# StephenTaf/Modern-Search-Engines-Project

Measured on AMD Instinct MI355X. Metric: queries/sec, two-stage retrieval top-100 (BM25 top-1000 + dense full scan + rerank/fuse), higher is better.
Workload: dtype f32 (exact f32 cosines of every returned document; candidates filtered by one pass of f16 products with a measured margin; batches <= 64 queries: f16x2-split products, |err| <= 8e-6) (dense cosine) / f64 (BM25, fuse)

## Files before the change

### modern-search-engines-project_amd/csrc/msr_common.h

```cpp
#pragma once
#include <hip/hip_runtime.h>
#include <stdint.h>

#define MSR_WAVE 64

__host__ __device__ __forceinline__ uint32_t msr_ord32(float f) {
    uint32_t u;
    __builtin_memcpy(&u, &f, 4);
    if (f == 0.0f) u = 0;
    return (u & 0x80000000u) ? ~u : (u | 0x80000000u);
}
__host__ __device__ __forceinline__ float msr_unord32(uint32_t u) {
    u = (u & 0x80000000u) ? (u & 0x7FFFFFFFu) : ~u;
    float f;
    __builtin_memcpy(&f, &u, 4);
    return f;
}
__host__ __device__ __forceinline__ uint64_t msr_ord64(double d) {
    uint64_t u;
    __builtin_memcpy(&u, &d, 8);
    if (d == 0.0) u = 0;
    return (u >> 63) ? ~u : (u | 0x8000000000000000ull);
}
__host__ __device__ __forceinline__ double msr_unord64(uint64_t u) {
    u = (u >> 63) ? (u & 0x7FFFFFFFFFFFFFFFull) : ~u;
    double d;
    __builtin_memcpy(&d, &u, 8);
    return d;
}

__device__ __forceinline__ bool msr_valid(float s) { return s > -__builtin_inff(); }
__device__ __forceinline__ bool msr_valid(double s) { return s > -__builtin_inf(); }
```

### modern-search-engines-project_amd/csrc/msr_dense.hip

```cpp
#include <stdlib.h>

#include <algorithm>
#include <type_traits>

#include "msr_common.h"
#include "msr_internal.h"
#include "msr_frag.h"

namespace {

constexpr int KSTEPS = MSR_DIM / 16;



template <int QB, int MODE, int WAVES, int OBD = 32> struct ScanCfgV2 {
    static constexpr int NL = MODE == MODE_BF16 ? MSR_DIM / 32 : MSR_DIM / 16;
    static constexpr int KS = MODE == MODE_F32 ? MSR_DIM / 16 : MSR_DIM / 32;
    static constexpr int QPIECES = MODE == MODE_F16X2 ? 2 : 1;
    static constexpr int ROW16 = MODE == MODE_BF16 ? MSR_DIM * 2 / 16 : MSR_DIM * 4 / 16;
    static constexpr int NQP = 16 * QB;
    static constexpr int SROW = NQP + 1;
    static constexpr int THREADS = WAVES * 64;
    static constexpr size_t q_bytes = (size_t)QB * KS * QPIECES * 64 * 16;
    static constexpr size_t t_bytes = (size_t)16 * SROW * 4;
    static constexpr size_t o_bytes = (size_t)OBD * SROW * 4;
    static constexpr size_t wave_bytes = (t_bytes + o_bytes + 15) & ~(size_t)15;
    static constexpr size_t total = q_bytes + WAVES * wave_bytes;
};

template <int QB, bool TILED, int LB, int MODE, int WAVES, int OBD = 32, int G = 1>
__global__ __launch_bounds__(WAVES * 64) void dense_scan_v2_kernel(DenseIndex ix, const void* __restrict__ emb,
                                                                    const int32_t* __restrict__ wspan,
                                                                    int n_wspans, const f32x4* __restrict__ qimg,
                                                                    int nq, int max_chunks,
                                                                    float* __restrict__ docscore, int dbg) {
    using L = ScanCfgV2<QB, MODE, WAVES, OBD>;
    constexpr int KS = L::KS, NL = L::NL;
    constexpr bool BF16 = MODE == MODE_BF16;
    constexpr bool DIRECT = OBD == 0;
    static_assert(OBD == 0 || OBD == 8 || OBD == 16 || OBD == 32, "staging depth");
    static_assert(NL % LB == 0 && (MODE != MODE_F16X2 || LB % 2 == 0), "whole load batches per group");
    static_assert(!(BF16 && TILED), "the interleaved image exists for f32 only");
    extern __shared__ __attribute__((aligned(16))) char smem[];
    f32x4* Qs = (f32x4*)smem;
    const int tid = threadIdx.x;
    const int lane = tid & 63;
    const int w = __builtin_amdgcn_readfirstlane(tid >> 6);
    float* T = (float*)(smem + L::q_bytes + (size_t)w * L::wave_bytes);
    float* OB = T + 16 * L::SROW;
    const int li = lane & 15, lg = lane >> 4;

    for (int idx = tid; idx < QB * KS * L::QPIECES * 64; idx += L::THREADS) Qs[idx] = qimg[idx];
    __syncthreads();

    const int s = blockIdx.x * WAVES + w;
    if (s >= n_wspans) return;
    if (ix.gate && *ix.gate == 0) return;
    const int64_t C = ix.n_chunks;
    const float NEG_INF = -__builtin_inff();
    const int d0 = wspan[s], d1 = wspan[s + 1];
    const int64_t c0 = ix.doc_off[d0], c1 = ix.doc_off[d1];

    int ob_base = d0, ob_n = 0;
    auto flush = [&]() {
        constexpr int OD = OBD > 0 ? OBD : 32;
        constexpr int QPI = 64 / OD;
        for (int qq0 = 0; qq0 < nq; qq0 += QPI) {
            const int qq = qq0 + lane / OD, dd = lane % OD;
            if (qq < nq && dd < ob_n && !(dbg & 1)) docscore[(int64_t)qq * ix.score_stride + ob_base + dd] = OB[dd * L::SROW + qq];
        }
        ob_base += ob_n;
        ob_n = 0;
    };
    auto emit = [&](float m) {
        if (DIRECT) {
            if (lane < nq) docscore[(int64_t)lane * ix.score_stride + ob_base] = m;
            ++ob_base;
            return;
        }
        if (lane < L::NQP) OB[ob_n * L::SROW + lane] = m;
        constexpr int OD = OBD > 0 ? OBD : 32;
        ++ob_n;
        if (((ob_base + ob_n) & (OD - 1)) == 0) flush();
    };

    int cur_doc = d0 - 1;
    bool open = false;
    int cnt = 0;
    float m = NEG_INF;

    if (c1 > c0) {
        constexpr int PSTRIDE = TILED ? 64 : 4;
        constexpr int NBATCH = NL / LB;
        const int64_t g0 = c0 >> 4, g1 = (c1 + 15) >> 4;
        auto row_ptr = [&](int64_t grp) -> const f32x4* {
            if (TILED) return (const f32x4*)emb + (size_t)grp * (16 * L::ROW16) + lane;
            int64_t r = grp * 16 + li;
            if (r > C - 1) r = C - 1;
            return (const f32x4*)emb + (size_t)r * L::ROW16 + lg;
        };
        auto meta_row = [&](int64_t grp) -> int64_t {
            int64_t r = grp * 16 + li;
            return r > C - 1 ? C - 1 : r;
        };
        auto clampg = [&](int64_t g) { return g < g1 ? g : g1 - 1; };
        f32x4 buf0[G][LB], buf1[G][LB];
        const f32x4* p[G];
        int dv[G];
        float iv[G];
#pragma unroll
        for (int g = 0; g < G; ++g) {
            p[g] = row_ptr(clampg(g0 + g));
#pragma unroll
            for (int u = 0; u < LB; ++u) buf0[g][u] = p[g][(size_t)u * PSTRIDE];
            dv[g] = ix.chunk_doc[meta_row(clampg(g0 + g))];
            iv[g] = ix.inv_norm[meta_row(clampg(g0 + g))];
        }
        __builtin_amdgcn_sched_barrier(0);
        auto body = [&](auto ph_c, int64_t grp) {
            constexpr int PH = decltype(ph_c)::value;
            const f32x4* pn[G];
#pragma unroll
            for (int g = 0; g < G; ++g) pn[g] = row_ptr(clampg(grp + G + g));
            const bool has_next = grp + G < g1;
            constexpr int NCH = (QB == 1 && G == 1) ? 2 : QB;
            f32x4 acc[G][NCH];
#pragma unroll
            for (int g = 0; g < G; ++g)
#pragma unroll
                for (int c = 0; c < NCH; ++c) acc[g][c] = (f32x4){0.f, 0.f, 0.f, 0.f};
            int dv_next[G];
            float iv_next[G];
#pragma unroll
            for (int g = 0; g < G; ++g) { dv_next[g] = dv[g]; iv_next[g] = iv[g]; }
#pragma unroll
            for (int nb = 0; nb < NBATCH; ++nb) {
                const bool into1 = ((nb + 1 + PH) & 1) != 0;
                if (nb + 1 < NBATCH) {
#pragma unroll
                    for (int g = 0; g < G; ++g)
#pragma unroll
                        for (int u = 0; u < LB; ++u) {
                            const f32x4 x = p[g][(size_t)((nb + 1) * LB + u) * PSTRIDE];
                            if (into1) buf1[g][u] = x; else buf0[g][u] = x;
                        }
                } else if (has_next) {
#pragma unroll
                    for (int g = 0; g < G; ++g) {
#pragma unroll
                        for (int u = 0; u < LB; ++u) {
                            const f32x4 x = pn[g][(size_t)u * PSTRIDE];
                            if (into1) buf1[g][u] = x; else buf0[g][u] = x;
                        }
                        dv_next[g] = ix.chunk_doc[meta_row(clampg(grp + G + g))];
                        iv_next[g] = ix.inv_norm[meta_row(clampg(grp + G + g))];
                    }
                }
                __builtin_amdgcn_sched_barrier(0);
                if constexpr (MODE == MODE_F16X2) {
#pragma unroll
                    for (int u = 0; u < LB; u += 2) {
                        const int t = (nb * LB + u) >> 1;
                        f16x8 ahi[G], alo[G];
#pragma unroll
                        for (int g = 0; g < G; ++g) {
                            const f32x4 a0 = ((nb + PH) & 1) ? buf1[g][u] : buf0[g][u];
                            const f32x4 a1 = ((nb + PH) & 1) ? buf1[g][u + 1] : buf0[g][u + 1];
                            split_f16(a0, a1, ahi[g], alo[g]);
                        }
                        f16x8 bhi[QB], blo[QB];
#pragma unroll
                        for (int qb = 0; qb < QB; ++qb) {
                            bhi[qb] = __builtin_bit_cast(f16x8, Qs[((qb * KS + t) * 2 + 0) * 64 + lane]);
                            blo[qb] = __builtin_bit_cast(f16x8, Qs[((qb * KS + t) * 2 + 1) * 64 + lane]);
                        }
                        if constexpr (NCH > QB) {
                            acc[0][0] = __builtin_amdgcn_mfma_f32_16x16x32_f16(alo[0], bhi[0], acc[0][0], 0, 0, 0);
                            acc[0][1] = __builtin_amdgcn_mfma_f32_16x16x32_f16(ahi[0], blo[0], acc[0][1], 0, 0, 0);
                            acc[0][t & 1] = __builtin_amdgcn_mfma_f32_16x16x32_f16(ahi[0], bhi[0], acc[0][t & 1], 0, 0, 0);
                        } else {
#pragma unroll
                            for (int piece = 0; piece < 3; ++piece)
#pragma unroll
                                for (int g = 0; g < G; ++g)
#pragma unroll
                                    for (int qb = 0; qb < QB; ++qb)
                                        acc[g][qb] = __builtin_amdgcn_mfma_f32_16x16x32_f16(
                                            piece == 0 ? alo[g] : ahi[g], piece == 1 ? blo[qb] : bhi[qb], acc[g][qb], 0, 0, 0);
                        }
                    }
                } else {
#pragma unroll
                    for (int u = 0; u < LB; ++u) {
                        const int t = nb * LB + u;
                        f32x4 a[G];
#pragma unroll
                        for (int g = 0; g < G; ++g) a[g] = ((nb + PH) & 1) ? buf1[g][u] : buf0[g][u];
                        f32x4 bq[QB];
#pragma unroll
                        for (int qb = 0; qb < QB; ++qb) bq[qb] = Qs[(qb * KS + t) * 64 + lane];
                        if constexpr (BF16) {
#pragma unroll
                            for (int g = 0; g < G; ++g)
#pragma unroll
                                for (int qb = 0; qb < QB; ++qb) {
                                    const int ch = NCH > QB ? (t & 1) : qb;
                                    acc[g][ch] = __builtin_amdgcn_mfma_f32_16x16x32_bf16(
                                        __builtin_bit_cast(bf16x8, a[g]), __builtin_bit_cast(bf16x8, bq[qb]), acc[g][ch], 0, 0, 0);
                                }
                        } else if constexpr (NCH > QB) {
                            acc[0][0] = __builtin_amdgcn_mfma_f32_16x16x4f32(a[0].x, bq[0].x, acc[0][0], 0, 0, 0);
                            acc[0][1] = __builtin_amdgcn_mfma_f32_16x16x4f32(a[0].y, bq[0].y, acc[0][1], 0, 0, 0);
                            acc[0][0] = __builtin_amdgcn_mfma_f32_16x16x4f32(a[0].z, bq[0].z, acc[0][0], 0, 0, 0);
                            acc[0][1] = __builtin_amdgcn_mfma_f32_16x16x4f32(a[0].w, bq[0].w, acc[0][1], 0, 0, 0);
                        } else {
#pragma unroll
                            for (int c = 0; c < 4; ++c)
#pragma unroll
                                for (int g = 0; g < G; ++g)
#pragma unroll
                                    for (int qb = 0; qb < QB; ++qb)
                                        acc[g][qb] = __builtin_amdgcn_mfma_f32_16x16x4f32(a[g][c], bq[qb][c], acc[g][qb], 0, 0, 0);
                        }
                    }
                }
            }
            if constexpr (NCH > QB) acc[0][0] = acc[0][0] + acc[0][1];
#pragma unroll
            for (int g = 0; g < G; ++g) {
#pragma unroll
                for (int reg = 0; reg < 4; ++reg) {
                    const float inv = __shfl(iv[g], 4 * lg + reg);
#pragma unroll
                    for (int qb = 0; qb < QB; ++qb) T[(4 * lg + reg) * L::SROW + 16 * qb + li] = acc[g][qb][reg] * inv;
                }
                const int64_t row0 = (grp + g) * 16;
#pragma unroll
                for (int r = 0; r < 16; ++r) {
                    const int64_t row = row0 + r;
                    const int d = __builtin_amdgcn_readlane(dv[g], r);
                    if (row < c0 || row >= c1) continue;
                    if (!open || d != cur_doc) {
                        if (open) emit(m);
                        for (int e = cur_doc + 1; e < d; ++e) emit(NEG_INF);
                        cur_doc = d; open = true; cnt = 0; m = NEG_INF;
                    }
                    if (max_chunks == 0 || cnt < max_chunks) {
                        const float v = lane < L::NQP ? T[r * L::SROW + lane] : NEG_INF;
                        m = fmaxf(m, v);
                    }
                    ++cnt;
                }
            }
#pragma unroll
            for (int g = 0; g < G; ++g) { p[g] = pn[g]; dv[g] = dv_next[g]; iv[g] = iv_next[g]; }
        };
        for (int64_t grp = g0; grp < g1;) {
            body(std::integral_constant<int, 0>{}, grp);
            grp += G;
            if constexpr ((NBATCH & 1) != 0) {
                if (grp >= g1) break;
                body(std::integral_constant<int, 1>{}, grp);
                grp += G;
            }
        }
    }
    if (open) emit(m);
    for (int e = cur_doc + 1; e < d1; ++e) emit(NEG_INF);
    if (ob_n) flush();
}

template <int MODE>
__global__ __launch_bounds__(256) void build_qimage_kernel(const float* __restrict__ qn, int n_blocks,
                                                            f32x4* __restrict__ qimg) {
    constexpr int KS = MODE == MODE_F32 ? MSR_DIM / 16 : MSR_DIM / 32;
    const int idx = blockIdx.x * 256 + threadIdx.x;
    if (idx >= n_blocks * KS * 64) return;
    const int l = idx & 63;
    const int t = (idx >> 6) % KS;
    const int qb = idx / (KS * 64);
    const float* src = qn + (size_t)(16 * qb + (l & 15)) * MSR_DIM;
    if (MODE == MODE_BF16) {
        const float* s8 = src + 32 * t + 8 * (l >> 4);
        bf16x8 v;
#pragma unroll
        for (int j = 0; j < 8; ++j) v[j] = (__bf16)s8[j];
        qimg[idx] = __builtin_bit_cast(f32x4, v);
    } else if (MODE == MODE_F16X2) {
        const f32x4 a = *(const f32x4*)(src + 16 * (2 * t) + 4 * (l >> 4));
        const f32x4 b = *(const f32x4*)(src + 16 * (2 * t + 1) + 4 * (l >> 4));
        f16x8 hi, lo;
        split_f16(a, b, hi, lo);
        qimg[(size_t)(idx >> 6) * 128 + l] = __builtin_bit_cast(f32x4, hi);
        qimg[(size_t)(idx >> 6) * 128 + 64 + l] = __builtin_bit_cast(f32x4, lo);
    } else {
        qimg[idx] = *(const f32x4*)(src + 16 * t + 4 * (l >> 4));
    }
}

__global__ __launch_bounds__(256) void fill_f32_kernel(float* __restrict__ dst, int64_t n, float value) {
    for (int64_t i = (int64_t)blockIdx.x * 256 + threadIdx.x; i < n; i += (int64_t)gridDim.x * 256) dst[i] = value;
}

__global__ __launch_bounds__(256) void prep_queries_kernel(const float* __restrict__ q, int nq,
                                                            float* __restrict__ qn, int nq_pad) {
    const int row = blockIdx.x * 4 + (threadIdx.x >> 6);
    const int lane = threadIdx.x & 63;
    if (row >= nq_pad) return;
    float v[12];
    float ss = 0.f;
    for (int j = 0; j < 12; ++j) {
        v[j] = row < nq ? q[(size_t)row * MSR_DIM + lane + 64 * j] : 0.f;
        ss += v[j] * v[j];
    }
    for (int off = 32; off > 0; off >>= 1) ss += __shfl_xor(ss, off);
    float nrm = sqrtf(ss);
    if (nrm == 0.f) nrm = 1.f;
    for (int j = 0; j < 12; ++j) qn[(size_t)row * MSR_DIM + lane + 64 * j] = v[j] / nrm;
}

__global__ void fill_chunk_doc_kernel(const int32_t* __restrict__ doc_off, int64_t n_docs,
                                      int32_t* __restrict__ chunk_doc) {
    const int64_t d = (int64_t)blockIdx.x * blockDim.x + threadIdx.x;
    if (d >= n_docs) return;
    for (int64_t c = doc_off[d]; c < doc_off[d + 1]; ++c) chunk_doc[c] = (int32_t)d;
}

__global__ __launch_bounds__(256) void row_inv_norm_kernel(const float* __restrict__ emb, int64_t n_rows,
                                                            float* __restrict__ inv_norm) {
    const int64_t row = (int64_t)blockIdx.x * 4 + (threadIdx.x >> 6);
    const int lane = threadIdx.x & 63;
    if (row >= n_rows) return;
    const f32x4* p = (const f32x4*)(emb + (size_t)row * MSR_DIM);
    float ss = 0.f;
    for (int j = 0; j < 3; ++j) {
        const f32x4 v = p[lane + 64 * j];
        ss += v.x * v.x + v.y * v.y + v.z * v.z + v.w * v.w;
    }
    for (int off = 32; off > 0; off >>= 1) ss += __shfl_xor(ss, off);
    float nrm = sqrtf(ss);
    if (nrm == 0.f) nrm = 1.f;
    if (lane == 0) inv_norm[row] = 1.0f / nrm;
}

__global__ __launch_bounds__(256) void interleave_kernel(const float* __restrict__ src, int64_t n_rows,
                                                          float* __restrict__ dst, int64_t n_vec) {
    for (int64_t v = (int64_t)blockIdx.x * blockDim.x + threadIdx.x; v < n_vec;
         v += (int64_t)gridDim.x * blockDim.x) {
        const int l = (int)(v & 63);
        const int64_t bt = v >> 6;
        const int t = (int)(bt % KSTEPS);
        const int64_t grp = bt / KSTEPS;
        const int64_t r = grp * 16 + (l & 15);
        f32x4 x = (f32x4){0.f, 0.f, 0.f, 0.f};
        if (r < n_rows) x = *(const f32x4*)(src + (size_t)r * MSR_DIM + 16 * t + 4 * (l >> 4));
        ((f32x4*)dst)[v] = x;
    }
}

template <bool TILED>
__global__ __launch_bounds__(64) void best_chunk_kernel(DenseIndex ix, const float* __restrict__ qn, int k,
                                                         int max_chunks, const int32_t* __restrict__ out_doc,
                                                         const int32_t* __restrict__ out_n,
                                                         int32_t* __restrict__ out_chunk, int per_wave) {
    const int q = blockIdx.y, lane = threadIdx.x;
    if (ix.gate && ix.gate[ix.gate_per64 ? q >> 6 : 0] == 0) return;
    float qv[12];
    for (int j = 0; j < 12; ++j) qv[j] = qn[(size_t)q * MSR_DIM + lane + 64 * j];
    const int r_end = (int)(blockIdx.x + 1) * per_wave < k ? (int)(blockIdx.x + 1) * per_wave : k;
    for (int r = blockIdx.x * per_wave; r < r_end; ++r) {
    if (r >= out_n[q]) {
        if (lane == 0) out_chunk[(int64_t)q * k + r] = -1;
        continue;
    }
    const int d = out_doc[(int64_t)q * k + r];
    const int64_t ds = ix.doc_off[d];
    int64_t de = ix.doc_off[d + 1];
    if (max_chunks > 0 && ds + max_chunks < de) de = ds + max_chunks;
    float best = -__builtin_inff();
    int64_t arg = -1;
    for (int64_t c = ds; c < de; ++c) {
        float s = 0.f;
        for (int j = 0; j < 12; ++j) {
            const int dim = lane + 64 * j;
            size_t off;
            if (TILED) {
                const int t = dim >> 4, g = (dim >> 2) & 3, e = dim & 3;
                off = (size_t)(c >> 4) * (16 * MSR_DIM) + ((size_t)t * 64 + g * 16 + (c & 15)) * 4 + e;
            } else {
                off = (size_t)c * MSR_DIM + dim;
            }
            s += ix.emb[off] * qv[j];
        }
        for (int o = 32; o > 0; o >>= 1) s += __shfl_xor(s, o);
        s *= ix.inv_norm[c];
        if (s > best) { best = s; arg = c; }
    }
    if (lane == 0) out_chunk[(int64_t)q * k + r] = (int32_t)arg;
    }
}

static int scan_debug_flags() {
#ifdef MSR_DIAG
    static const int v = [] { const char* e = getenv("MSR_SCAN_DEBUG"); return e ? atoi(e) : 0; }();
    return v;
#else
    return 0;
#endif
}

template <int QB, bool TILED, int LB, int WAVES = 8, int OBD = 32, int MODE = MODE_F32, int G = 1>
hipError_t launch_scan_v2(const DenseIndex& ix, const float* qn, int nq, int max_chunks, float* docscore,
                          hipStream_t stream) {
    using L = ScanCfgV2<QB, MODE, WAVES, OBD>;
    static_assert(L::total <= 160 * 1024, "LDS budget");
    const size_t lds = L::total;
    hipError_t err = hipFuncSetAttribute((const void*)dense_scan_v2_kernel<QB, TILED, LB, MODE, WAVES, OBD, G>,
                                         hipFuncAttributeMaxDynamicSharedMemorySize, (int)lds);
    if (err != hipSuccess) return err;
    const int n_img = QB * L::KS * 64;
    build_qimage_kernel<MODE><<<(n_img + 255) / 256, 256, 0, stream>>>(qn, QB, (f32x4*)ix.qimg);
    const int32_t* spans = WAVES == 12 ? ix.wspan12_doc : ix.wspan_doc;
    const int n_sp = WAVES == 12 ? ix.n_wspans12 : ix.n_wspans;
    const int grid = (n_sp + WAVES - 1) / WAVES;
    dense_scan_v2_kernel<QB, TILED, LB, MODE, WAVES, OBD, G><<<grid, L::THREADS, lds, stream>>>(
        ix, ix.emb, spans, n_sp, (const f32x4*)ix.qimg, nq, max_chunks, docscore, scan_debug_flags());
    return hipGetLastError();
}

template <int QB, int WAVES, int OBD, int LB = 12>
hipError_t launch_scan_bf16_cfg(const DenseIndex& ix, const float* qn, int nq, int max_chunks, float* docscore,
                                hipStream_t stream) {
    using L = ScanCfgV2<QB, MODE_BF16, WAVES, OBD>;
    const size_t lds = L::total;
    static_assert(L::total <= 160 * 1024, "LDS budget");
    hipError_t err = hipFuncSetAttribute((const void*)dense_scan_v2_kernel<QB, false, LB, MODE_BF16, WAVES, OBD>,
                                         hipFuncAttributeMaxDynamicSharedMemorySize, (int)lds);
    if (err != hipSuccess) return err;
    const int n_img = QB * L::KS * 64;
    build_qimage_kernel<MODE_BF16><<<(n_img + 255) / 256, 256, 0, stream>>>(qn, QB, (f32x4*)ix.qimg);
    const int grid = (ix.n_wspans + WAVES - 1) / WAVES;
    dense_scan_v2_kernel<QB, false, LB, MODE_BF16, WAVES, OBD><<<grid, L::THREADS, lds, stream>>>(
        ix, ix.emb_bf16, ix.wspan_doc, ix.n_wspans, (const f32x4*)ix.qimg, nq, max_chunks, docscore, scan_debug_flags());
    return hipGetLastError();
}

template <int QB>
hipError_t launch_scan_bf16(const DenseIndex& ix, const float* qn, int nq, int max_chunks, float* docscore,
                            hipStream_t stream) {
    if constexpr (QB <= 2) return launch_scan_bf16_cfg<QB, 8, 32>(ix, qn, nq, max_chunks, docscore, stream);
#ifdef MSR_DIAG
    static const int knob = [] { const char* v = getenv("MSR_BF16_CFG"); return v ? atoi(v) : 0; }();
    if (knob == 1) return launch_scan_bf16_cfg<QB, 8, 8>(ix, qn, nq, max_chunks, docscore, stream);
    if (knob == 2) return launch_scan_bf16_cfg<QB, 8, 0>(ix, qn, nq, max_chunks, docscore, stream);
    if (knob == 3) return launch_scan_bf16_cfg<QB, 4, 32, 24>(ix, qn, nq, max_chunks, docscore, stream);
#endif
    return launch_scan_bf16_cfg<QB, 4, 32>(ix, qn, nq, max_chunks, docscore, stream);
}

template <int QB, bool TILED>
hipError_t dispatch_variant(const DenseIndex& ix, const float* qn, int nq, int max_chunks, float* docscore,
                            hipStream_t stream) {
    if (ix.variant == 2) return launch_scan_v2<QB, TILED, 12>(ix, qn, nq, max_chunks, docscore, stream);
    return launch_scan_v2<QB, TILED, 12, 8, 32, MODE_F16X2>(ix, qn, nq, max_chunks, docscore, stream);
}

__global__ __launch_bounds__(256) void norm_range_kernel(const float* __restrict__ inv_norm, int64_t n,
                                                          uint32_t* __restrict__ out) {
    uint32_t lo = 0x7F800000u, hi = 0;
    for (int64_t i = (int64_t)blockIdx.x * 256 + threadIdx.x; i < n; i += (int64_t)gridDim.x * 256) {
        const uint32_t u = __float_as_uint(inv_norm[i]);
        lo = u < lo ? u : lo; hi = u > hi ? u : hi;
    }
    for (int o = 32; o > 0; o >>= 1) {
        const uint32_t a = __shfl_xor(lo, o), b = __shfl_xor(hi, o);
        lo = a < lo ? a : lo; hi = b > hi ? b : hi;
    }
    if ((threadIdx.x & 63) == 0) { atomicMin(&out[0], lo); atomicMax(&out[1], hi); }
}

}

hipError_t msr_dense_scan(const DenseIndex& ix, const float* qn, int nq, int max_chunks, float* docscore,
                          hipStream_t stream) {
    if (nq <= 0 || ix.n_docs <= 0) return hipSuccess;
    if ((ix.variant == 14 || ix.variant == 15) && ix.wide_ok && ix.layout == 0 && max_chunks == 0)
        return msr_dense_scan_wide(ix, qn, nq, docscore, stream);
    if (ix.variant == 2 && nq > 32 && ix.wide_ok && ix.layout == 0 && max_chunks == 0)
        return msr_dense_scan_wide_exact(ix, qn, nq, docscore, stream);
    if (nq > 32) return hipErrorInvalidValue;
    const bool tiled = ix.layout == 1;
    if (nq <= 16)
        return tiled ? dispatch_variant<1, true>(ix, qn, nq, max_chunks, docscore, stream)
                     : dispatch_variant<1, false>(ix, qn, nq, max_chunks, docscore, stream);
    return tiled ? dispatch_variant<2, true>(ix, qn, nq, max_chunks, docscore, stream)
                 : dispatch_variant<2, false>(ix, qn, nq, max_chunks, docscore, stream);
}

hipError_t msr_build_qimage(int mode, const float* qn, int n_blocks, void* qimg, hipStream_t stream) {
    const int ks = mode == MODE_F32 ? MSR_DIM / 16 : MSR_DIM / 32;
    const int n_img = n_blocks * ks * 64;
    const int grid = (n_img + 255) / 256;
    if (mode == MODE_F32) build_qimage_kernel<MODE_F32><<<grid, 256, 0, stream>>>(qn, n_blocks, (f32x4*)qimg);
    else if (mode == MODE_BF16) build_qimage_kernel<MODE_BF16><<<grid, 256, 0, stream>>>(qn, n_blocks, (f32x4*)qimg);
    else build_qimage_kernel<MODE_F16X2><<<grid, 256, 0, stream>>>(qn, n_blocks, (f32x4*)qimg);
    return hipGetLastError();
}

hipError_t msr_inv_norm_range(const float* inv_norm, int64_t n, uint32_t* out2, hipStream_t stream) {
    const uint32_t init[2] = {0x7F800000u, 0u};
    hipError_t err = hipMemcpyAsync(out2, init, sizeof(init), hipMemcpyHostToDevice, stream);
    if (err != hipSuccess) return err;
    if (n > 0) norm_range_kernel<<<1024, 256, 0, stream>>>(inv_norm, n, out2);
    return hipGetLastError();
}

hipError_t msr_dense_scan_bf16(const DenseIndex& ix, const float* qn, int nq, int max_chunks, float* docscore,
                               hipStream_t stream) {
    if (nq <= 0 || ix.n_docs <= 0) return hipSuccess;
    if (nq > 64 || !ix.emb_bf16) return hipErrorInvalidValue;
    if (nq <= 16) return launch_scan_bf16<1>(ix, qn, nq, max_chunks, docscore, stream);
    if (nq <= 32) return launch_scan_bf16<2>(ix, qn, nq, max_chunks, docscore, stream);
    if (nq <= 48) return launch_scan_bf16<3>(ix, qn, nq, max_chunks, docscore, stream);
    return launch_scan_bf16<4>(ix, qn, nq, max_chunks, docscore, stream);
}

hipError_t msr_fill_f32(float* dst, int64_t n, float value, hipStream_t stream) {
    if (n <= 0) return hipSuccess;
    fill_f32_kernel<<<(unsigned)std::min<int64_t>((n + 255) / 256, 65536), 256, 0, stream>>>(dst, n, value);
    return hipGetLastError();
}

hipError_t msr_prep_queries(const float* q, int nq, float* qn, int nq_pad, hipStream_t stream) {
    if (nq_pad <= 0) return hipSuccess;
    prep_queries_kernel<<<(nq_pad + 3) / 4, 256, 0, stream>>>(q, nq, qn, nq_pad);
    return hipGetLastError();
}

hipError_t msr_fill_chunk_doc(const int32_t* doc_off, int64_t n_docs, int32_t* chunk_doc, hipStream_t stream) {
    if (n_docs <= 0) return hipSuccess;
    fill_chunk_doc_kernel<<<(unsigned)((n_docs + 255) / 256), 256, 0, stream>>>(doc_off, n_docs, chunk_doc);
    return hipGetLastError();
}

hipError_t msr_row_inv_norm(const float* emb, int64_t n_rows, float* inv_norm, hipStream_t stream) {
    if (n_rows <= 0) return hipSuccess;
    row_inv_norm_kernel<<<(unsigned)((n_rows + 3) / 4), 256, 0, stream>>>(emb, n_rows, inv_norm);
    return hipGetLastError();
}

hipError_t msr_interleave(const float* src, int64_t n_rows, float* dst, hipStream_t stream) {
    if (n_rows <= 0) return hipSuccess;
    const int64_t n_vec = ((n_rows + 15) / 16) * KSTEPS * 64;
    int64_t blocks = (n_vec + 255) / 256;
    if (blocks > 65536) blocks = 65536;
    interleave_kernel<<<(unsigned)blocks, 256, 0, stream>>>(src, n_rows, dst, n_vec);
    return hipGetLastError();
}

hipError_t msr_best_chunk(const DenseIndex& ix, const float* qn, int nq, int k, int max_chunks,
                          const int32_t* out_doc, const int32_t* out_n, int32_t* out_chunk, hipStream_t stream) {
    if (nq <= 0 || k <= 0) return hipSuccess;
    const int per_wave = ix.gate ? 16 : 1;
    dim3 grid((unsigned)((k + per_wave - 1) / per_wave), (unsigned)nq);
    if (ix.layout == 1)
        best_chunk_kernel<true><<<grid, 64, 0, stream>>>(ix, qn, k, max_chunks, out_doc, out_n, out_chunk, per_wave);
    else
        best_chunk_kernel<false><<<grid, 64, 0, stream>>>(ix, qn, k, max_chunks, out_doc, out_n, out_chunk, per_wave);
    return hipGetLastError();
}
```

### modern-search-engines-project_amd/csrc/msr_engine.hip

```cpp
#include <hip/hip_runtime.h>
#include <stdarg.h>
#include <stdio.h>
#include <stdlib.h>
#include <string.h>

#include <algorithm>
#include <new>
#include <vector>

#include "../../include/msretr.h"
#include "msr_devmem.h"
#include "msr_internal.h"

struct HipMem {
    static hipError_t alloc(void** p, size_t bytes) { return hipMalloc(p, bytes); }
    static void free(void* p) { (void)hipFree(p); }
};
using Group = DevGroup<HipMem>;

struct msr_engine {
    msr_config cfg;
    char err[512];
    Group mem_engine;
    Group mem_corpus;
// ... 988 lines not shown
    if (n_rows == 0) return MSR_OK;
    HIP_TRY(e, hipSetDevice(e->cfg.device));
    HIP_TRY(e, msr_phrase_sets_run(e->tok_off, e->tok_ids, e->bm25.n_docs, e->bm25.n_terms, n_rows, phrase_off, phrase_terms,
                                   cand_bits, n_cand, cand_stride, row_cand, out_bits, out_stride, (hipStream_t)stream));
    return MSR_OK;
}

extern "C" int msr_proximity_sets(msr_engine* e, int32_t n_rows, const int32_t* phrase_off, const int32_t* phrase_terms,
                                  const int32_t* row_span, const int32_t* row_ordered, const uint32_t* cand_bits, int32_t n_cand,
                                  int64_t cand_stride, const int32_t* row_cand, uint32_t* out_bits, int64_t out_stride,
                                  void* stream) {
    if (!e) return MSR_ERR_INVALID;
    int rc = tokens_bound(e, "msr_proximity_sets");
    if (rc) return rc;
    rc = set_rows_args_ok(e, "msr_proximity_sets", n_rows, out_bits && phrase_off && row_span && row_ordered,
                          "out_bits, phrase_off, row_span or row_ordered", out_stride, "n_cand", n_cand, cand_bits && row_cand,
                          "cand_bits or row_cand", "cand_stride", cand_stride);
    if (rc) return rc;
    if (n_rows == 0) return MSR_OK;
    HIP_TRY(e, hipSetDevice(e->cfg.device));
    HIP_TRY(e, msr_proximity_sets_run(e->tok_off, e->tok_ids, e->bm25.n_docs, e->bm25.n_terms, n_rows, phrase_off, phrase_terms,
                                      row_span, row_ordered, cand_bits, n_cand, cand_stride, row_cand, out_bits, out_stride,
                                      (hipStream_t)stream));
    return MSR_OK;
}

extern "C" int msr_best_windows(msr_engine* e, int32_t n_pairs, const int32_t* pair_doc, const int32_t* pair_row, int32_t n_rows,
                                const int32_t* row_off, const int32_t* row_terms, const int32_t* row_weights,
                                const int32_t* row_span, int32_t* out_start, int32_t* out_cover, int32_t* out_hits,
                                uint64_t* out_mask, uint32_t* out_terms, void* stream) {
    if (!e) return MSR_ERR_INVALID;
    const int rc = tokens_bound(e, "msr_best_windows");
    if (rc) return rc;
    if (n_pairs < 0 || n_rows < 0)
        return fail(e, MSR_ERR_INVALID, "msr_best_windows: bad argument (n_pairs=%d, n_rows=%d)", n_pairs, n_rows);
    if (n_pairs == 0) return MSR_OK;
    if (n_rows == 0) return fail(e, MSR_ERR_INVALID, "msr_best_windows: bad argument (n_rows=0 with n_pairs=%d)", n_pairs);
    if (!pair_doc || !pair_row || !row_off || !row_terms || !row_weights || !row_span)
        return fail(e, MSR_ERR_INVALID, "msr_best_windows: bad argument (pair_doc, pair_row, row_off, row_terms, row_weights or "
                    "row_span is NULL with n_pairs=%d)", n_pairs);
    if (!out_start || !out_cover || !out_hits || !out_mask || !out_terms)
        return fail(e, MSR_ERR_INVALID, "msr_best_windows: bad argument (an output pointer is NULL with n_pairs=%d)", n_pairs);
    HIP_TRY(e, hipSetDevice(e->cfg.device));
    HIP_TRY(e, msr_best_windows_run(e->tok_off, e->tok_ids, e->bm25.n_docs, e->bm25.n_terms, n_pairs, pair_doc, pair_row, n_rows,
                                    row_off, row_terms, row_weights, row_span, out_start, out_cover, out_hits, out_mask, out_terms,
                                    (hipStream_t)stream));
    return MSR_OK;
}

extern "C" int msr_bind_vocab(msr_engine* e, const int64_t* char_off, const uint16_t* chars, const uint32_t* weight,
                              int64_t n_terms, int64_t n_chars, void* stream) {
    if (!e) return MSR_ERR_INVALID;
    if (!e->have_postings) return fail(e, MSR_ERR_NOT_BOUND, "msr_bind_vocab: postings not bound");
    HIP_TRY(e, hipSetDevice(e->cfg.device));
    drop_vocab(e);
    if (!char_off || !weight || n_chars < 0 || (n_chars > 0 && !chars)) return fail(e, MSR_ERR_INVALID, "msr_bind_vocab: bad argument");
    if (n_terms != e->bm25.n_terms)
        return fail(e, MSR_ERR_INVALID, "msr_bind_vocab: n_terms %lld differs from bound postings (%lld)", (long long)n_terms,
                    (long long)e->bm25.n_terms);
    hipStream_t st = (hipStream_t)stream;
    if (!e->sim_flag) ALLOC(e, e->mem_engine, e->sim_flag, 64);
    int32_t flag = 0;
    HIP_TRY(e, hipMemsetAsync(e->sim_flag, 0, sizeof(int32_t), st));
    HIP_TRY(e, msr_vocab_validate(char_off, weight, n_terms, n_chars, e->sim_flag, st));
    HIP_TRY(e, hipMemcpyAsync(&flag, e->sim_flag, sizeof(int32_t), hipMemcpyDeviceToHost, st));
    HIP_TRY(e, hipStreamSynchronize(st));
    if (flag) {
        static const char* why[] = {"", "char_off does not run from 0 to n_chars", "char_off descends",
                                    "a weight is 2^31 or more"};
        return fail(e, MSR_ERR_INVALID, "msr_bind_vocab: malformed vocabulary: %s", why[std::min(std::max(flag, 0), 3)]);
    }
    ALLOC(e, e->mem_postings, e->voc_sig, (size_t)std::max<int64_t>(n_terms, 1) * sizeof(uint64_t));
    hipError_t err = msr_vocab_signatures(char_off, chars, n_terms, e->voc_sig, st);
    if (err == hipSuccess) err = hipStreamSynchronize(st);
    if (err != hipSuccess) {
        e->mem_postings.free_one(&e->voc_sig);
        return fail(e, MSR_ERR_HIP, "msr_bind_vocab: %s", hipGetErrorString(err));
    }
    e->voc_char_off = char_off; e->voc_chars = chars; e->voc_weight = weight; e->voc_n_chars = n_chars;
    e->have_vocab = true;
    return MSR_OK;
}

extern "C" int64_t msr_fuzzy_scratch_bytes(int64_t n_terms, int32_t n_words, int32_t limit) {
    if (n_terms < 0 || n_terms >= (1ll << 31) || n_words < 0 || n_words > MSR_FUZZY_MAX_WORDS || limit < 1 ||
        limit > MSR_FUZZY_MAX_LIMIT)
        return -1;
    return (int64_t)n_words * msr_fuzzy_spans(n_terms) * ((int64_t)limit * 8 + 4);
}

extern "C" int msr_fuzzy_terms(msr_engine* e, int32_t n_words, const int32_t* word_off, const uint16_t* word_chars,
                               const int32_t* word_max, int32_t limit, int32_t* out_term, int32_t* out_dist, int32_t* out_n,
                               int32_t* out_total, void* scratch, int64_t scratch_bytes, void* stream) {
    if (!e) return MSR_ERR_INVALID;
    if (!e->have_postings || !e->have_vocab)
        return fail(e, MSR_ERR_NOT_BOUND, "msr_fuzzy_terms: vocabulary not bound (msr_bind_vocab: the index has no term strings)");
    if (n_words < 0 || n_words > MSR_FUZZY_MAX_WORDS || limit < 1 || limit > MSR_FUZZY_MAX_LIMIT)
        return fail(e, MSR_ERR_INVALID, "msr_fuzzy_terms: bad argument (n_words=%d, at most %d; limit=%d, 1 .. %d)", n_words,
                    MSR_FUZZY_MAX_WORDS, limit, MSR_FUZZY_MAX_LIMIT);
    if (n_words == 0) return MSR_OK;
    if (!word_off || !word_chars || !word_max || !out_term || !out_dist || !out_n || !out_total || !scratch)
        return fail(e, MSR_ERR_INVALID, "msr_fuzzy_terms: bad argument (a NULL pointer with n_words=%d)", n_words);
    const int64_t need = msr_fuzzy_scratch_bytes(e->bm25.n_terms, n_words, limit);
    if (need < 0 || scratch_bytes < need || ((uintptr_t)scratch & 7))
        return fail(e, MSR_ERR_INVALID, "msr_fuzzy_terms: bad argument (scratch_bytes=%lld, needed %lld, 8-byte aligned)",
                    (long long)scratch_bytes, (long long)need);
    HIP_TRY(e, hipSetDevice(e->cfg.device));
    HIP_TRY(e, msr_fuzzy_terms_run(e->voc_char_off, e->voc_chars, e->voc_weight, e->voc_sig, e->bm25.n_terms, n_words, word_off,
                                   word_chars, word_max, limit, out_term, out_dist, out_n, out_total, scratch,
                                   (hipStream_t)stream));
    return MSR_OK;
}

extern "C" int64_t msr_wildcard_scratch_bytes(int64_t n_terms, int32_t n_patterns, int32_t limit) {
    if (n_terms < 0 || n_terms >= (1ll << 31) || n_patterns < 0 || n_patterns > MSR_WILD_MAX_PATTERNS || limit < 1 ||
        limit > MSR_WILD_MAX_LIMIT)
        return -1;
    return (int64_t)n_patterns * msr_fuzzy_spans(n_terms) * ((int64_t)limit * 8 + 4);
}

extern "C" int msr_wildcard_terms(msr_engine* e, int32_t n_patterns, const int32_t* pat_off, const uint16_t* pat_chars,
                                  int32_t limit, int32_t* out_term, int32_t* out_n, int32_t* out_total, void* scratch,
                                  int64_t scratch_bytes, void* stream) {
    if (!e) return MSR_ERR_INVALID;
    if (!e->have_postings || !e->have_vocab)
        return fail(e, MSR_ERR_NOT_BOUND, "msr_wildcard_terms: vocabulary not bound (msr_bind_vocab: the index has no term strings)");
    if (n_patterns < 0 || n_patterns > MSR_WILD_MAX_PATTERNS || limit < 1 || limit > MSR_WILD_MAX_LIMIT)
        return fail(e, MSR_ERR_INVALID, "msr_wildcard_terms: bad argument (n_patterns=%d, at most %d; limit=%d, 1 .. %d)",
                    n_patterns, MSR_WILD_MAX_PATTERNS, limit, MSR_WILD_MAX_LIMIT);
    if (n_patterns == 0) return MSR_OK;
    if (!pat_off || !pat_chars || !out_term || !out_n || !out_total || !scratch)
        return fail(e, MSR_ERR_INVALID, "msr_wildcard_terms: bad argument (a NULL pointer with n_patterns=%d)", n_patterns);
    const int64_t need = msr_wildcard_scratch_bytes(e->bm25.n_terms, n_patterns, limit);
    if (need < 0 || scratch_bytes < need || ((uintptr_t)scratch & 7))
        return fail(e, MSR_ERR_INVALID, "msr_wildcard_terms: bad argument (scratch_bytes=%lld, needed %lld, 8-byte aligned)",
                    (long long)scratch_bytes, (long long)need);
    HIP_TRY(e, hipSetDevice(e->cfg.device));
    HIP_TRY(e, msr_wildcard_terms_run(e->voc_char_off, e->voc_chars, e->voc_weight, e->voc_sig, e->bm25.n_terms, n_patterns,
                                      pat_off, pat_chars, limit, out_term, out_n, out_total, scratch, (hipStream_t)stream));
    return MSR_OK;
}

extern "C" int msr_combine_sets(msr_engine* e, int32_t n_rows, const int32_t* and_off, const int32_t* and_rows,
                                const int32_t* not_off, const int32_t* not_rows, const uint32_t* in_bits, int32_t n_in,
                                int64_t in_stride, uint32_t* out_bits, int64_t out_stride, void* stream) {
    if (!e) return MSR_ERR_INVALID;
    if (!e->have_postings) return fail(e, MSR_ERR_NOT_BOUND, "msr_combine_sets: postings not bound");
    const int rc = set_rows_args_ok(e, "msr_combine_sets", n_rows, out_bits && and_off && not_off, "out_bits, and_off or not_off",
                                    out_stride, "n_in", n_in, in_bits != nullptr, "in_bits", "in_stride", in_stride);
    if (rc) return rc;
    if (n_rows == 0) return MSR_OK;
    HIP_TRY(e, hipSetDevice(e->cfg.device));
    HIP_TRY(e, msr_combine_sets_run(e->bm25.n_docs, n_rows, and_off, and_rows, not_off, not_rows, in_bits, n_in, in_stride,
                                    out_bits, out_stride, (hipStream_t)stream));
    return MSR_OK;
}

extern "C" int msr_debug_bm25_split(msr_engine* e, int32_t n_queries, int32_t* tiles_per_item, int32_t* n_segments) {
    if (!e) return MSR_ERR_INVALID;
    if (!e->have_postings) return fail(e, MSR_ERR_NOT_BOUND, "msr_debug_bm25_split: postings not bound");
    if (n_queries < 1 || n_queries > e->cfg.max_queries || !tiles_per_item || !n_segments)
        return fail(e, MSR_ERR_INVALID, "msr_debug_bm25_split: bad argument (n_queries=%d, max_queries=%d)", n_queries,
                    e->cfg.max_queries);
    int tpw = 1, n_spans = 0;
    msr_bm25_split(e->bm25.n_tiles, n_queries, &tpw, &n_spans);
    *tiles_per_item = tpw;
    *n_segments = n_spans;
    return MSR_OK;
}

extern "C" int msr_debug_select(msr_engine* e, int32_t mode, const void* scores, int64_t n, int64_t stride, int32_t n_queries,
                                int32_t k, const int32_t* idx, const int32_t* counts, int32_t n_seg, int64_t seg_stride,
                                const uint64_t* win_base, const uint32_t* set_bits, int32_t n_sets, int64_t set_stride,
                                const int32_t* q_set, const int32_t* gate, int32_t gate_per64, int32_t* out_doc, void* out_score,
                                int32_t* out_n, msr_select_state* out_state, void* stream) {
    static_assert(sizeof(msr_select_state) == sizeof(SelState), "msr_select_state mirrors SelState");
    if (!e) return MSR_ERR_INVALID;
    if (mode < MSR_SELECT_F32 || mode > MSR_SELECT_F64_LIST)
        return fail(e, MSR_ERR_INVALID, "msr_debug_select: bad argument (mode=%d)", mode);
    if (n_queries < 1 || n_queries > e->cfg.max_queries || k < 1 || k > e->cfg.max_k)
        return fail(e, MSR_ERR_INVALID, "msr_debug_select: bad argument (n_queries=%d, max_queries=%d, k=%d, max_k=%d)", n_queries,
                    e->cfg.max_queries, k, e->cfg.max_k);
    if (!scores || !out_doc || !out_score || !out_n || n < 0 || n >= (1ll << 31) || stride < n)
        return fail(e, MSR_ERR_INVALID, "msr_debug_select: bad argument (NULL scores or output, or n=%lld, stride=%lld)",
                    (long long)n, (long long)stride);
    if (mode == MSR_SELECT_F64_LIST && (!idx || !counts || n_seg < 1 || seg_stride < 0 || (int64_t)n_seg * seg_stride > stride))
        return fail(e, MSR_ERR_INVALID, "msr_debug_select: bad argument (list: idx or counts NULL, n_seg=%d < 1, or n_seg * "
                    "seg_stride=%lld > stride=%lld)", n_seg, (long long)seg_stride, (long long)stride);
    if (mode == MSR_SELECT_F32_WITHIN &&
        (n_sets < 1 || !set_bits || !q_set || set_stride < (n + 31) / 32))
        return fail(e, MSR_ERR_INVALID, "msr_debug_select: bad argument (within: n_sets=%d < 1, set_bits or q_set NULL, or "
                    "set_stride=%lld < ceil(n / 32))", n_sets, (long long)set_stride);
    hipStream_t st = (hipStream_t)stream;
    HIP_TRY(e, hipSetDevice(e->cfg.device));
    SelScratch sel = e->sel;
    sel.gate = gate;
    sel.gate_per64 = gate && gate_per64 ? 1 : 0;
    switch (mode) {
    case MSR_SELECT_F32:
        HIP_TRY(e, msr_select_topk(32, scores, n, stride, n_queries, k, sel, out_doc, out_score, out_n, st));
        break;
    case MSR_SELECT_F64:
        HIP_TRY(e, msr_select_topk(64, scores, n, stride, n_queries, k, sel, out_doc, out_score, out_n, st));
        break;
    case MSR_SELECT_F32_WITHIN: {
        const MsrSetView set{set_bits, set_stride, q_set, n_sets};
        HIP_TRY(e, msr_select_topk_within((const float*)scores, n, stride, n_queries, k, sel, set, out_doc, (float*)out_score,
                                          out_n, st));
        break;
    }
    default:
        HIP_TRY(e, msr_select_topk_list((const double*)scores, idx, counts, n_seg, seg_stride, stride, n_queries, k, sel, out_doc,
                                        (double*)out_score, out_n, st, win_base));
    }
    if (out_state)
        HIP_TRY(e, hipMemcpyAsync(out_state, e->sel.state, (size_t)n_queries * sizeof(SelState), hipMemcpyDeviceToDevice, st));
    return MSR_OK;
}

extern "C" int msr_bm25_score_docs(msr_engine* e, const int32_t* q_term_off, const int32_t* q_terms, const int32_t* q_qtf,
                                   int32_t n_queries, const int32_t* doc, const int32_t* doc_n, int32_t max_docs,
                                   double* out_score, int32_t* out_touched, void* stream) {
    if (!e) return MSR_ERR_INVALID;
    if (!e->have_postings) return fail(e, MSR_ERR_NOT_BOUND, "msr_bm25_score_docs: postings not bound");
    if (n_queries < 0 || max_docs < 0 || !q_term_off || (n_queries > 0 && max_docs > 0 && (!doc || !out_score || !out_touched)))
        return fail(e, MSR_ERR_INVALID, "msr_bm25_score_docs: bad argument (n_queries=%d, max_docs=%d)", n_queries, max_docs);
    if (n_queries == 0 || max_docs == 0) return MSR_OK;
    HIP_TRY(e, hipSetDevice(e->cfg.device));
    HIP_TRY(e, msr_bm25_point(e->bm25, q_term_off, q_terms, q_qtf, n_queries, doc, doc_n, max_docs, out_score, out_touched,
                              (hipStream_t)stream));
    return MSR_OK;
}

extern "C" int msr_union_candidates(msr_engine* e, int32_t n_queries, const int32_t* lex_doc, const double* lex_score,
                                    const int32_t* lex_n, int32_t k_lex, const int32_t* dense_doc, const double* dense_bm25,
                                    const int32_t* dense_n, int32_t k_dense, int32_t* out_doc, double* out_score, int32_t* out_src,
                                    int32_t* out_n, int32_t max_cand, void* stream) {
    if (!e) return MSR_ERR_INVALID;
    if (n_queries < 0 || k_lex < 0 || k_lex > MSR_MAX_K || k_dense < 0 || k_dense > MSR_MAX_K || max_cand < 1 ||
        (int64_t)k_lex + k_dense > max_cand)
        return fail(e, MSR_ERR_INVALID, "msr_union_candidates: bad argument (k_lex=%d, k_dense=%d: each in [0, %d], their sum <= "
                    "max_cand=%d)", k_lex, k_dense, MSR_MAX_K, max_cand);
    if (!out_doc || !out_score || !out_src || !out_n || (k_lex > 0 && (!lex_doc || !lex_score || !lex_n)) ||
        (k_dense > 0 && (!dense_doc || !dense_bm25 || !dense_n)))
        return fail(e, MSR_ERR_INVALID, "msr_union_candidates: bad argument (NULL list)");
    if (n_queries == 0) return MSR_OK;
    HIP_TRY(e, hipSetDevice(e->cfg.device));
    HIP_TRY(e, msr_union_lists(n_queries, lex_doc, lex_score, lex_n, k_lex, dense_doc, dense_bm25, dense_n, k_dense, out_doc,
                               out_score, out_src, out_n, max_cand, (hipStream_t)stream));
    return MSR_OK;
}

static int dense_gated_fallback(msr_engine* e, int nq, int k, int32_t* out_doc, float* out_score, int32_t* out_chunk,
                                int32_t* out_n, hipStream_t st) {
    const int64_t N = e->dense.n_docs;
    DenseIndex ix = e->dense;
    ix.gate = e->gf_gate;
    HIP_TRY(e, msr_dense_scan_slices(ix, e->gf_qn, nq, (float*)e->score_rows, e->gf_fb_qimg, st));
    SelScratch sel = e->sel;
    sel.gate = e->gf_gate; sel.gate_per64 = 1;
    HIP_TRY(e, msr_select_topk(32, e->score_rows, N, e->dense.score_stride, nq, k, sel, out_doc, out_score, out_n, st));
    ix.gate = e->gf_gate; ix.gate_per64 = 1;
    if (out_chunk) HIP_TRY(e, msr_best_chunk(ix, e->gf_qn, nq, k, 0, out_doc, out_n, out_chunk, st));
    return MSR_OK;
}

static bool dense_sweep_wide(const msr_engine* e, int max_chunks_per_doc) {
    return (e->dense.variant == 2 || e->dense.variant == 14 || e->dense.variant == 15) && e->dense.layout == 0 &&
           e->dense.wide_ok && max_chunks_per_doc == 0;
}

static bool dense_stream_ok(const msr_engine* e, int k) {
    return dense_sweep_wide(e, 0) && e->gf_ok && e->dense.variant == 14 && e->gf.n_tiles >= 2 * k;
}

static int dense_stream_cap(const msr_engine* e) { return e->gf.max_groups >= 2 ? (e->gf.max_groups & ~1) * 128 : 128; }

static hipEvent_t* pass_events(msr_engine* e, int kind, hipEvent_t ev[4]) {
    if (!e->timing || e->ev_count[kind] >= msr_engine::EV_RING || e->ev_count[3] >= msr_engine::EV_RING) return nullptr;
    ev[0] = e->ev_start[3][e->ev_count[3]]; ev[1] = e->ev_stop[3][e->ev_count[3]];
    ev[2] = e->ev_start[kind][e->ev_count[kind]]; ev[3] = e->ev_stop[kind][e->ev_count[kind]];
    return ev;
}
static void pass_events_used(msr_engine* e, int kind, const hipEvent_t* ev) {
    if (ev) { e->ev_count[kind]++; e->ev_count[3]++; }
}

extern "C" int msr_dense_split_max(const msr_engine* e, int32_t k) {
    if (!e || !e->have_chunks || k < 1 || k > e->cfg.max_k || !dense_stream_ok(e, k)) return 0;
    return dense_stream_cap(e);
}

extern "C" int msr_dense_topk_begin(msr_engine* e, const float* q, int32_t n_queries, int32_t k, int32_t k_part, float* out_part,
                                    void* stream) {
    if (!e) return MSR_ERR_INVALID;
    if (!e->have_chunks) return fail(e, MSR_ERR_NOT_BOUND, "msr_dense_topk_begin: chunks not bound");
    if (e->split_pending) return fail(e, MSR_ERR_INVALID, "msr_dense_topk_begin: the previous begin has not been ended");
    const int cap = msr_dense_split_max(e, k);
    if (!q || !out_part || k_part < 1 || k_part > k || n_queries <= 64 || n_queries > cap)
        return fail(e, MSR_ERR_INVALID, "msr_dense_topk_begin: needs 64 < n_queries <= msr_dense_split_max() = %d, 1 <= k_part <= k (got %d, %d, %d)",
                    cap, n_queries, k_part, k);
    hipStream_t st = (hipStream_t)stream;
    HIP_TRY(e, hipSetDevice(e->cfg.device));
    HIP_TRY(e, msr_prep_queries(q, n_queries, e->gf_qn, (n_queries + 63) / 64 * 64, st));
    HIP_TRY(e, hipMemsetAsync(e->gf_gate, 0, GF_GATE_BYTES, st));
    hipEvent_t ev_buf[4];
    hipEvent_t* ev = pass_events(e, 0, ev_buf);
    int width = 0;
    int segs = 0;
    HIP_TRY(e, msr_gemm_f32_pass(e->gf, e->dense, e->gf_qn, n_queries, k, k_part, out_part, ev, &width, &segs, st));
    e->last_dense_width = width;
    e->last_dense_segments = segs;
    pass_events_used(e, 0, ev);
    e->split_pending = n_queries;
    return MSR_OK;
}

extern "C" int msr_dense_topk_end(msr_engine* e, int32_t n_queries, int32_t k, const float* bound, int32_t* out_doc,
                                  float* out_score, int32_t* out_chunk, int32_t* out_n, void* stream) {
    if (!e) return MSR_ERR_INVALID;
    if (!e->have_chunks) return fail(e, MSR_ERR_NOT_BOUND, "msr_dense_topk_end: chunks not bound");
    if (!e->gf_ok || e->split_pending != n_queries || n_queries <= 0)
        return fail(e, MSR_ERR_INVALID, "msr_dense_topk_end: no matching msr_dense_topk_begin (pending %d, got %d)", e->split_pending, n_queries);
    if (!out_doc || !out_score || !out_n || k < 1 || k > e->cfg.max_k) return fail(e, MSR_ERR_INVALID, "msr_dense_topk_end: bad argument");
    e->split_pending = 0;
    hipStream_t st = (hipStream_t)stream;
    HIP_TRY(e, hipSetDevice(e->cfg.device));
    HIP_TRY(e, msr_gemm_f32_finish(e->gf, e->dense, e->gf_qn, n_queries, k, bound, out_doc, out_score, out_chunk, out_n, e->gf_gate, st));
    return dense_gated_fallback(e, n_queries, k, out_doc, out_score, out_chunk, out_n, st);
}

static int dense_sweeps(msr_engine* e, const float* q, int q0, int cnt, int k, int max_chunks_per_doc, bool wide, const int32_t* gate,
                        int32_t* out_doc, float* out_score, int32_t* out_chunk, int32_t* out_n, hipStream_t st,
                        const MsrSetView* set) {
    const int64_t N = e->dense.n_docs;
    const int slice = wide ? 64 : 32;
    DenseIndex ix = e->dense;
    SelScratch sel = e->sel;
    for (int s0 = q0; s0 < q0 + cnt; s0 += slice) {
        const int nq = std::min(slice, q0 + cnt - s0);
        ix.gate = sel.gate = gate ? gate + (s0 - q0) / 64 : nullptr;
        const int nq_pad = nq > 32 ? 64 : (nq > 16 || (wide && e->dense.variant >= 14)) ? 32 : 16;
        const bool timed = !gate && e->timing && e->ev_count[0] < msr_engine::EV_RING;
        HIP_TRY(e, msr_prep_queries(q + (int64_t)s0 * MSR_DIM, nq, e->qn, nq_pad, st));
        if (timed) HIP_TRY(e, hipEventRecord(e->ev_start[0][e->ev_count[0]], st));
        HIP_TRY(e, msr_dense_scan(ix, e->qn, nq, max_chunks_per_doc, (float*)e->score_rows, st));
        if (timed) {
            HIP_TRY(e, hipEventRecord(e->ev_stop[0][e->ev_count[0]], st));
            e->ev_count[0]++;
        }
        if (set) {
            MsrSetView sv = *set;
            sv.q_set += s0;
            HIP_TRY(e, msr_select_topk_within((const float*)e->score_rows, N, e->dense.score_stride, nq, k, sel, sv,
                                              out_doc + (int64_t)s0 * k, out_score + (int64_t)s0 * k, out_n + s0, st));
        } else {
            HIP_TRY(e, msr_select_topk(32, e->score_rows, N, e->dense.score_stride, nq, k, sel, out_doc + (int64_t)s0 * k,
                                       out_score + (int64_t)s0 * k, out_n + s0, st));
        }
        if (out_chunk)
            HIP_TRY(e, msr_best_chunk(ix, e->qn, nq, k, max_chunks_per_doc, out_doc + (int64_t)s0 * k,
                                      out_n + s0, out_chunk + (int64_t)s0 * k, st));
    }
    return MSR_OK;
}

extern "C" int msr_dense_topk(msr_engine* e, const float* q, int32_t n_queries, int32_t k, int32_t max_chunks_per_doc,
                              int32_t* out_doc, float* out_score, int32_t* out_chunk, int32_t* out_n, void* stream) {
    if (!e) return MSR_ERR_INVALID;
    if (!e->have_chunks) return fail(e, MSR_ERR_NOT_BOUND, "msr_dense_topk: chunks not bound");
    if (e->split_pending)
        return fail(e, MSR_ERR_INVALID, "msr_dense_topk: an msr_dense_topk_begin is pending (its scratch is in use): call msr_dense_topk_end first");
    if (n_queries < 0 || k < 1 || k > e->cfg.max_k || max_chunks_per_doc < 0 || !q || !out_doc || !out_score || !out_n)
        return fail(e, MSR_ERR_INVALID, "msr_dense_topk: bad argument (k=%d, max_k=%d)", k, e->cfg.max_k);
    if (n_queries == 0) return MSR_OK;
    hipStream_t st = (hipStream_t)stream;
    HIP_TRY(e, hipSetDevice(e->cfg.device));
    const bool wide = dense_sweep_wide(e, max_chunks_per_doc);
    const bool gemm = wide && dense_stream_ok(e, k);
    e->last_dense_width = gemm && n_queries > 64 ? 0 : (wide ? 64 : 32);
    e->last_dense_segments = 0;
    int q0 = 0;
    while (q0 < n_queries) {
        const int left = n_queries - q0;
        if (gemm && left > 64) {
            const int nq = std::min(dense_stream_cap(e), left);
            HIP_TRY(e, msr_prep_queries(q + (int64_t)q0 * MSR_DIM, nq, e->gf_qn, (nq + 63) / 64 * 64, st));
            HIP_TRY(e, hipMemsetAsync(e->gf_gate, 0, GF_GATE_BYTES, st));
            hipEvent_t ev_buf[4];
            hipEvent_t* ev = pass_events(e, 0, ev_buf);
            int width = 0, segs = 0;
            HIP_TRY(e, msr_gemm_f32_topk(e->gf, e->dense, e->gf_qn, nq, k, out_doc + (int64_t)q0 * k,
                                         out_score + (int64_t)q0 * k, out_chunk ? out_chunk + (int64_t)q0 * k : nullptr,
                                         out_n + q0, e->gf_gate, ev, &width, &segs, st));
            e->last_dense_width = std::max(e->last_dense_width, width);
            e->last_dense_segments = segs;
            pass_events_used(e, 0, ev);
            {
                int rcf = dense_gated_fallback(e, nq, k, out_doc + (int64_t)q0 * k, out_score + (int64_t)q0 * k,
                                               out_chunk ? out_chunk + (int64_t)q0 * k : nullptr, out_n + q0, st);
                if (rcf) return rcf;
            }
            q0 += nq;
        } else {
            const int nq = std::min(wide ? 64 : 32, left);
            int rc = dense_sweeps(e, q, q0, nq, k, max_chunks_per_doc, wide, nullptr, out_doc, out_score, out_chunk, out_n, st,
                                  nullptr);
            if (rc) return rc;
            q0 += nq;
        }
    }
    return MSR_OK;
}

extern "C" int msr_dense_topk_within(msr_engine* e, const float* q, int32_t n_queries, int32_t k, int32_t max_chunks_per_doc,
                                     const uint32_t* set_bits, int32_t n_sets, int64_t set_stride, const int32_t* q_set,
                                     int32_t* out_doc, float* out_score, int32_t* out_chunk, int32_t* out_n, void* stream) {
    if (!e) return MSR_ERR_INVALID;
    if (!e->have_chunks) return fail(e, MSR_ERR_NOT_BOUND, "msr_dense_topk_within: chunks not bound");
    if (e->split_pending)
        return fail(e, MSR_ERR_INVALID, "msr_dense_topk_within: an msr_dense_topk_begin is pending (its scratch is in use): call msr_dense_topk_end first");
    if (n_queries < 0 || k < 1 || k > e->cfg.max_k || max_chunks_per_doc < 0 || !q || !out_doc || !out_score || !out_n)
        return fail(e, MSR_ERR_INVALID, "msr_dense_topk_within: bad argument (k=%d, max_k=%d)", k, e->cfg.max_k);
    {
        const int rc = within_args_ok(e, "msr_dense_topk_within", e->dense.n_docs, set_bits, n_sets, set_stride, q_set);
        if (rc) return rc;
    }
    if (n_sets == 0)
        return msr_dense_topk(e, q, n_queries, k, max_chunks_per_doc, out_doc, out_score, out_chunk, out_n, stream);
    if (n_queries == 0) return MSR_OK;
    hipStream_t st = (hipStream_t)stream;
    HIP_TRY(e, hipSetDevice(e->cfg.device));
    const bool wide = dense_sweep_wide(e, max_chunks_per_doc);
    e->last_dense_width = wide ? 64 : 32;
    e->last_dense_segments = 0;
    const MsrSetView set{set_bits, set_stride, q_set, n_sets};
    return dense_sweeps(e, q, 0, n_queries, k, max_chunks_per_doc, wide, nullptr, out_doc, out_score, out_chunk, out_n, st, &set);
}

static int sim_out_of_range(msr_engine* e, const int32_t* v, int64_t n, int64_t hi, hipStream_t st) {
    if (!e->sim_flag) ALLOC(e, e->mem_engine, e->sim_flag, 64);
    int32_t flag = 0;
    HIP_TRY(e, hipMemsetAsync(e->sim_flag, 0, sizeof(int32_t), st));
    HIP_TRY(e, msr_check_range(v, n, hi, e->sim_flag, st));
    HIP_TRY(e, hipMemcpyAsync(&flag, e->sim_flag, sizeof(int32_t), hipMemcpyDeviceToHost, st));
    HIP_TRY(e, hipStreamSynchronize(st));
    return flag ? 1 : 0;
}

extern "C" int msr_gather_rows(msr_engine* e, const int32_t* rows, int32_t n, float* out, void* stream) {
    if (!e) return MSR_ERR_INVALID;
    if (!e->have_chunks) return fail(e, MSR_ERR_NOT_BOUND, "msr_gather_rows: chunks not bound");
    if (n < 0 || (n > 0 && (!rows || !out))) return fail(e, MSR_ERR_INVALID, "msr_gather_rows: bad argument (n=%d)", n);
    if (n == 0) return MSR_OK;
    hipStream_t st = (hipStream_t)stream;
    HIP_TRY(e, hipSetDevice(e->cfg.device));
    const int bad = sim_out_of_range(e, rows, n, e->dense.n_chunks, st);
    if (bad < 0) return bad;
    if (bad) return fail(e, MSR_ERR_INVALID, "msr_gather_rows: a row lies outside [0, n_chunks = %lld)", (long long)e->dense.n_chunks);
    HIP_TRY(e, msr_gather_rows_run(e->dense, rows, n, out, st));
    return MSR_OK;
}

extern "C" int msr_dense_topk_grouped(msr_engine* e, const float* q, int32_t n_rows, const int32_t* group_off, int32_t n_groups,
                                      const int32_t* excl_off, const int32_t* excl_doc, int32_t k, float min_score,
                                      const uint32_t* set_bits, int32_t n_sets, int64_t set_stride, const int32_t* g_set,
                                      int32_t* out_doc, float* out_score, int32_t* out_chunk, int32_t* out_src_row,
                                      int32_t* out_n, void* stream) {
    static const char* fn = "msr_dense_topk_grouped";
    if (!e) return MSR_ERR_INVALID;
    if (!e->have_chunks) return fail(e, MSR_ERR_NOT_BOUND, "%s: chunks not bound", fn);
    if (e->split_pending)
        return fail(e, MSR_ERR_INVALID, "%s: an msr_dense_topk_begin is pending (its scratch is in use): call msr_dense_topk_end first", fn);
    if (n_rows < 0 || n_groups < 0 || k < 1 || k > e->cfg.max_k || min_score != min_score || !group_off || !excl_off ||
        (n_rows > 0 && !q) || (n_groups > 0 && (!out_doc || !out_score || !out_chunk || !out_src_row || !out_n)))
        return fail(e, MSR_ERR_INVALID, "%s: bad argument (n_rows=%d, n_groups=%d, k=%d, max_k=%d)", fn, n_rows, n_groups, k,
                    e->cfg.max_k);
    {
        const int rc = within_args_ok(e, fn, e->dense.n_docs, set_bits, n_sets, set_stride, g_set);
        if (rc) return rc;
    }
    hipStream_t st = (hipStream_t)stream;
    HIP_TRY(e, hipSetDevice(e->cfg.device));
    std::vector<int32_t> h_goff((size_t)n_groups + 1), h_eoff((size_t)n_groups + 1);
    HIP_TRY(e, hipMemcpyAsync(h_goff.data(), group_off, h_goff.size() * sizeof(int32_t), hipMemcpyDeviceToHost, st));
    HIP_TRY(e, hipMemcpyAsync(h_eoff.data(), excl_off, h_eoff.size() * sizeof(int32_t), hipMemcpyDeviceToHost, st));
    HIP_TRY(e, hipStreamSynchronize(st));
    if (h_goff[0] != 0 || h_goff[n_groups] != n_rows)
        return fail(e, MSR_ERR_INVALID, "%s: group_off must run from 0 to n_rows = %d (got %d .. %d)", fn, n_rows, h_goff[0],
                    h_goff[n_groups]);
    if (h_eoff[0] != 0) return fail(e, MSR_ERR_INVALID, "%s: excl_off[0] = %d, must be 0", fn, h_eoff[0]);
    int max_excl = 0;
    for (int g = 0; g < n_groups; ++g) {
        if (h_goff[g + 1] < h_goff[g]) return fail(e, MSR_ERR_INVALID, "%s: group_off not monotone at group %d", fn, g);
        if (h_eoff[g + 1] < h_eoff[g]) return fail(e, MSR_ERR_INVALID, "%s: excl_off not monotone at group %d", fn, g);
        max_excl = std::max(max_excl, h_eoff[g + 1] - h_eoff[g]);
    }
    if ((int64_t)k + max_excl > e->cfg.max_k)
        return fail(e, MSR_ERR_INVALID, "%s: k + max |excl_g| = %lld exceeds max_k = %d", fn, (long long)k + max_excl, e->cfg.max_k);
    const int64_t n_excl = h_eoff[n_groups];
    if (n_excl > 0) {
        if (!excl_doc) return fail(e, MSR_ERR_INVALID, "%s: excl_doc is NULL with %lld exclusions", fn, (long long)n_excl);
        const int bad = sim_out_of_range(e, excl_doc, n_excl, e->dense.n_docs, st);
        if (bad < 0) return bad;
        if (bad) return fail(e, MSR_ERR_INVALID, "%s: an excluded document lies outside [0, n_docs = %lld)", fn, (long long)e->dense.n_docs);
    }
    if (n_groups == 0) return MSR_OK;
    const int kk = k + max_excl;
    const size_t L = (size_t)n_rows * kk;
    const size_t lists_bytes = (L * 3 + 2 * (size_t)n_rows + 64) * 4;
    int rc = grow(e, e->mem_engine, &e->sim_lists, &e->sim_lists_bytes, lists_bytes, "grouped lists");
    if (rc) return rc;
    rc = grow(e, e->mem_engine, &e->sim_over, &e->sim_over_bytes, 2 * L * 16 + 64, "grouped merge records");
    if (rc) return rc;
    int32_t* l_doc = (int32_t*)e->sim_lists;
    float* l_score = (float*)(l_doc + L);
    int32_t* l_chunk = (int32_t*)(l_score + L);
    int32_t* l_n = l_chunk + L;
    int32_t* row_set = l_n + n_rows;
    if (n_sets > 0) HIP_TRY(e, msr_group_row_sets(group_off, n_groups, g_set, row_set, st));
    for (int r0 = 0; r0 < n_rows; r0 += e->cfg.max_queries) {
        const int cnt = std::min(e->cfg.max_queries, n_rows - r0);
        const int64_t o = (int64_t)r0 * kk;
        rc = msr_dense_topk_within(e, q + (int64_t)r0 * MSR_DIM, cnt, kk, 0, set_bits, n_sets, set_stride,
                                   n_sets > 0 ? row_set + r0 : nullptr, l_doc + o, l_score + o, l_chunk + o, l_n + r0, stream);
        if (rc) return rc;
    }
    GroupedMergeArgs a{};
    a.l_doc = l_doc; a.l_score = l_score; a.l_chunk = l_chunk; a.l_n = l_n; a.kk = kk;
    a.group_off = group_off; a.excl_off = excl_off; a.excl_doc = excl_doc; a.k = k; a.min_score = min_score;
    a.out_doc = out_doc; a.out_score = out_score; a.out_chunk = out_chunk; a.out_src = out_src_row; a.out_n = out_n;
    a.g_hi = (uint64_t*)e->sim_over;
    a.g_lo = (uint32_t*)(a.g_hi + 2 * L);
    a.g_val = a.g_lo + 2 * L;
    HIP_TRY(e, msr_grouped_merge(a, n_groups, st));
    return MSR_OK;
}

static int rerank_args_ok(msr_engine* e, const char* fn, int32_t n_queries, int32_t max_cand, int32_t max_chunks) {
    if (n_queries < 0 || max_cand < 1 || max_cand > e->cfg.rerank_max_docs)
        return fail(e, MSR_ERR_INVALID, "%s: bad argument (max_cand=%d, rerank_max_docs=%d)", fn, max_cand,
                    e->cfg.rerank_max_docs);
    if (max_chunks < 1 || max_chunks > MSR_RERANK_MAX_CHUNKS)
        return fail(e, MSR_ERR_INVALID, "%s: max_chunks out of range [1, %d]", fn, MSR_RERANK_MAX_CHUNKS);
    return MSR_OK;
}

static constexpr int BT_SLICE = 128;
static constexpr int GM_SLICE = 1024;
static constexpr int GM_WV_CAP = 16384;

static int build_bf16(msr_engine* e, hipStream_t st) {
    const int64_t C = e->dense.n_chunks;
    const int64_t n_pad = C + 512;
    ALLOC(e, e->mem_bf16, e->emb_bf16, (size_t)n_pad * MSR_DIM * 2);
    const size_t QS = GM_SLICE;
    if (!e->bt_top_doc) ALLOC(e, e->mem_engine, e->bt_top_doc, (size_t)BT_SLICE * MSR_MAX_K * 4);
    if (!e->bt_top_score) ALLOC(e, e->mem_engine, e->bt_top_score, (size_t)BT_SLICE * MSR_MAX_K * 4);
    if (!e->bt_top_n) ALLOC(e, e->mem_engine, e->bt_top_n, (size_t)BT_SLICE * 4);
    if (!e->bt_cand_doc) ALLOC(e, e->mem_engine, e->bt_cand_doc, QS * MSR_SEL_CAP * 4);
    if (!e->bt_cand_score) ALLOC(e, e->mem_engine, e->bt_cand_score, QS * MSR_SEL_CAP * 4);
    if (!e->bt_cand_chunk) ALLOC(e, e->mem_engine, e->bt_cand_chunk, QS * MSR_SEL_CAP * 4);
    if (!e->bt_cand_n) ALLOC(e, e->mem_engine, e->bt_cand_n, QS * 4);
    ALLOC(e, e->mem_bf16, e->bf_ones, (size_t)C * 4);
    ALLOC(e, e->mem_bf16, e->bf_err, 4);
    ALLOC(e, e->mem_bf16, e->bf_margin, QS * 4);
    HIP_TRY(e, hipMemsetAsync(e->bt_cand_n, 0, QS * 4, st));
    HIP_TRY(e, msr_unit_bf16_rows(e->dense.emb, e->dense.inv_norm, C, n_pad, e->emb_bf16, e->bf_err, st));
    HIP_TRY(e, msr_fill_f32(e->bf_ones, C, 1.0f, st));
    e->dense.emb_bf16 = e->emb_bf16;
    e->dense_bf16 = e->dense;
    e->dense_bf16.inv_norm = e->bf_ones;
    if (e->dense.wide_ok) {
        ALLOC(e, e->mem_bf16, e->bf_row_meta, (size_t)(C + 16) * 8);
        HIP_TRY(e, msr_pack_row_meta(e->chunk_doc, e->bf_ones, C, e->bf_row_meta, st));
        e->dense_bf16.row_meta = e->bf_row_meta;
    }
    const int n_tiles = e->n_tiles;
    const int grid = e->n_cus / 8 * 8;
    if (e->tiles_ok && n_tiles >= 64 && grid >= 32) {
        const int stride = (n_tiles + 31) / 32 * 32;
        GemmIndex& g = e->gemm;
        g.emb_n = e->emb_bf16; g.tile_row = e->tile_row; g.n_tiles = n_tiles; g.n_cus = e->n_cus; g.max_queries = GM_SLICE;
        g.tmax_stride = stride; g.wv_cap = GM_WV_CAP;
        ALLOC(e, e->mem_bf16, g.qmat, (size_t)GM_SLICE * MSR_DIM * 2);
        ALLOC(e, e->mem_bf16, e->gm_qn, (size_t)GM_SLICE * MSR_DIM * 4);
        ALLOC(e, e->mem_bf16, g.tmax, (size_t)GM_SLICE * stride * 4);
        ALLOC(e, e->mem_bf16, g.tmax_t, (size_t)n_tiles * 2 * GM_SLICE * 4);
        ALLOC(e, e->mem_bf16, g.thr, (size_t)GM_SLICE * 4);
        ALLOC(e, e->mem_bf16, g.thr2, (size_t)GM_SLICE * 4);
        ALLOC(e, e->mem_bf16, g.flag, (size_t)GM_SLICE * 4);
        ALLOC(e, e->mem_bf16, g.wgbuf, (size_t)grid * 8 * GM_WV_CAP * 16);
        ALLOC(e, e->mem_bf16, g.wv_count, (size_t)grid * 8 * 4);
        ALLOC(e, e->mem_bf16, g.pairs, (size_t)GM_SLICE * msr_gemm_pair_cap() * 8);
        ALLOC(e, e->mem_bf16, g.pair_n, (size_t)GM_SLICE * 4);
        HIP_TRY(e, hipMemsetAsync(g.pair_n, 0, (size_t)GM_SLICE * 4, st));
        e->gemm_ok = true;
    }
    return MSR_OK;
}

extern "C" int msr_enable_bf16(msr_engine* e, void* stream) {
    if (!e) return MSR_ERR_INVALID;
    if (!e->have_chunks) return fail(e, MSR_ERR_NOT_BOUND, "msr_enable_bf16: chunks not bound");
    if (e->cfg.scan_layout != 0) return fail(e, MSR_ERR_INVALID, "msr_enable_bf16: needs the row-major layout");
    if (e->emb_bf16) return MSR_OK;
    HIP_TRY(e, hipSetDevice(e->cfg.device));
    const int rc = build_bf16(e, (hipStream_t)stream);
    if (rc) drop_bf16(e);
    return rc;
}

extern "C" int msr_tune(msr_engine* e, int32_t key, int32_t value) {
    if (!e) return MSR_ERR_INVALID;
#ifdef MSR_DIAG
    if (key == 100) { msr_gemm_set_dbg(value); return MSR_OK; }
    if (key == 101) { msr_gemm_f32_set_dbg(value); return MSR_OK; }
    if (key == 102) { msr_bm25_set_dbg(value); return MSR_OK; }
#endif
    return fail(e, MSR_ERR_INVALID, "msr_tune: unknown key %d / value %d", key, value);
}

extern "C" int msr_batch_gemm_ok(const msr_engine* e) { return e && e->have_chunks && e->emb_bf16 && e->gemm_ok ? 1 : 0; }

extern "C" int msr_dense_topk_bf16(msr_engine* e, const float* q, int32_t n_queries, int32_t k,
                                   int32_t max_chunks_per_doc, int32_t* out_doc, float* out_score, int32_t* out_chunk,
                                   int32_t* out_n, void* stream) {
    if (!e) return MSR_ERR_INVALID;
    if (!e->have_chunks || !e->emb_bf16) return fail(e, MSR_ERR_NOT_BOUND, "msr_dense_topk_bf16: call msr_enable_bf16 first");
    if (e->split_pending)
        return fail(e, MSR_ERR_INVALID, "msr_dense_topk_bf16: an msr_dense_topk_begin is pending (its scratch is in use): call msr_dense_topk_end first");
    if (n_queries < 0 || k < 1 || k > e->cfg.max_k || max_chunks_per_doc < 0 || !q || !out_doc || !out_score || !out_n)
        return fail(e, MSR_ERR_INVALID, "msr_dense_topk_bf16: bad argument (k=%d, max_k=%d)", k, e->cfg.max_k);
    if (n_queries == 0) return MSR_OK;
    hipStream_t st = (hipStream_t)stream;
    HIP_TRY(e, hipSetDevice(e->cfg.device));
    const int64_t N = e->dense.n_docs;
    if (e->gemm_ok && max_chunks_per_doc == 0 && n_queries > BT_SLICE && e->gemm.n_tiles >= 2 * k) {
        for (int q0 = 0; q0 < n_queries; q0 += GM_SLICE) {
            const int nq = std::min(GM_SLICE, n_queries - q0);
            HIP_TRY(e, msr_prep_queries(q + (int64_t)q0 * MSR_DIM, nq, e->gm_qn, nq, st));
            HIP_TRY(e, msr_batch_margin(e->gm_qn, nq, e->bf_err, e->bf_margin, st));
            hipEvent_t ev_buf[4];
            hipEvent_t* ev = pass_events(e, 2, ev_buf);
            HIP_TRY(e, msr_gemm_candidates(e->gemm, e->dense, e->gm_qn, nq, k, e->bf_margin, e->bt_cand_doc, e->bt_cand_chunk,
                                           e->bt_cand_n, ev, st));
            pass_events_used(e, 2, ev);
            HIP_TRY(e, msr_batch_rescore_rows(e->dense, e->gm_qn, nq, k, (const int32_t*)e->gemm.pairs, 2, msr_gemm_pair_cap(),
                                              e->bt_cand_doc, e->bt_cand_score, e->bt_cand_chunk, e->bt_cand_n,
                                              out_doc + (int64_t)q0 * k, out_score + (int64_t)q0 * k,
                                              out_chunk ? out_chunk + (int64_t)q0 * k : nullptr, out_n + q0, st));
        }
        return MSR_OK;
    }
#ifdef MSR_DIAG
    static const bool wide_knob = [] { const char* v = getenv("MSR_BF16_WIDE"); return !v || atoi(v) != 0; }();
#else
    const bool wide_knob = true;
#endif
    const bool wide_able = wide_knob && e->dense.wide_ok && max_chunks_per_doc == 0;
    const int slice = wide_able && e->dense.wide_ok64 ? 128 : 64;
    for (int q0 = 0; q0 < n_queries; q0 += slice) {
        const int nq = std::min(slice, n_queries - q0);
        const bool wide = wide_able && nq > 32;
        const int nq_pad = wide ? (nq > 64 ? 128 : 64) : (nq + 15) / 16 * 16;
        HIP_TRY(e, msr_prep_queries(q + (int64_t)q0 * MSR_DIM, nq, e->qn, nq_pad, st));
        HIP_TRY(e, msr_batch_margin(e->qn, nq, e->bf_err, e->bf_margin, st));
        const bool timed = e->timing && e->ev_count[0] < msr_engine::EV_RING;
        if (timed) HIP_TRY(e, hipEventRecord(e->ev_start[0][e->ev_count[0]], st));
        if (wide) HIP_TRY(e, msr_dense_scan_bf16_wide(e->dense_bf16, e->qn, nq, (float*)e->score_rows, st));
        else HIP_TRY(e, msr_dense_scan_bf16(e->dense_bf16, e->qn, nq, max_chunks_per_doc, (float*)e->score_rows, st));
        if (timed) {
            HIP_TRY(e, hipEventRecord(e->ev_stop[0][e->ev_count[0]], st));
            e->ev_count[0]++;
        }
        HIP_TRY(e, msr_select_topk(32, (const float*)e->score_rows, N, e->dense.score_stride, nq, k, e->sel, e->bt_top_doc,
                                   e->bt_top_score, e->bt_top_n, st));
        HIP_TRY(e, msr_batch_finish(e->dense, e->qn, nq, k, max_chunks_per_doc, e->bf_margin, (const float*)e->score_rows,
                                    e->bt_top_score, e->bt_top_n, e->bt_cand_doc, e->bt_cand_score, e->bt_cand_chunk,
                                    e->bt_cand_n, out_doc + (int64_t)q0 * k, out_score + (int64_t)q0 * k,
                                    out_chunk ? out_chunk + (int64_t)q0 * k : nullptr, out_n + q0, st));
    }
    return MSR_OK;
}

static int rerank_gather_impl(msr_engine* e, const char* fn, const float* q, int32_t n_queries, const int32_t* cand_doc,
                              const int32_t* cand_n, int32_t max_cand, int32_t doc_base, int32_t row_base, int32_t max_chunks,
                              float* out_cos, int32_t* out_meta, int32_t q_per_block, int64_t block_stride, void* stream,
                              const RerankRecords* rec = nullptr) {
    if (!e) return MSR_ERR_INVALID;
    if (!e->have_chunks) return fail(e, MSR_ERR_NOT_BOUND, "%s: chunks not bound", fn);
    if (!q || !cand_doc || !cand_n || (!rec && (!out_cos || !out_meta))) return fail(e, MSR_ERR_INVALID, "%s: null argument", fn);
    int rc = rerank_args_ok(e, fn, n_queries, max_cand, max_chunks);
    if (rc) return rc;
    if (e->url_group && e->url_group_n != e->dense.n_docs)
        return fail(e, MSR_ERR_INVALID, "%s: doc meta bound for %lld docs, chunks for %lld", fn,
                    (long long)e->url_group_n, (long long)e->dense.n_docs);
// ... 176 lines not shown
```

### modern-search-engines-project_amd/csrc/msr_frag.h

```cpp
#pragma once
#include <hip/hip_runtime.h>

typedef float f32x4 __attribute__((ext_vector_type(4)));
typedef __bf16 bf16x8 __attribute__((ext_vector_type(8)));
typedef _Float16 f16x8 __attribute__((ext_vector_type(8)));
typedef _Float16 f16x2 __attribute__((ext_vector_type(2)));

constexpr int MODE_F32 = 0, MODE_BF16 = 1, MODE_F16X2 = 2, MODE_PRE = 3;

__device__ __forceinline__ void split_f16(const f32x4& a, const f32x4& b, f16x8& hi, f16x8& lo) {
    const float x[8] = {a.x, a.y, a.z, a.w, b.x, b.y, b.z, b.w};
#pragma unroll
    for (int j = 0; j < 8; j += 2) {
        const f16x2 h = __builtin_bit_cast(f16x2, __builtin_amdgcn_cvt_pkrtz(x[j], x[j + 1]));
        const f16x2 l = __builtin_bit_cast(f16x2, __builtin_amdgcn_cvt_pkrtz(x[j] - (float)h[0], x[j + 1] - (float)h[1]));
        hi[j] = h[0]; hi[j + 1] = h[1];
        lo[j] = l[0]; lo[j + 1] = l[1];
    }
}

__device__ __forceinline__ f16x8 cvt_f16_rtn(const f32x4& a, const f32x4& b) {
    f16x8 h;
    h[0] = (_Float16)a.x; h[1] = (_Float16)a.y; h[2] = (_Float16)a.z; h[3] = (_Float16)a.w;
    h[4] = (_Float16)b.x; h[5] = (_Float16)b.y; h[6] = (_Float16)b.z; h[7] = (_Float16)b.w;
    return h;
}
__device__ __forceinline__ float f16_err2(float x) {
    const float h = (float)(_Float16)x;
    const float d = __builtin_fabsf(h) < 6.103515625e-05f ? x : h - x;
    return d * d;
}
```

### modern-search-engines-project_amd/csrc/msr_gemm.hip

```cpp
#include <type_traits>

#include "msr_common.h"
#include "msr_internal.h"
#include "msr_frag.h"
#include "msr_gemm_dev.h"

namespace {


__global__ __launch_bounds__(256) void unit_bf16_rows_kernel(const float* __restrict__ src, const float* __restrict__ inv_norm,
                                                              int64_t n_rows, int64_t n_pad, bf16x8* __restrict__ dst,
                                                              uint32_t* __restrict__ err_max) {
    const int lane = threadIdx.x & 63;
    const int64_t wave = (int64_t)blockIdx.x * 4 + (threadIdx.x >> 6), n_waves = (int64_t)gridDim.x * 4;
    float worst = 0.f;
    for (int64_t r = wave; r < n_pad; r += n_waves) {
        float ss = 0.f;
#pragma unroll
        for (int h = 0; h < 2; ++h) {
            const int c = lane + 64 * h;
            if (c >= MSR_DIM / 8) continue;
            bf16x8 v;
            if (r < n_rows) {
                const float sc = inv_norm ? inv_norm[r] : 1.0f;
                const f32x4 x = ((const f32x4*)(src + (size_t)r * MSR_DIM))[2 * c], y = ((const f32x4*)(src + (size_t)r * MSR_DIM))[2 * c + 1];
                const float u[8] = {x.x * sc, x.y * sc, x.z * sc, x.w * sc, y.x * sc, y.y * sc, y.z * sc, y.w * sc};
#pragma unroll
                for (int j = 0; j < 8; ++j) {
                    v[j] = (__bf16)u[j];
                    const float d = (float)v[j] - u[j];
                    ss += d * d;
                }
            } else {
#pragma unroll
                for (int j = 0; j < 8; ++j) v[j] = (__bf16)0.f;
            }
            dst[(size_t)r * (MSR_DIM / 8) + c] = v;
        }
        for (int o = 32; o > 0; o >>= 1) ss += __shfl_xor(ss, o);
        worst = fmaxf(worst, ss);
    }
    if (lane == 0 && err_max) atomicMax(err_max, __float_as_uint(sqrtf(worst)));
}

__global__ __launch_bounds__(256) void batch_margin_kernel(const float* __restrict__ qn, int nq, const uint32_t* __restrict__ err_max,
                                                            float* __restrict__ margin) {
    const int q = blockIdx.x * 4 + (threadIdx.x >> 6), lane = threadIdx.x & 63;
    if (q >= nq) return;
    float ss = 0.f;
    for (int j = lane; j < MSR_DIM; j += 64) {
        const float x = qn[(size_t)q * MSR_DIM + j];
        const float d = (float)(__bf16)x - x;
        ss += d * d;
    }
    for (int o = 32; o > 0; o >>= 1) ss += __shfl_xor(ss, o);
    if (lane == 0) {
        const float dq = sqrtf(ss) * 1.0001f, dE = __uint_as_float(*err_max) * 1.0001f;
        margin[q] = 2.0f * (dE * (1.0f + dq) + dq * 1.000001f) + 1.0e-4f;
    }
}

template <int PARTS>
__global__ __launch_bounds__(256) void gemm_tmax_kernel(const float* __restrict__ in, int n_j, int parts, int nq_pad,
                                                         float* __restrict__ out, int out_stride) {
    __shared__ __attribute__((aligned(16))) float t[32][132];
    const int j0 = blockIdx.x * 32, q0 = blockIdx.y * 128;
    const int tx = threadIdx.x & 31, ty = threadIdx.x >> 5;
    const float ninf = -__builtin_inff();
    const size_t step = (size_t)nq_pad / 4;
#pragma unroll
    for (int h = 0; h < 2; ++h) {
        const f32x4* src[2];
#pragma unroll
        for (int r = 0; r < 2; ++r) {
            const int j = j0 + ty + 8 * (2 * h + r);
            const int jc = j < n_j ? j : n_j - 1;
            src[r] = (const f32x4*)(in + (size_t)jc * parts * nq_pad + q0) + tx;
        }
        f32x4 v[2] = {{ninf, ninf, ninf, ninf}, {ninf, ninf, ninf, ninf}};
        if constexpr (PARTS > 0) {
            f32x4 x[2][PARTS];
#pragma unroll
            for (int r = 0; r < 2; ++r)
#pragma unroll
                for (int p = 0; p < PARTS; ++p) x[r][p] = src[r][p * step];
#pragma unroll
            for (int r = 0; r < 2; ++r)
#pragma unroll
                for (int p = 0; p < PARTS; ++p) {
                    v[r].x = fmaxf(v[r].x, x[r][p].x); v[r].y = fmaxf(v[r].y, x[r][p].y);
                    v[r].z = fmaxf(v[r].z, x[r][p].z); v[r].w = fmaxf(v[r].w, x[r][p].w);
                }
        } else {
            for (int p = 0; p < parts; ++p) {
#pragma unroll
                for (int r = 0; r < 2; ++r) {
                    const f32x4 x = src[r][p * step];
                    v[r].x = fmaxf(v[r].x, x.x); v[r].y = fmaxf(v[r].y, x.y); v[r].z = fmaxf(v[r].z, x.z); v[r].w = fmaxf(v[r].w, x.w);
                }
            }
        }
#pragma unroll
        for (int r = 0; r < 2; ++r) *(f32x4*)&t[ty + 8 * (2 * h + r)][4 * tx] = v[r];
    }
    __syncthreads();
    const int j = j0 + tx;
    if (j < n_j) {
#pragma unroll
        for (int r = 0; r < 4; ++r) {
            const int ql = 4 * (ty + 8 * r);
            const f32x4 v = *(const f32x4*)&t[tx][ql];
            float* o = out + (size_t)(q0 + ql) * out_stride + j;
            o[0] = v.x; o[(size_t)out_stride] = v.y; o[2 * (size_t)out_stride] = v.z; o[3 * (size_t)out_stride] = v.w;
        }
    }
}

__global__ __launch_bounds__(1024) void gemm_kth_kernel(const float* __restrict__ tmax, int n, int stride, int nq, int k,
                                                         const float* __restrict__ margin, float* __restrict__ thr,
                                                         int32_t* __restrict__ flag, float short_val, float margin_scale,
                                                         int raise) {
    __shared__ uint32_t hist[2048];
    __shared__ uint32_t wsum[16];
    __shared__ uint32_t s_bin, s_kk, s_hit;
    const int q = blockIdx.x, t = threadIdx.x, lane = t & 63, wave = t >> 6;
    if (q >= nq) {
        if (t == 0 && !raise) { thr[q] = short_val; if (flag) flag[q] = 0; }
        return;
    }
    const float* row = tmax + (size_t)q * stride;
    uint32_t prefix = 0, mask = 0, kk = (uint32_t)k;
    bool short_row = false;
#pragma unroll 1
    for (int pass = 0; pass < 3; ++pass) {
        const int shift = pass == 0 ? 21 : pass == 1 ? 10 : 0;
        const uint32_t nb = pass == 2 ? 1024u : 2048u;
        hist[t] = 0; hist[t + 1024] = 0;
        if (t == 0) s_hit = 0;
        __syncthreads();
        for (int i = t; i < n; i += 1024) {
            const float x = row[i];
            if (!msr_valid(x)) continue;
            const uint32_t key = msr_ord32(x);
            if ((key & mask) == prefix) atomicAdd(&hist[(key >> shift) & (nb - 1)], 1u);
        }
        __syncthreads();
        const uint32_t h0 = 2 * t < (int)nb ? hist[2 * t] : 0u, h1 = 2 * t + 1 < (int)nb ? hist[2 * t + 1] : 0u;
        const uint32_t c2 = h0 + h1;
        uint32_t inc = c2;
#pragma unroll
        for (int o = 1; o < 64; o <<= 1) {
            const uint32_t v = __shfl_down(inc, o);
            if (lane + o < 64) inc += v;
        }
        if (lane == 0) wsum[wave] = inc;
        __syncthreads();
        uint32_t above = inc - c2;
        for (int w2 = wave + 1; w2 < 16; ++w2) above += wsum[w2];
        if (above < kk && kk <= above + c2) {
            if (above + h1 >= kk) { s_bin = 2 * t + 1; s_kk = kk - above; }
            else { s_bin = 2 * t; s_kk = kk - above - h1; }
            s_hit = 1;
        }
        __syncthreads();
        if (!s_hit) { short_row = true; break; }
        prefix |= s_bin << shift;
        mask |= (nb - 1) << shift;
        kk = s_kk;
        __syncthreads();
    }
    if (t == 0) {
        const float v = short_row ? short_val : msr_unord32(prefix) - (margin ? margin_scale * margin[q] : 0.0f);
        if (raise) {
            if (!short_row && v > thr[q]) thr[q] = v;
        } else {
            thr[q] = v;
            if (flag) flag[q] = short_row ? 1 : 0;
        }
    }
}


__global__ __launch_bounds__(256) void gemm_bucket_kernel(const int4* __restrict__ wgbuf, int wg_cap,
                                                           const int32_t* __restrict__ wg_count,
                                                           const float* __restrict__ thr2, int2* __restrict__ pairs,
                                                           int pair_cap, int32_t* __restrict__ pair_n) {
    const int wg = blockIdx.y;
    int n = wg_count[wg];
    if (n > wg_cap) n = wg_cap;
    for (int i = blockIdx.x * 256 + threadIdx.x; i < n; i += gridDim.x * 256) {
        const int4 e = wgbuf[(size_t)wg * wg_cap + i];
        if (__int_as_float(e.z) >= thr2[e.y]) {
            const int pos = atomicAdd(&pair_n[e.y], 1);
            if (pos < pair_cap) pairs[(size_t)e.y * pair_cap + pos] = make_int2(e.x, e.z);
        }
    }
}

__global__ __launch_bounds__(256) void gemm_entry_tmax_kernel(const int4* __restrict__ wgbuf, int wg_cap,
                                                               const int32_t* __restrict__ wg_count,
                                                               float* __restrict__ tmax, int stride, int tile_lo, int n_tiles,
                                                               int nq_pad) {
    const int wg = blockIdx.x;
    int n = wg_count[wg];
    if (n > wg_cap) n = wg_cap;
    for (int i = threadIdx.x; i < n; i += 256) {
        const int4 e = wgbuf[(size_t)wg * wg_cap + i];
        if ((unsigned)e.y >= (unsigned)nq_pad || e.w < tile_lo || e.w >= n_tiles) continue;
        float* p = tmax + (size_t)e.y * stride + e.w;
        if (e.z >= 0) atomicMax((int*)p, e.z);
        else atomicMin((unsigned int*)p, (unsigned int)e.z);
    }
}
__global__ __launch_bounds__(256) void gemm_fill_kernel(f32x4* __restrict__ dst, size_t n4, float v) {
    const size_t i = (size_t)blockIdx.x * 256 + threadIdx.x;
    if (i < n4) dst[i] = (f32x4){v, v, v, v};
}

constexpr int GM_PAIR_CAP = 4096;
static_assert(GM_PAIR_CAP <= (1 << 13), "cand_first_len packs first and len into 13 bits each");
__global__ __launch_bounds__(1024) void gemm_cand_kernel(int2* __restrict__ pairs, int32_t* __restrict__ pair_n,
                                                          const int32_t* __restrict__ chunk_doc, int64_t n_rows,
                                                          const int32_t* __restrict__ wg_count, int n_wg, int wg_cap,
                                                          const int32_t* __restrict__ flag, int k,
                                                          const float* __restrict__ margin,
                                                          int32_t* __restrict__ cand_doc, int32_t* __restrict__ cand_first_len,
                                                          int32_t* __restrict__ cand_n) {
    __shared__ uint64_t key[GM_PAIR_CAP];
    __shared__ uint32_t pay[GM_PAIR_CAP];
    __shared__ int s_heads, s_over;
    const int q = blockIdx.x, t = threadIdx.x;
    const int raw = pair_n[q];
    int over = raw > GM_PAIR_CAP || (flag && flag[q]);
    for (int i = t; i < n_wg; i += 1024) over |= wg_count[i] > wg_cap;
    if (t == 0) s_heads = 0;
    s_over = 0;
    __syncthreads();
    if (over) s_over = 1;
    __syncthreads();
    if (s_over) {
        if (t == 0) { cand_n[q] = MSR_SEL_CAP + 1; pair_n[q] = 0; }
        return;
    }
    int P = 64;
    while (P < raw) P <<= 1;
    auto sort_desc = [&]() {
        for (int kk = 2; kk <= P; kk <<= 1)
            for (int j = kk >> 1; j > 0; j >>= 1) {
                for (int idx = t; idx < (P >> 1); idx += 1024) {
                    const int i = ((idx & ~(j - 1)) << 1) | (idx & (j - 1));
                    const int p = i | j;
                    const bool desc = (i & kk) == 0;
                    const uint64_t x = key[i], y = key[p];
                    if (desc ? x < y : x > y) {
                        key[i] = y; key[p] = x;
                        const uint32_t v = pay[i]; pay[i] = pay[p]; pay[p] = v;
                    }
                }
                __syncthreads();
            }
    };
    for (int i = t; i < P; i += 1024) {
        uint64_t kk = 0;
        uint32_t row = 0;
        if (i < raw) {
            const int2 e = pairs[(size_t)q * GM_PAIR_CAP + i];
            if (e.x >= 0 && e.x < n_rows) {
                kk = ((uint64_t)(uint32_t)(chunk_doc[e.x] + 1) << 32) | msr_ord32(__int_as_float(e.y));
                row = (uint32_t)e.x;
            }
        }
        key[i] = kk; pay[i] = row;
    }
    __syncthreads();
    sort_desc();
    uint64_t mine[GM_PAIR_CAP / 1024];
    uint32_t mine_run[GM_PAIR_CAP / 1024];
#pragma unroll
    for (int u = 0; u < GM_PAIR_CAP / 1024; ++u) {
        const int i = t + u * 1024;
        uint64_t kk = 0;
        uint32_t run = 0;
        if (i < P && key[i] != 0) {
            pairs[(size_t)q * GM_PAIR_CAP + i].x = (int32_t)pay[i];
            const uint32_t d = (uint32_t)(key[i] >> 32);
            if (i == 0 || (uint32_t)(key[i - 1] >> 32) != d) {
                kk = ((uint64_t)(uint32_t)key[i] << 32) | (uint32_t)~(uint32_t)(d - 1);
                int len = 1;
                while (i + len < P && (uint32_t)(key[i + len] >> 32) == d) ++len;
                run = (uint32_t)i | ((uint32_t)len << 13);
            }
        }
        mine[u] = kk; mine_run[u] = run;
    }
    __syncthreads();
#pragma unroll
    for (int u = 0; u < GM_PAIR_CAP / 1024; ++u) {
        const int i = t + u * 1024;
        if (i < P) {
            key[i] = mine[u]; pay[i] = mine_run[u];
            if (mine[u]) atomicAdd(&s_heads, 1);
        }
    }
    __syncthreads();
    sort_desc();
    const int heads = s_heads;
    const float tk = heads >= k ? msr_unord32((uint32_t)(key[k - 1] >> 32)) : -__builtin_inff();
    const float cut = tk - margin[q];
    __shared__ int s_keep;
    if (t == 0) s_keep = 0;
    __syncthreads();
    for (int i = t; i < heads; i += 1024)
        if (msr_unord32((uint32_t)(key[i] >> 32)) >= cut) {
            atomicAdd(&s_keep, 1);
            if (i < MSR_SEL_CAP) {
                cand_doc[(size_t)q * MSR_SEL_CAP + i] = (int32_t)~(uint32_t)key[i];
                cand_first_len[(size_t)q * MSR_SEL_CAP + i] = (int32_t)pay[i];
            }
        }
    __syncthreads();
    if (t == 0) { cand_n[q] = s_keep; pair_n[q] = 0; }
}

int g_gemm_dbg = 0;

}

hipError_t msr_unit_bf16_rows(const float* src, const float* inv_norm, int64_t n_rows, int64_t n_pad, void* dst,
                              uint32_t* err_max, hipStream_t stream) {
    if (n_pad <= 0) return hipSuccess;
    hipError_t err = err_max ? hipMemsetAsync(err_max, 0, 4, stream) : hipSuccess;
    if (err != hipSuccess) return err;
    unit_bf16_rows_kernel<<<8192, 256, 0, stream>>>(src, inv_norm, n_rows, n_pad, (bf16x8*)dst, err_max);
    return hipGetLastError();
}

hipError_t msr_batch_margin(const float* qn, int nq, const uint32_t* err_max, float* margin, hipStream_t stream) {
    if (nq <= 0) return hipSuccess;
    batch_margin_kernel<<<(nq + 3) / 4, 256, 0, stream>>>(qn, nq, err_max, margin);
    return hipGetLastError();
}

int msr_gemm_pair_cap() { return GM_PAIR_CAP; }

hipError_t msr_gemm_tmax(const float* tmax_t, int n_j, int parts, int nq_pad, float* out, int out_stride, hipStream_t stream) {
    if (n_j <= 0 || nq_pad <= 0) return hipSuccess;
    if (parts <= 0 || nq_pad % 128 != 0) return hipErrorInvalidValue;
    const dim3 grid((n_j + 31) / 32, nq_pad / 128);
    if (parts == 8) gemm_tmax_kernel<8><<<grid, 256, 0, stream>>>(tmax_t, n_j, parts, nq_pad, out, out_stride);
    else if (parts == 1) gemm_tmax_kernel<1><<<grid, 256, 0, stream>>>(tmax_t, n_j, parts, nq_pad, out, out_stride);
    else gemm_tmax_kernel<0><<<grid, 256, 0, stream>>>(tmax_t, n_j, parts, nq_pad, out, out_stride);
    return hipGetLastError();
}
hipError_t msr_gemm_kth(const float* tmax, int n, int stride, int nq, int nq_pad, int k, const float* margin, float* thr,
                        int32_t* flag, hipStream_t stream, float short_val, float margin_scale, bool raise) {
    if (nq_pad <= 0) return hipSuccess;
    gemm_kth_kernel<<<nq_pad, 1024, 0, stream>>>(tmax, n, stride, nq, k, margin, thr, raise ? nullptr : flag, short_val, margin_scale,
                                                 raise ? 1 : 0);
    return hipGetLastError();
}
hipError_t msr_gemm_bucket(const void* wvbuf, int wv_cap, const int32_t* wv_count, int n_waves, const float* thr2,
                           void* pairs, int32_t* pair_n, hipStream_t stream) {
    gemm_bucket_kernel<<<dim3(2, (unsigned)n_waves), 256, 0, stream>>>((const int4*)wvbuf, wv_cap, wv_count, thr2, (int2*)pairs,
                                                                      GM_PAIR_CAP, pair_n);
    return hipGetLastError();
}
hipError_t msr_gemm_tmax_clear(float* tmax, int stride, int nq_pad, hipStream_t stream) {
    const size_t n4 = (size_t)nq_pad * stride / 4;
    if (n4 == 0) return hipSuccess;
    if (stride % 4 != 0) return hipErrorInvalidValue;
    gemm_fill_kernel<<<(unsigned)((n4 + 255) / 256), 256, 0, stream>>>((f32x4*)tmax, n4, -__builtin_inff());
    return hipGetLastError();
}
hipError_t msr_gemm_entry_tmax(const void* wvbuf, int wv_cap, const int32_t* wv_count, int n_waves, float* tmax, int stride,
                               int tile_lo, int n_tiles, int nq_pad, hipStream_t stream) {
    if (tile_lo < 0 || n_tiles > stride) return hipErrorInvalidValue;
    gemm_entry_tmax_kernel<<<(unsigned)n_waves, 256, 0, stream>>>((const int4*)wvbuf, wv_cap, wv_count, tmax, stride, tile_lo,
                                                                 n_tiles, nq_pad);
    return hipGetLastError();
}
void msr_gemm_set_dbg(int v) { g_gemm_dbg = v; }

hipError_t msr_gemm_candidates(const GemmIndex& g, const DenseIndex& ix, const float* qn, int nq, int k, const float* margin,
                               int32_t* cand_doc, int32_t* cand_first_len, int32_t* cand_n, hipEvent_t* ev, hipStream_t stream) {
    const int nq_pad = (nq + 255) / 256 * 256;
    const int nt = nq_pad / 256;
    if (nq <= 0 || nq_pad > g.max_queries || k < 1 || g.n_tiles < 2 * k) return hipErrorInvalidValue;
    const int grid = g.n_cus / 8 * 8;
    if (grid < 8 || grid / 8 < nt) return hipErrorInvalidValue;
    hipError_t err;
    int ss = g.n_tiles / (8 * k);
    ss = ss < 1 ? 1 : (ss > 16 ? 16 : ss);
#ifdef MSR_DIAG
    if (g_gemm_dbg & 256) ss = 1;
#endif
    const int n_s = (g.n_tiles - ss / 2 + ss - 1) / ss;
    {
        if ((err = msr_stream256_bf16_qimage(qn, nq, nt, g.qmat, stream)) != hipSuccess) return err;
        StreamArgs a{};
        a.E = (const char*)g.emb_n; a.inv_pad = nullptr; a.qimg = (const char*)g.qmat; a.tile_row = g.tile_row;
        a.n_rows = ix.n_chunks; a.tmax_t = g.tmax_t; a.nt = nt; a.q_base = 0; a.append = 0;
        a.t_first = ss / 2; a.t_stride = ss; a.t_count = n_s;
        if (ev && (err = hipEventRecord(ev[0], stream)) != hipSuccess) return err;
        if ((err = msr_stream256_bf16_launch(false, a, grid, stream)) != hipSuccess) return err;
        if (ev && (err = hipEventRecord(ev[1], stream)) != hipSuccess) return err;
        if ((err = msr_gemm_tmax(g.tmax_t, n_s, 1, nq_pad, (float*)g.tmax, g.tmax_stride, stream)) != hipSuccess) return err;
        gemm_kth_kernel<<<nq_pad, 1024, 0, stream>>>((const float*)g.tmax, n_s, g.tmax_stride, nq, k, margin, g.thr, g.flag, __builtin_inff(), 1.0f, 0);
        a.t_first = 0; a.t_stride = 1; a.t_count = g.n_tiles;
        a.thr = g.thr; a.wvbuf = g.wgbuf; a.wv_cap = g.wv_cap; a.wv_count = g.wv_count;
        if (ev && (err = hipEventRecord(ev[2], stream)) != hipSuccess) return err;
        if ((err = msr_stream256_bf16_launch(true, a, grid, stream)) != hipSuccess) return err;
        if (ev && (err = hipEventRecord(ev[3], stream)) != hipSuccess) return err;
        if ((err = msr_gemm_tmax(g.tmax_t, g.n_tiles, 1, nq_pad, (float*)g.tmax, g.tmax_stride, stream)) != hipSuccess) return err;
        gemm_kth_kernel<<<nq_pad, 1024, 0, stream>>>((const float*)g.tmax, g.n_tiles, g.tmax_stride, nq, k, margin, g.thr2, nullptr, __builtin_inff(), 1.0f, 0);
    }
    gemm_bucket_kernel<<<dim3(2, (unsigned)grid * 8), 256, 0, stream>>>((const int4*)g.wgbuf, g.wv_cap, g.wv_count, g.thr2,
                                                                       (int2*)g.pairs, GM_PAIR_CAP, g.pair_n);
    gemm_cand_kernel<<<nq, 1024, 0, stream>>>((int2*)g.pairs, g.pair_n, ix.chunk_doc, ix.n_chunks, g.wv_count, grid * 8, g.wv_cap,
                                              g.flag, k, margin, cand_doc, cand_first_len, cand_n);
    return hipGetLastError();
}
```

### modern-search-engines-project_amd/csrc/msr_gemm_f32.hip

```cpp
#include <cmath>
#include <type_traits>

#include "msr_common.h"
#include "msr_internal.h"
#include "msr_frag.h"
#include "msr_gemm_dev.h"

namespace {

constexpr int GF_THREADS = 512;
constexpr int GF_KT = MSR_DIM / 32;
constexpr int GF_ROWB = MSR_DIM * 4;
constexpr int GF_PAIR_CAP = 4096;

typedef StreamArgs GemmF32Args;

__device__ __forceinline__ const char* uniform_ptr(const char* p) {
    const uint64_t u = (uint64_t)p;
    const uint32_t lo = __builtin_amdgcn_readfirstlane((uint32_t)u), hi = __builtin_amdgcn_readfirstlane((uint32_t)(u >> 32));
    return (const char*)(((uint64_t)hi << 32) | lo);
}

constexpr int GS_NB = 8;
constexpr int GS_STEP = 8192;
// ... 399 lines not shown
    };
    constexpr int NKB = GF_KT / G2_NB;
    constexpr int BLKB = TILED ? RSLOTS * 2048 : RSLOTS * 128;
    stage_b(0, 0);
#pragma unroll
    for (int s = 0; s < RSLOTS; ++s)
#pragma unroll
        for (int mi = 0; mi < NMI; ++mi) ring[s][mi][0] = ring[s][mi][1] = (f32x4){0.f, 0.f, 0.f, 0.f};
    load_rows(std::integral_constant<int, 0>{}, bp, vp, std::integral_constant<int, 0>{});
    load_rows(std::integral_constant<int, 1>{}, bp, vp, std::integral_constant<int, 128>{});
    if (!BF16) {
        load_rows(std::integral_constant<int, RSLOTS - 2>{}, bp, vp, std::integral_constant<int, 256>{});
        load_rows(std::integral_constant<int, RSLOTS - 1>{}, bp, vp, std::integral_constant<int, 384>{});
    }
    wait_vm0();
    pin_rows(std::integral_constant<int, 0>{}); pin_rows(std::integral_constant<int, 1>{});
    pin_rows(std::integral_constant<int, RSLOTS - 2>{}); pin_rows(std::integral_constant<int, RSLOTS - 1>{});
    wg_barrier();
    int pb = 0;

    const float NEG_INF = -__builtin_inff();
    f16x8 bh[4];
#pragma unroll
    for (int i = 0; i < 4; ++i)
#pragma unroll
        for (int j = 0; j < 8; ++j) bh[i][j] = (_Float16)0.f;
    auto step = [&](auto s4_c, int kn, bool last) {
        constexpr int s4 = decltype(s4_c)::value;
        constexpr int slot = s4 / KPS, half = s4 % KPS;
        using SL = std::integral_constant<int, slot>;
        __builtin_amdgcn_sched_barrier(0);
#ifdef MSR_DIAG
        if (a.dbg & 32768) __builtin_amdgcn_s_setprio(3);
#endif
        if (half == 0) {
            if (BF16) asm volatile("s_waitcnt vmcnt(12)" ::: "memory");
            else asm volatile("s_waitcnt vmcnt(20)" ::: "memory");
            pin_rows(SL{});
        }
        f16x8 af[NMI];
#pragma unroll
        for (int mi = 0; mi < NMI; ++mi)
            af[mi] = BF16 ? take16(ring[slot][mi][half]) : cvt_f16_rtn(ring[slot][mi][0], ring[slot][mi][1]);
#pragma unroll
        for (int mi = 0; mi < NMI; ++mi) asm volatile("" :: "v"(af[mi]));
        if ((!BF16 || F16I) && s4 == 1 && last) {
            const char* src = uniform_ptr((const char*)(a.inv_pad + (size_t)row0 + w * 32));
            __builtin_amdgcn_global_load_lds((glb_void*)(src + (uint32_t)(fresh_lane() * 4)), (lds_void*)inv_lds, 4, 0, 0);
        }
        if (half == KPS - 1) {
#ifdef MSR_DIAG
            if (!(a.dbg & 262144))
#endif
            {
            if (last) load_rows(SL{}, bn, vn, std::integral_constant<int, slot * 128>{});
            else load_rows(SL{}, bp + (uint64_t)(kn * BLKB), vp, std::integral_constant<int, slot * 128>{});
            }
        }
#ifdef MSR_DIAG
        if (a.dbg & 32768) __builtin_amdgcn_s_setprio(0);
#endif
        __builtin_amdgcn_sched_barrier(0);
        const uint32_t ln = fresh_lane();
        const uint32_t fo = (ln & 15) * 64 + (((ln >> 4) ^ (((ln >> 3) & 1) << 1)) << 4);
        const char* bq = smem + pb * G2_BLK + s4 * G2_STEP + wc * (128 * 64) + fo;
        if (!BF16) {
#ifdef MSR_DIAG
            if (a.dbg & 8) return;
#endif
#pragma unroll
            for (int n4 = 0; n4 < NNI / 4; ++n4) {
                f16x8 b4[4];
#pragma unroll
                for (int i = 0; i < 4; ++i) b4[i] = *(const f16x8*)(bq + (4 * n4 + i) * 1024);
#ifdef MSR_DIAG
                if (a.dbg & 16) {
#pragma unroll
                    for (int i = 0; i < 4; ++i) asm volatile("" :: "v"(b4[i]));
                    continue;
                }
#endif
#pragma unroll
                for (int mi = 0; mi < NMI; ++mi)
#pragma unroll
                    for (int i = 0; i < 4; ++i)
                        acc[mi][4 * n4 + i] = __builtin_amdgcn_mfma_f32_16x16x32_f16(af[mi], b4[i], acc[mi][4 * n4 + i], 0, 0, 0);
            }
            return;
        }
        const uint32_t la = (uint32_t)(uintptr_t)(lds_char*)bq;
        if (s4 == 0) {
            lds_read16<0>(bh[0], la); lds_read16<1024>(bh[1], la); lds_read16<2048>(bh[2], la); lds_read16<3072>(bh[3], la);
        }
        auto frag = [&](auto f_c) {
            constexpr int f = decltype(f_c)::value;
            constexpr int ahead = (s4 + 1 < G2_NB) ? 3 : (NNI - 1 - f < 3 ? NNI - 1 - f : 3);
            if (ahead == 3) asm volatile("s_waitcnt lgkmcnt(3)" ::: "memory");
            else if (ahead == 2) asm volatile("s_waitcnt lgkmcnt(2)" ::: "memory");
            else if (ahead == 1) asm volatile("s_waitcnt lgkmcnt(1)" ::: "memory");
            else asm volatile("s_waitcnt lgkmcnt(0)" ::: "memory");
            asm volatile("" : "+v"(bh[f & 3]));
#pragma unroll
            for (int mi = 0; mi < NMI; ++mi)
                acc[mi][f] = F16I ? __builtin_amdgcn_mfma_f32_16x16x32_f16(af[mi], bh[f & 3], acc[mi][f], 0, 0, 0)
                                  : __builtin_amdgcn_mfma_f32_16x16x32_bf16(
                    __builtin_bit_cast(bf16x8, af[mi]), __builtin_bit_cast(bf16x8, bh[f & 3]), acc[mi][f], 0, 0, 0);
            if (f + 4 < NNI) lds_read16<(f + 4) * 1024>(bh[f & 3], la);
            else if (s4 + 1 < G2_NB) lds_read16<G2_STEP + (f + 4 - NNI) * 1024>(bh[f & 3], la);
        };
        frag(std::integral_constant<int, 0>{}); frag(std::integral_constant<int, 1>{});
        frag(std::integral_constant<int, 2>{}); frag(std::integral_constant<int, 3>{});
        frag(std::integral_constant<int, 4>{}); frag(std::integral_constant<int, 5>{});
        frag(std::integral_constant<int, 6>{}); frag(std::integral_constant<int, 7>{});
        frag(std::integral_constant<int, 8>{}); frag(std::integral_constant<int, 9>{});
        frag(std::integral_constant<int, 10>{}); frag(std::integral_constant<int, 11>{});
        frag(std::integral_constant<int, 12>{}); frag(std::integral_constant<int, 13>{});
        frag(std::integral_constant<int, 14>{}); frag(std::integral_constant<int, 15>{});
    };
    int jt_prev = jt;
    for (int it = 0; it < n_mine; ++it) {
#pragma unroll 1
        for (int kb = 0; kb < NKB; ++kb) {
            const bool last = kb == NKB - 1;
            const int kn = last ? 0 : kb + 1;
#ifdef MSR_DIAG
            if (!(a.dbg & 524288))
#endif
            stage_b(kn, pb ^ 1);
            step(std::integral_constant<int, 0>{}, kn, last);
            step(std::integral_constant<int, 1>{}, kn, last);
            step(std::integral_constant<int, 2>{}, kn, last);
            step(std::integral_constant<int, 3>{}, kn, last);
            if (BF16) asm volatile("s_waitcnt vmcnt(8)" ::: "memory");
            else asm volatile("s_waitcnt vmcnt(16)" ::: "memory");
#ifdef MSR_DIAG
            if (!(a.dbg & 131072))
#endif
            wg_barrier();
            pb ^= 1;
            if (JOIN && kb == 0 && it > 0) flush_tmax(jt_prev, (it - 1) & 1);
        }
        const int ln_e = (int)fresh_lane();
        const int lg_e = ln_e >> 4;
        f32x4 inv4[NMI];
        if (!BF16 || F16I) {
            if (F16I) asm volatile("s_waitcnt vmcnt(8)" ::: "memory");
            else asm volatile("s_waitcnt vmcnt(12)" ::: "memory");
#pragma unroll
            for (int mi = 0; mi < NMI; ++mi) inv4[mi] = *(const f32x4*)(inv_lds + mi * 16 + 4 * lg_e);
        }
        const int n_valid = row_end - row0;
        const int col_e = wc * 128 + (ln_e & 15);
        float thr_nx = (EMIT && !THR_REGS) ? thr_lds[col_e] : 0.f;
#ifdef MSR_DIAG
        if (a.dbg & 65536) {
#pragma unroll
            for (int ni = 0; ni < NNI; ++ni)
#pragma unroll
                for (int mi = 0; mi < NMI; ++mi) acc[mi][ni] = (f32x4){0.f, 0.f, 0.f, 0.f};
        } else
#endif
#pragma unroll
        for (int ni = 0; ni < NNI; ++ni) {
            f32x4 v[NMI];
            float cmax = NEG_INF;
            const float thr_cur = thr_nx;
            if (EMIT && !THR_REGS && ni + 1 < NNI) thr_nx = thr_lds[(ni + 1) * 16 + col_e];
#pragma unroll
            for (int mi = 0; mi < NMI; ++mi) {
                const int blk = wr * WROWS + mi * 16;
                if (BF16 && !F16I) v[mi] = acc[mi][ni];
                else v[mi] = acc[mi][ni] * inv4[mi];
                if (blk + 16 > n_valid) {
#pragma unroll
                    for (int rr = 0; rr < 4; ++rr)
                        if (blk + 4 * lg_e + rr >= n_valid) v[mi][rr] = NEG_INF;
                }
                cmax = max2_raw(cmax, max3_raw(max2_raw(v[mi][0], v[mi][1]), v[mi][2], v[mi][3]));
                acc[mi][ni] = (f32x4){0.f, 0.f, 0.f, 0.f};
            }
            if (EMIT) {
                float thr;
                if (THR_REGS) thr = (float)__builtin_bit_cast(_Float16, (uint16_t)(ni & 1 ? thr_h[ni >> 1] >> 16 : thr_h[ni >> 1] & 0xffffu));
                else thr = thr_cur;
                if (__ballot(cmax >= thr) != 0) {
                    const int q = q_base + ni * 16 + col_e;
#pragma unroll
                    for (int mi = 0; mi < NMI; ++mi) {
                        const int rb = wr * WROWS + mi * 16 + 4 * lg_e;
#pragma unroll
                        for (int rr = 0; rr < 4; ++rr) {
                            const float x = v[mi][rr];
                            const bool hit = x >= thr;
                            const unsigned long long hm = __ballot(hit);
                            if (hm != 0) {
                                const int pos = wave_cnt + (int)__builtin_amdgcn_mbcnt_hi((uint32_t)(hm >> 32), __builtin_amdgcn_mbcnt_lo((uint32_t)hm, 0u));
                                if (hit && pos < a.wv_cap)
                                    wvbuf[pos] = make_int4(row0 + rb + rr, q, __float_as_int(x), tile_of(jt));
                                wave_cnt += __popcll(hm);
                            }
                        }
                    }
                }
            }
            if (TMAX) {
                float m = cmax;
                auto s32 = __builtin_amdgcn_permlane32_swap(__float_as_uint(m), __float_as_uint(m), false, false);
                m = max2_raw(__uint_as_float(s32[0]), __uint_as_float(s32[1]));
                auto s16 = __builtin_amdgcn_permlane16_swap(__float_as_uint(m), __float_as_uint(m), false, false);
                m = max2_raw(__uint_as_float(s16[0]), __uint_as_float(s16[1]));
                if (JOIN) {
                    if (lg_e == 0) atomicMax(tmx + (it & 1) * 256 + ni * 16 + col_e, ord_key(m));
                } else {
                    if (lg_e == 0) a.tmax_t[((size_t)jt * 8 + w) * nq_pad + grp * 256 + ni * 16 + col_e] = m;
                }
            }
        }
        jt_prev = jt;
        jt = jn;
        row0 = row0n;
        row_end = a.tile_row[tile_of(jt) + 1];
        jn = jt + G < a.t_count ? jt + G : jt;
        row0n = a.tile_row[tile_of(jn)];
        bp = bn; bn = tile_base(TILED ? a.tile_trow[tile_of(jn)] : row0n);
#pragma unroll
        for (int mi = 0; mi < NV; ++mi) { vp[mi] = vn[mi]; vn[mi] = row_off(row0n, mi); }
    }
    wait_vm0();
    if (JOIN) {
        wg_barrier();
        flush_tmax(jt_prev, (n_mine - 1) & 1);
    }
    if (EMIT && lane == 0) a.wv_count[blockIdx.x * 8 + w] = wave_cnt;
}

template <bool BF16, bool TOBF16 = BF16>
__global__ __launch_bounds__(256) void build_qimg2_kernel(const float* __restrict__ qn, int nq, f16x8* __restrict__ qimg) {
    const int i = blockIdx.x * 256 + threadIdx.x;
    if (i >= GF_KT * 256 * 4) return;
    const int g = blockIdx.y;
    const int cp = i & 3, ql = (i >> 2) & 255, kt = i >> 10;
    const int q = 256 * g + ql;
    const int c = cp ^ (((ql >> 3) & 1) << 1);
    f16x8 h;
    if (q < nq) {
        const float* src = qn + (size_t)q * MSR_DIM + (BF16 ? 64 * (kt >> 1) + 16 * c + 8 * (kt & 1) : 32 * kt + 8 * c);
        if (TOBF16) {
            bf16x8 b;
#pragma unroll
            for (int j = 0; j < 8; ++j) b[j] = (__bf16)src[j];
            h = __builtin_bit_cast(f16x8, b);
        } else {
            h = cvt_f16_rtn(*(const f32x4*)src, *(const f32x4*)(src + 4));
        }
    } else {
#pragma unroll
        for (int j = 0; j < 8; ++j) h[j] = (_Float16)0.f;
    }
    qimg[(size_t)g * (GF_KT * 256 * 4) + i] = h;
}

__global__ __launch_bounds__(256) void build_qimg1_kernel(const float* __restrict__ qn, int nq, f16x8* __restrict__ qimg) {
    const int i = blockIdx.x * 256 + threadIdx.x;
    if (i >= GF_KT * 128 * 4) return;
    const int g = blockIdx.y;
    const int cp = i & 3, ql = (i >> 2) & 127, kt = i >> 9;
    const int q = 128 * g + ql;
    const int c = cp ^ (((ql >> 3) & 1) << 1);
    f16x8 h;
    if (q < nq) {
        const float* src = qn + (size_t)q * MSR_DIM + 32 * kt + 8 * c;
        h = cvt_f16_rtn(*(const f32x4*)src, *(const f32x4*)(src + 4));
    } else {
#pragma unroll
        for (int j = 0; j < 8; ++j) h[j] = (_Float16)0.f;
    }
    qimg[(size_t)g * (GF_KT * 128 * 4) + i] = h;
}

__global__ __launch_bounds__(256) void pad_inv_kernel(const float* __restrict__ inv, int64_t n, int64_t n_pad, float* __restrict__ out) {
    const int64_t i = (int64_t)blockIdx.x * 256 + threadIdx.x;
    if (i < n_pad) out[i] = i < n ? inv[i] : 1.0f;
}

__global__ __launch_bounds__(256) void f16_row_error_kernel(const float* __restrict__ src, const float* __restrict__ inv_norm,
                                                             int64_t n_rows, uint32_t* __restrict__ err_max) {
    const int lane = threadIdx.x & 63;
    const int64_t wave = (int64_t)blockIdx.x * 4 + (threadIdx.x >> 6), n_waves = (int64_t)gridDim.x * 4;
    float worst = 0.f;
    for (int64_t r = wave; r < n_rows; r += n_waves) {
        const f32x4* p = (const f32x4*)(src + (size_t)r * MSR_DIM);
        float ss = 0.f;
#pragma unroll
        for (int h = 0; h < 3; ++h) {
            const f32x4 x = p[lane + 64 * h];
            ss += f16_err2(x.x) + f16_err2(x.y) + f16_err2(x.z) + f16_err2(x.w);
        }
        for (int o = 32; o > 0; o >>= 1) ss += __shfl_xor(ss, o);
        worst = fmaxf(worst, sqrtf(ss) * inv_norm[r]);
    }
    if (lane == 0) atomicMax(err_max, __float_as_uint(worst));
}

__global__ __launch_bounds__(256) void f16_margin_kernel(const float* __restrict__ qn, int nq, const uint32_t* __restrict__ err_max,
                                                          float* __restrict__ margin) {
    const int q = blockIdx.x * 4 + (threadIdx.x >> 6), lane = threadIdx.x & 63;
    if (q >= nq) return;
    float ss = 0.f;
    for (int j = lane; j < MSR_DIM; j += 64) ss += f16_err2(qn[(size_t)q * MSR_DIM + j]);
    for (int o = 32; o > 0; o >>= 1) ss += __shfl_xor(ss, o);
    if (lane == 0) {
        const float dq = sqrtf(ss) * 1.0001f, dE = __uint_as_float(*err_max) * 1.0001f;
        margin[q] = 2.0f * (dE * (1.0f + dq) + dq * 1.000001f) + 1.0e-4f;
    }
}

static_assert(GF_PAIR_CAP <= (1 << 13), "cand_first_len packs first and len into 13 bits each");
__global__ __launch_bounds__(1024) void gemm_f32_cand_kernel(int2* __restrict__ pairs, int32_t* __restrict__ pair_n,
                                                              const int32_t* __restrict__ chunk_doc, int64_t n_rows,
                                                              const int32_t* __restrict__ wv_count, int n_waves, int wv_cap,
                                                              const int32_t* __restrict__ flag, int32_t* __restrict__ cand_doc,
                                                              int32_t* __restrict__ cand_first_len,
                                                              int32_t* __restrict__ cand_n, int32_t* __restrict__ gate) {
    __shared__ uint64_t key[GF_PAIR_CAP];
    __shared__ int s_over, s_n;
    const int q = blockIdx.x, t = threadIdx.x;
    const int raw = pair_n[q];
    int over = raw > GF_PAIR_CAP || flag[q];
    for (int i = t; i < n_waves; i += 1024) over |= wv_count[i] > wv_cap;
    if (t == 0) { s_n = 0; s_over = 0; }
    __syncthreads();
    if (over) s_over = 1;
    __syncthreads();
    if (s_over) {
        if (t == 0) { cand_n[q] = 0; pair_n[q] = 0; atomicOr(gate + (q >> 6), 1); }
        return;
    }
    int P = 64;
    while (P < raw) P <<= 1;
    for (int i = t; i < P; i += 1024) {
        uint64_t kk = 0u;
        if (i < raw) {
            const int64_t row = pairs[(size_t)q * GF_PAIR_CAP + i].x;
            if (row >= 0 && row < n_rows)
                kk = ((uint64_t)((uint32_t)chunk_doc[row] + 1u) << 32) | (uint32_t)row;
        }
        key[i] = kk;
    }
    __syncthreads();
    for (int kk = 2; kk <= P; kk <<= 1)
        for (int j = kk >> 1; j > 0; j >>= 1) {
            for (int idx = t; idx < (P >> 1); idx += 1024) {
                const int i = ((idx & ~(j - 1)) << 1) | (idx & (j - 1));
                const int p = i | j;
                const bool desc = (i & kk) == 0;
                const uint64_t a = key[i], b = key[p];
                if (desc ? a < b : a > b) { key[i] = b; key[p] = a; }
            }
            __syncthreads();
        }
    for (int i = t; i < P; i += 1024) {
        const uint64_t kk = key[i];
        if (kk == 0) continue;
        pairs[(size_t)q * GF_PAIR_CAP + i].x = (int32_t)(uint32_t)kk;
        const uint32_t d = (uint32_t)(kk >> 32);
        if (i == 0 || (uint32_t)(key[i - 1] >> 32) != d) {
            int len = 1;
            while (i + len < P && (uint32_t)(key[i + len] >> 32) == d) ++len;
            const int slot = atomicAdd(&s_n, 1);
            cand_doc[(size_t)q * MSR_SEL_CAP + slot] = (int32_t)(d - 1u);
            cand_first_len[(size_t)q * MSR_SEL_CAP + slot] = i | (len << 13);
        }
    }
    __syncthreads();
    if (t == 0) { cand_n[q] = s_n; pair_n[q] = 0; }
}

int g_f32_dbg = 0;

template <bool EMIT>
hipError_t launch_stream_t(const GemmF32Args& a, int grid, hipStream_t stream) {
    static bool attr_done = false;
    if (!attr_done) {
        hipError_t err = hipFuncSetAttribute((const void*)gemm_stream_kernel<EMIT>, hipFuncAttributeMaxDynamicSharedMemorySize, GS_LDS);
        if (err != hipSuccess) return err;
        attr_done = true;
    }
    gemm_stream_kernel<EMIT><<<grid, GF_THREADS, GS_LDS, stream>>>(a);
    return hipGetLastError();
}
template <bool EMIT, bool BF16, bool TILED = false, bool NTL = false, bool F16I = false>
hipError_t launch_stream256_t(const GemmF32Args& a, int grid, hipStream_t stream) {
    static bool attr_done = false;
    if (!attr_done) {
        hipError_t err = hipFuncSetAttribute((const void*)gemm_stream256_kernel<EMIT, BF16, TILED, NTL, F16I>, hipFuncAttributeMaxDynamicSharedMemorySize, G2_LDS);
        if (err != hipSuccess) return err;
        attr_done = true;
    }
    gemm_stream256_kernel<EMIT, BF16, TILED, NTL, F16I><<<grid, G2_THREADS, G2_LDS, stream>>>(a);
    return hipGetLastError();
}

__global__ __launch_bounds__(256) void f16_rows_kernel(const float* __restrict__ src, int64_t n_rows, int64_t n_pad,
                                                        f16x8* __restrict__ dst) {
    const int64_t n8 = n_pad * (MSR_DIM / 8), stride = (int64_t)gridDim.x * 256;
    for (int64_t i = (int64_t)blockIdx.x * 256 + threadIdx.x; i < n8; i += stride) {
        const int64_t r = i / (MSR_DIM / 8);
        f16x8 h;
        if (r < n_rows) {
            const float* p = src + i * 8;
            h = cvt_f16_rtn(*(const f32x4*)p, *(const f32x4*)(p + 4));
        } else {
#pragma unroll
            for (int j = 0; j < 8; ++j) h[j] = (_Float16)0.f;
        }
        dst[i] = h;
    }
}

template <int ROWB>
__global__ __launch_bounds__(256) void tile_rows_kernel(const char* __restrict__ E, const int32_t* __restrict__ tile_row,
                                                         const int32_t* __restrict__ tile_trow, f32x4* __restrict__ Et) {
    constexpr int SLOTS = ROWB / 128;
    const int t_ = blockIdx.x;
    const int row0 = tile_row[t_], n = tile_row[t_ + 1] - row0;
    const int groups = (n + 15) >> 4;
    f32x4* dst = Et + (size_t)tile_trow[t_] * (ROWB / 16);
    const int pieces = groups * SLOTS * 128;
    for (int i = threadIdx.x; i < pieces; i += 256) {
        const int lane = i & 63, half = (i >> 6) & 1, sl = (i >> 7) % SLOTS, g = i / (128 * SLOTS);
        const int lr = 16 * g + (lane & 15);
        f32x4 v = {0.f, 0.f, 0.f, 0.f};
        if (lr < n) v = *(const f32x4*)(E + (size_t)(row0 + lr) * ROWB + 128 * sl + 32 * (lane >> 4) + 16 * half);
        dst[i] = v;
    }
}
hipError_t launch_f32(int width, bool emit, const GemmF32Args& a, int grid, hipStream_t stream, bool tiled = false,
                      bool image16 = false) {
    if (image16)
        return emit ? launch_stream256_t<true, true, false, false, true>(a, grid, stream)
                    : launch_stream256_t<false, true, false, false, true>(a, grid, stream);
    bool ntl = width == 256 && tiled && a.nt == 1;
#ifdef MSR_DIAG
    if (g_f32_dbg & 16384) ntl = false;
#endif
    if (ntl)
        return emit ? launch_stream256_t<true, false, true, true>(a, grid, stream) : launch_stream256_t<false, false, true, true>(a, grid, stream);
    if (width == 256 && tiled)
        return emit ? launch_stream256_t<true, false, true>(a, grid, stream) : launch_stream256_t<false, false, true>(a, grid, stream);
    if (width == 256) return emit ? launch_stream256_t<true, false>(a, grid, stream) : launch_stream256_t<false, false>(a, grid, stream);
    return emit ? launch_stream_t<true>(a, grid, stream) : launch_stream_t<false>(a, grid, stream);
}

}

void msr_gemm_f32_set_dbg(int v) { g_f32_dbg = v; }

hipError_t msr_stream256_bf16_launch(bool emit, const StreamArgs& a, int grid, hipStream_t stream) {
    if (a.nt < 1 || (grid & 7) || (grid >> 3) < a.nt) return hipErrorInvalidValue;
#ifdef MSR_DIAG
    if (g_f32_dbg & (32768 | 65536 | 131072 | 262144 | 524288)) { StreamArgs b = a; b.dbg |= g_f32_dbg & (32768 | 65536 | 131072 | 262144 | 524288); return emit ? launch_stream256_t<true, true>(b, grid, stream) : launch_stream256_t<false, true>(b, grid, stream); }
#endif
    return emit ? launch_stream256_t<true, true>(a, grid, stream) : launch_stream256_t<false, true>(a, grid, stream);
}
hipError_t msr_stream256_bf16_qimage(const float* qn, int nq, int n_groups, void* qimg, hipStream_t stream) {
    build_qimg2_kernel<true><<<dim3((GF_KT * 256 * 4 + 255) / 256, n_groups), 256, 0, stream>>>(qn, nq, (f16x8*)qimg);
    return hipGetLastError();
}

hipError_t msr_tile_rows(const float* emb, const int32_t* tile_row, const int32_t* tile_trow, int n_tiles, void* emb_tiled,
                         hipStream_t stream) {
    if (n_tiles <= 0) return hipSuccess;
    tile_rows_kernel<MSR_DIM * 4><<<n_tiles, 256, 0, stream>>>((const char*)emb, tile_row, tile_trow, (f32x4*)emb_tiled);
    return hipGetLastError();
}


hipError_t msr_f16_rows(const float* emb, int64_t n_rows, int64_t n_pad, void* out, hipStream_t stream) {
    if (n_pad <= 0) return hipSuccess;
    f16_rows_kernel<<<8192, 256, 0, stream>>>(emb, n_rows, n_pad, (f16x8*)out);
    return hipGetLastError();
}

hipError_t msr_pad_inv_norm(const float* inv, int64_t n, int64_t n_pad, float* out, hipStream_t stream) {
    if (n_pad <= 0) return hipSuccess;
    pad_inv_kernel<<<(unsigned)((n_pad + 255) / 256), 256, 0, stream>>>(inv, n, n_pad, out);
    return hipGetLastError();
}

hipError_t msr_f16_row_error(const float* emb, const float* inv_norm, int64_t n_rows, uint32_t* err_max, hipStream_t stream) {
    hipError_t err = hipMemsetAsync(err_max, 0, 4, stream);
    if (err != hipSuccess) return err;
    f16_row_error_kernel<<<8192, 256, 0, stream>>>(emb, inv_norm, n_rows, err_max);
    return hipGetLastError();
}

namespace {
struct PassShape {
    int ss, n_s;
    int n_seg;
    int bound[4];
};
PassShape pass_shape(int T, int k, int grid, bool single, int dbg) {
    PassShape p{};
    int ss = T / (3 * k);
    ss = ss < 1 ? 1 : (ss > 64 ? 64 : ss);
    p.ss = ss;
    p.n_s = (T - ss / 2 + ss - 1) / ss;
    p.n_seg = 1; p.bound[0] = 0; p.bound[1] = T;
    if (single) return p;
    (void)dbg;
#ifdef MSR_DIAG
    if ((dbg & 16777216) && grid >= 2 * k && p.n_s > grid) {
        p.n_s = p.n_s / grid * grid;
        p.ss = T / p.n_s;
    }
#endif
    const double root = std::sqrt((double)T * (double)p.n_s);
    int want3 = 0;
#ifdef MSR_DIAG
    want3 = dbg & 2097152;
#endif
    if (want3) {
        const double r = std::cbrt((double)T / (double)p.n_s);
        const int m1 = (int)std::floor(p.n_s * r / grid + 0.5), m2 = (int)std::floor(p.n_s * r * r / grid + 0.5);
        const int64_t t1 = (int64_t)m1 * grid, t2 = (int64_t)m2 * grid;
        if (m1 >= 1 && m2 > m1 && t1 >= 2 * k && T - t2 >= grid) {
            p.n_seg = 3; p.bound[1] = (int)t1; p.bound[2] = (int)t2; p.bound[3] = T;
            return p;
        }
    }
    int64_t t1 = (int64_t)std::floor(root / grid + 0.5) * grid;
#ifdef MSR_DIAG
    if (dbg & 4194304) t1 = std::max<int64_t>(grid, t1 / 2 / grid * grid);
    if (dbg & 8388608) t1 = 2 * t1;
#endif
    if (t1 >= std::max(grid, 2 * k) && T - t1 >= grid) {
        p.n_seg = 2; p.bound[1] = (int)t1; p.bound[2] = T;
    }
    return p;
}

}

hipError_t msr_gemm_f32_pass(const GemmF32Index& g, const DenseIndex& ix, const float* qn, int nq, int k, int k_part,
                             float* out_part, hipEvent_t* ev, int* width_out, int* seg_out, hipStream_t stream) {
    const int W = nq > 128 ? 256 : 128;
    const int waves = 8;
    const int G = (nq + W - 1) / W;
    if (nq <= 0 || G * W > 128 * g.max_groups || k < 1 || g.n_tiles < 2 * k) return hipErrorInvalidValue;
    if (width_out) *width_out = W;
    hipError_t err;
    int NT0 = 1;
    if (W == 256 && (g.n_cus & 7) == 0) NT0 = std::min(std::min(G, g.max_nt), g.n_cus >> 3);
    bool image16 = W == 256 && NT0 > 1 && g.emb_f16 != nullptr;
#ifdef MSR_DIAG
    if (g_f32_dbg & (2048 | 1048576)) image16 = false;
#endif
    if (image16) build_qimg2_kernel<true, false><<<dim3((GF_KT * 256 * 4 + 255) / 256, G), 256, 0, stream>>>(qn, nq, (f16x8*)g.qimg);
    else if (W == 256) build_qimg2_kernel<false><<<dim3((GF_KT * 256 * 4 + 255) / 256, G), 256, 0, stream>>>(qn, nq, (f16x8*)g.qimg);
    else build_qimg1_kernel<<<dim3((GF_KT * 128 * 4 + 255) / 256, G), 256, 0, stream>>>(qn, nq, (f16x8*)g.qimg);
    f16_margin_kernel<<<(nq + 3) / 4, 256, 0, stream>>>(qn, nq, g.err_max, g.margin);
    const float* margin = g.margin;
    const int grid = g.n_cus;
    const PassShape shape = pass_shape(g.n_tiles, k, grid, g.single_emit != 0, g_f32_dbg);
    const int ss = shape.ss, n_s = shape.n_s;
    if (seg_out) *seg_out = shape.n_seg;
    const size_t qimg_bytes = (size_t)GF_KT * W * 64;
    int NT = 1;
    if (W == 256 && (grid & 7) == 0) NT = std::min(std::min(G, g.max_nt), grid >> 3);
#ifdef MSR_DIAG
    if (g_f32_dbg & 2048) NT = 1;
    if (g_f32_dbg & 4096) NT = std::min(NT, 2);
#endif
    GemmF32Args a{};
    a.dbg = g_f32_dbg; a.nt = 1;
    a.E = (const char*)ix.emb; a.inv_pad = g.inv_pad; a.tile_row = g.tile_row;
    bool tiled = W == 256 && g.emb_tiled != nullptr && !image16;
#ifdef MSR_DIAG
    if (g_f32_dbg & 8192) tiled = false;
#endif
    if (tiled) { a.E = (const char*)g.emb_tiled; a.tile_trow = g.tile_trow; }
    if (image16) a.E = (const char*)g.emb_f16;
    const int tmax_parts = image16 ? 1 : waves;
    a.n_rows = ix.n_chunks; a.tmax_t = g.tmax_t;
    a.t_first = ss / 2; a.t_stride = ss; a.t_count = n_s;
    for (int gi = 0; gi < G; gi += NT) {
        a.nt = std::min(NT, G - gi);
        a.qimg = (const char*)g.qimg + gi * qimg_bytes;
        if (ev && gi == 0 && (err = hipEventRecord(ev[0], stream)) != hipSuccess) return err;
        if ((err = launch_f32(W, false, a, grid, stream, tiled, image16)) != hipSuccess) return err;
        if (ev && gi == 0 && (err = hipEventRecord(ev[1], stream)) != hipSuccess) return err;
        if ((err = msr_gemm_tmax(g.tmax_t, n_s, tmax_parts, W * a.nt, g.tmax + (size_t)gi * W * g.tmax_stride, g.tmax_stride, stream)) != hipSuccess) return err;
    }
    if ((err = msr_gemm_kth(g.tmax, n_s, g.tmax_stride, nq, W * G, k, margin, g.thr, g.flag, stream)) != hipSuccess) return err;
    bool entry_tmax = W == 256 && !image16;
#ifdef MSR_DIAG
    if (g_f32_dbg & 33554432) entry_tmax = false;
#endif
    if (entry_tmax && (err = msr_gemm_tmax_clear(g.tmax, g.tmax_stride, W * G, stream)) != hipSuccess) return err;
    a.t_stride = 1;
    a.wvbuf = g.wvbuf; a.wv_cap = g.wv_cap * (8 / waves); a.wv_count = g.wv_count;
    for (int s = 0; s < shape.n_seg; ++s) {
        const int t0 = shape.bound[s], t1 = shape.bound[s + 1];
        a.t_first = t0; a.t_count = t1 - t0;
        for (int gi = 0; gi < G; gi += NT) {
            a.nt = std::min(NT, G - gi);
            a.qimg = (const char*)g.qimg + gi * qimg_bytes;
            a.thr = g.thr + gi * W; a.q_base = gi * W; a.append = (s > 0 || gi > 0);
            if (ev && gi == 0 && s == 0 && (err = hipEventRecord(ev[2], stream)) != hipSuccess) return err;
            if ((err = launch_f32(W, true, a, grid, stream, tiled, image16)) != hipSuccess) return err;
            if (ev && gi == 0 && s == shape.n_seg - 1 && (err = hipEventRecord(ev[3], stream)) != hipSuccess) return err;
            if (!entry_tmax &&
                (err = msr_gemm_tmax(g.tmax_t, t1 - t0, tmax_parts, W * a.nt, g.tmax + (size_t)gi * W * g.tmax_stride + t0, g.tmax_stride, stream)) != hipSuccess) return err;
        }
        if (entry_tmax && (err = msr_gemm_entry_tmax(g.wvbuf, a.wv_cap, g.wv_count, grid * waves, g.tmax, g.tmax_stride, t0,
                                                     g.n_tiles, W * G, stream)) != hipSuccess) return err;
        if (s + 1 < shape.n_seg &&
            (err = msr_gemm_kth(g.tmax, t1, g.tmax_stride, nq, W * G, k, margin, g.thr, nullptr, stream, __builtin_inff(), 1.0f, true)) != hipSuccess)
            return err;
    }
    if ((err = msr_gemm_kth(g.tmax, g.n_tiles, g.tmax_stride, nq, W * G, k, margin, g.thr2, nullptr, stream)) != hipSuccess) return err;
    if (out_part && (err = msr_gemm_kth(g.tmax, g.n_tiles, g.tmax_stride, nq, nq, k_part, margin, out_part, nullptr, stream,
                                        -__builtin_inff(), 0.5f)) != hipSuccess) return err;
    return hipSuccess;
}

namespace {
__global__ __launch_bounds__(256) void raise_thr_kernel(float* __restrict__ thr2, const float* __restrict__ bound,
                                                         const float* __restrict__ margin, int nq) {
    const int q = blockIdx.x * 256 + threadIdx.x;
    if (q >= nq) return;
    const float b = bound[q] - 0.5f * margin[q];
    if (b > thr2[q]) thr2[q] = b;
}
}

hipError_t msr_gemm_f32_finish(const GemmF32Index& g, const DenseIndex& ix, const float* qn, int nq, int k, const float* bound,
                               int32_t* out_doc, float* out_score, int32_t* out_chunk, int32_t* out_n, int32_t* gate,
                               hipStream_t stream) {
    const int waves = 8, grid = g.n_cus;
    const int wv_cap = g.wv_cap * (8 / waves);
    if (nq <= 0 || k < 1) return hipErrorInvalidValue;
    hipError_t err;
    if (bound) {
        raise_thr_kernel<<<(nq + 255) / 256, 256, 0, stream>>>(g.thr2, bound, g.margin, nq);
        if ((err = hipGetLastError()) != hipSuccess) return err;
    }
    if ((err = msr_gemm_bucket(g.wvbuf, wv_cap, g.wv_count, grid * waves, g.thr2, g.pairs, g.pair_n, stream)) != hipSuccess) return err;
    gemm_f32_cand_kernel<<<nq, 1024, 0, stream>>>((int2*)g.pairs, g.pair_n, ix.chunk_doc, ix.n_chunks, g.wv_count, grid * waves,
                                                  wv_cap, g.flag, g.cand_doc, g.cand_chunk, g.cand_n, gate);
    if ((err = hipGetLastError()) != hipSuccess) return err;
    return msr_batch_rescore_rows(ix, qn, nq, k, (const int32_t*)g.pairs, 2, GF_PAIR_CAP, g.cand_doc, g.cand_score, g.cand_chunk,
                                  g.cand_n, out_doc, out_score, out_chunk, out_n, stream);
}

hipError_t msr_gemm_f32_topk(const GemmF32Index& g, const DenseIndex& ix, const float* qn, int nq, int k,
                             int32_t* out_doc, float* out_score, int32_t* out_chunk,
                             int32_t* out_n, int32_t* gate, hipEvent_t* ev, int* width_out, int* seg_out, hipStream_t stream) {
    hipError_t err = msr_gemm_f32_pass(g, ix, qn, nq, k, k, nullptr, ev, width_out, seg_out, stream);
    if (err != hipSuccess) return err;
    return msr_gemm_f32_finish(g, ix, qn, nq, k, nullptr, out_doc, out_score, out_chunk, out_n, gate, stream);
}
```

### modern-search-engines-project_amd/csrc/msr_internal.h

```cpp
#pragma once
#include <hip/hip_runtime.h>
#include <stdint.h>

#define MSR_DIM 768
#define MSR_SEL_BINS 4096
#define MSR_SEL_CAP 4096

struct SelState {
    uint64_t pref_hi, mask_hi;
    uint32_t pref_lo, mask_lo;
    int32_t k_rem;
    int32_t n_above;
    int32_t done;
    int32_t n_sel;
};

struct SelScratch {
    uint32_t* hist;
    SelState* state;
    uint64_t* cand_hi;
    uint32_t* cand_lo;
    int32_t* cand_n;
    const int32_t* gate;
    int gate_per64;
};

struct MsrSetView {
    const uint32_t* bits;
    int64_t stride;
    const int32_t* q_set;
    int32_t n_sets;
};
struct MsrSetRow {
    const uint32_t* bits;
    int32_t mode;
};
__device__ __forceinline__ MsrSetRow msr_set_row(int q, const MsrSetView& s) {
    const int32_t v = s.q_set[q];
    if (v == -1) return MsrSetRow{nullptr, 0};
    if (v < -1 || v >= s.n_sets) return MsrSetRow{nullptr, 2};
    return MsrSetRow{s.bits + (int64_t)v * s.stride, 1};
}
__device__ __forceinline__ bool msr_in_set(const MsrSetRow& r, int64_t d) {
    return r.mode == 0 || (r.mode == 1 && ((r.bits[d >> 5] >> (d & 31)) & 1u));
}

hipError_t msr_select_topk(int score_bits, const void* scores, int64_t n, int64_t stride, int nq, int k,
                           const SelScratch& sc, int32_t* out_doc, void* out_score, int32_t* out_n,
                           hipStream_t stream);
hipError_t msr_select_topk_within(const float* scores, int64_t n, int64_t stride, int nq, int k, const SelScratch& sc,
                                  const MsrSetView& set, int32_t* out_doc, float* out_score, int32_t* out_n, hipStream_t stream);

hipError_t msr_select_topk_list(const double* scores, const int32_t* idx, const int32_t* counts, int n_seg, int64_t seg_stride,
                                int64_t stride, int nq, int k, const SelScratch& sc, int32_t* out_doc,
                                double* out_score, int32_t* out_n, hipStream_t stream, const uint64_t* win_base = nullptr);

hipError_t msr_merge_lists(int score_bits, const int32_t* in_doc, const void* in_score, const int32_t* in_n,
                           const int32_t* in_pay, int n_parts, int64_t part_stride_bytes, int nq, int k, int32_t* out_doc,
                           void* out_score, int32_t* out_n, int32_t* out_pay, hipStream_t stream);

int msr_fail_global(int code, const char* fmt, ...);

constexpr int MSR_SCAN_BLOCK = 4096;
hipError_t exclusive_scan(const int64_t* in, int64_t n, int64_t* out, int64_t* tmp, int64_t* total, hipStream_t st);
inline int64_t exclusive_scan_tmp_words(int64_t n) {
    if (n <= 0) return 0;
    const int64_t nb = (n + MSR_SCAN_BLOCK - 1) / MSR_SCAN_BLOCK, nb2 = (nb + MSR_SCAN_BLOCK - 1) / MSR_SCAN_BLOCK;
    return 2 * nb + 2 * nb2;
}

struct Bm25Post {
    int32_t doc;
    uint32_t comp_lo, comp_hi;
};
struct Bm25Index {
    const int64_t* term_off;
    const int32_t* post_doc;
    const int32_t* post_tf;
    const int32_t* doc_len;
    const float* idf;
    int64_t n_terms, n_postings, n_docs;
    double avgdl, k1, b;
    const int32_t* heavy_id;
    const uint32_t* tile_off;
    int32_t n_tiles;
    const Bm25Post* post;
    const int32_t* dense_id;
    const double* dense_comp;
    int64_t dense_stride;
};
hipError_t msr_bm25_dnorm(const int32_t* doc_len, int64_t n_docs, int64_t n_pad, double k1, double b, double avgdl, double* out,
                          hipStream_t stream);
hipError_t msr_bm25_post_comp(const int32_t* post_doc, const int32_t* post_tf, const double* dnorm, double k1, int64_t n,
                              Bm25Post* out, hipStream_t stream);
hipError_t msr_bm25_build_dense(const Bm25Index& ix, const int32_t* dense_terms, int n_dense, double* dense_comp,
                                int64_t dense_stride, hipStream_t stream);
constexpr int MSR_BM25_TILE = 1024;
constexpr int MSR_BM25_HEAVY_DF = 2048;
constexpr int MSR_BM25_MAX_DENSE = 64;
hipError_t msr_bm25_build_skip(const Bm25Index& ix, const int32_t* heavy_terms, int n_heavy, uint32_t* tile_off,
                               hipStream_t stream);
int msr_bm25_max_segments(int64_t n_docs);
hipError_t msr_bm25_window(const Bm25Index& ix, const int32_t* q_term_off, const int32_t* q_terms, const int32_t* q_qtf,
                           int q_first, int nq, uint64_t* out , hipStream_t stream);
void msr_bm25_split(int n_tiles, int nq, int* tpw, int* n_spans);
hipError_t msr_bm25_scores(const Bm25Index& ix, const int32_t* q_term_off, const int32_t* q_terms,
                           const int32_t* q_qtf, int q_first, int nq, double min_score, double* cand_score,
                           int32_t* cand_doc, int32_t* seg_n, int* n_seg, int64_t* seg_stride, hipStream_t stream,
                           const MsrSetView* set = nullptr);

hipError_t msr_bm25_point(const Bm25Index& ix, const int32_t* q_term_off, const int32_t* q_terms, const int32_t* q_qtf, int nq,
                          const int32_t* doc, const int32_t* doc_n, int max_docs, double* out_score, int32_t* out_touched,
                          hipStream_t stream);
hipError_t msr_union_lists(int nq, const int32_t* lex_doc, const double* lex_score, const int32_t* lex_n, int k_lex,
                           const int32_t* dense_doc, const double* dense_bm25, const int32_t* dense_n, int k_dense,
                           int32_t* out_doc, double* out_score, int32_t* out_src, int32_t* out_n, int max_cand,
                           hipStream_t stream);

hipError_t msr_term_sets_run(const Bm25Index& ix, int n_rows, const int32_t* must_off, const int32_t* must_terms,
                             const int32_t* not_off, const int32_t* not_terms, const uint32_t* base_bits, int n_base,
                             int64_t base_stride, const int32_t* row_base, uint32_t* out_bits, int64_t out_stride,
                             hipStream_t stream);

hipError_t msr_tokens_validate(const int64_t* tok_off, const int32_t* tok_ids, int64_t n_docs, int64_t n_tokens, int64_t n_terms,
                               int32_t* flag, hipStream_t stream);
hipError_t msr_phrase_sets_run(const int64_t* tok_off, const int32_t* tok_ids, int64_t n_docs, int64_t n_terms, int n_rows,
                               const int32_t* phrase_off, const int32_t* phrase_terms, const uint32_t* cand_bits, int n_cand,
                               int64_t cand_stride, const int32_t* row_cand, uint32_t* out_bits, int64_t out_stride,
                               hipStream_t stream);
hipError_t msr_proximity_sets_run(const int64_t* tok_off, const int32_t* tok_ids, int64_t n_docs, int64_t n_terms, int n_rows,
                                  const int32_t* phrase_off, const int32_t* phrase_terms, const int32_t* row_span,
                                  const int32_t* row_ordered, const uint32_t* cand_bits, int n_cand, int64_t cand_stride,
                                  const int32_t* row_cand, uint32_t* out_bits, int64_t out_stride, hipStream_t stream);
hipError_t msr_best_windows_run(const int64_t* tok_off, const int32_t* tok_ids, int64_t n_docs, int64_t n_terms, int n_pairs,
                                const int32_t* pair_doc, const int32_t* pair_row, int n_rows, const int32_t* row_off,
                                const int32_t* row_terms, const int32_t* row_weights, const int32_t* row_span, int32_t* out_start,
                                int32_t* out_cover, int32_t* out_hits, uint64_t* out_mask, uint32_t* out_terms,
                                hipStream_t stream);
hipError_t msr_vocab_validate(const int64_t* char_off, const uint32_t* weight, int64_t n_terms, int64_t n_chars, int32_t* flag,
                              hipStream_t stream);
hipError_t msr_vocab_signatures(const int64_t* char_off, const uint16_t* chars, int64_t n_terms, uint64_t* sig,
                                hipStream_t stream);
int64_t msr_fuzzy_spans(int64_t n_terms);
hipError_t msr_fuzzy_terms_run(const int64_t* char_off, const uint16_t* chars, const uint32_t* weight, const uint64_t* sig,
                               int64_t n_terms, int n_words, const int32_t* word_off, const uint16_t* word_chars,
                               const int32_t* word_max, int limit, int32_t* out_term, int32_t* out_dist, int32_t* out_n,
                               int32_t* out_total, void* scratch, hipStream_t stream);
hipError_t msr_wildcard_terms_run(const int64_t* char_off, const uint16_t* chars, const uint32_t* weight, const uint64_t* sig,
                                  int64_t n_terms, int n_patterns, const int32_t* pat_off, const uint16_t* pat_chars, int limit,
                                  int32_t* out_term, int32_t* out_n, int32_t* out_total, void* scratch, hipStream_t stream);
struct FacetTable {
    const uint16_t* local;
    const int32_t* span_off;
    const int32_t* span_values;
    const int32_t* value_off;
    const int32_t* value_pos;
    int32_t n_values;
    int64_t n_entries;
};
hipError_t msr_facet_validate(const FacetTable& f, int64_t n_docs, int32_t* flag, hipStream_t stream);
int64_t msr_facet_row_bytes(const FacetTable& f, int64_t n_docs);
hipError_t msr_facet_counts_run(const Bm25Index& ix, const FacetTable& f, int n_rows, const int32_t* any_off,
                                const int32_t* any_terms, const uint32_t* base_bits, int n_base, int64_t base_stride,
                                const int32_t* row_base, int limit, int32_t* out_hits, int32_t* out_n_values_hit,
                                int32_t* out_top_value, int32_t* out_top_count, int32_t* out_counts, int64_t count_stride,
                                void* scratch, hipStream_t stream);
hipError_t msr_combine_sets_run(int64_t n_docs, int n_rows, const int32_t* and_off, const int32_t* and_rows,
                                const int32_t* not_off, const int32_t* not_rows, const uint32_t* in_bits, int n_in,
                                int64_t in_stride, uint32_t* out_bits, int64_t out_stride, hipStream_t stream);

hipError_t msr_bm25_validate(const Bm25Index& ix, int32_t* flag, hipStream_t stream);

constexpr int MSR_WIDE_RING = 128;
struct DenseIndex {
    const float* emb;
    const int32_t* doc_off;
    const int32_t* chunk_doc;
    const float* inv_norm;
    const int32_t* span_doc;
    int64_t n_chunks, n_docs;
    int64_t score_stride;
    int32_t n_spans;
    int32_t layout;
    const int32_t* wspan_doc;
    int32_t n_wspans;
    const int32_t* wspan12_doc;
    int32_t n_wspans12;
    void* qimg;
    const void* emb_bf16;
    const void* emb_presplit;
    const void* row_meta;
    int32_t wide_ok;
    int32_t wide_ok64;
    const int32_t* gate;
    int32_t variant;
    int32_t gate_per64;
};
hipError_t msr_dense_scan(const DenseIndex& ix, const float* qn, int nq, int max_chunks, float* docscore,
                          hipStream_t stream);
hipError_t msr_dense_scan_bf16(const DenseIndex& ix, const float* qn, int nq, int max_chunks, float* docscore,
                               hipStream_t stream);
hipError_t msr_dense_scan_wide(const DenseIndex& ix, const float* qn, int nq, float* docscore, hipStream_t stream);
size_t msr_ksplit_slice_image_bytes();
hipError_t msr_dense_scan_slices(const DenseIndex& ix, const float* qn, int nq, float* docscore, void* qimg_slices,
                                 hipStream_t stream);
hipError_t msr_dense_scan_wide_exact(const DenseIndex& ix, const float* qn, int nq, float* docscore, hipStream_t stream);
hipError_t msr_dense_scan_bf16_wide(const DenseIndex& ix, const float* qn, int nq, float* docscore,
                                    hipStream_t stream);
hipError_t msr_build_qimage(int mode, const float* qn, int n_blocks, void* qimg, hipStream_t stream);
hipError_t msr_presplit_rows(const float* src, int64_t n_rows, void* dst, hipStream_t stream);
hipError_t msr_pack_row_meta(const int32_t* chunk_doc, const float* inv_norm, int64_t n, void* row_meta, hipStream_t stream);
hipError_t msr_fill_f32(float* dst, int64_t n, float value, hipStream_t stream);
hipError_t msr_inv_norm_range(const float* inv_norm, int64_t n, uint32_t* out2, hipStream_t stream);
hipError_t msr_prep_queries(const float* q, int nq, float* qn, int nq_pad, hipStream_t stream);
hipError_t msr_fill_chunk_doc(const int32_t* doc_off, int64_t n_docs, int32_t* chunk_doc, hipStream_t stream);
hipError_t msr_row_inv_norm(const float* emb, int64_t n_rows, float* inv_norm, hipStream_t stream);
hipError_t msr_interleave(const float* src, int64_t n_rows, float* dst, hipStream_t stream);
hipError_t msr_best_chunk(const DenseIndex& ix, const float* qn, int nq, int k, int max_chunks,
                          const int32_t* out_doc, const int32_t* out_n, int32_t* out_chunk, hipStream_t stream);

hipError_t msr_check_range(const int32_t* v, int64_t n, int64_t hi, int32_t* flag, hipStream_t stream);
hipError_t msr_gather_rows_run(const DenseIndex& ix, const int32_t* rows, int n, float* out, hipStream_t stream);
hipError_t msr_group_row_sets(const int32_t* group_off, int n_groups, const int32_t* g_set, int32_t* row_set, hipStream_t stream);
struct GroupedMergeArgs {
    const int32_t* l_doc; const float* l_score; const int32_t* l_chunk; const int32_t* l_n;
    int32_t kk;
    const int32_t* group_off;
    const int32_t* excl_off;
    const int32_t* excl_doc;
    int32_t k;
    float min_score;
    int32_t* out_doc; float* out_score; int32_t* out_chunk; int32_t* out_src; int32_t* out_n;
    uint64_t* g_hi; uint32_t* g_lo; uint32_t* g_val;
};
hipError_t msr_grouped_merge(const GroupedMergeArgs& a, int n_groups, hipStream_t stream);

struct RerankParams {
    double smoothing, max_boost, max_decay;
    int32_t max_chunks;
};
#define MSR_RERANK_RECORD_WORDS 16
struct RerankRecords {
    int32_t* out;
    const int32_t* q_base;
    const int32_t* blk_off;
    int64_t capacity;
    int q_first;
};
hipError_t msr_rerank_gather(const DenseIndex& ix, const int32_t* url_group, const float* qn, int nq,
                             const int32_t* cand_doc, const int32_t* cand_n, int max_cand, int doc_base,
                             int row_base, int max_chunks, float* cos_out ,
                             int32_t* meta , int q_per_block, int64_t block_stride,
                             const RerankRecords& rec, hipStream_t stream);
hipError_t msr_rerank_plan_run(int nq, const int32_t* cand_doc, const int32_t* cand_n, int max_cand, const int32_t* bounds,
                               int n_shards, int my, int qps, int32_t* counts, int32_t* send_base, int32_t* blk_off,
                               int32_t* recv_off, int32_t* pair, hipStream_t stream);
hipError_t msr_rerank_scatter_run(const int32_t* records, int64_t capacity, const int32_t* counts, const int32_t* recv_off, int n_shards, int nq,
                                  int qps, int q_first, int n_mine, int max_cand, float* cos_out, int32_t* meta_out,
                                  hipStream_t stream);
hipError_t msr_rerank_fuse_run(int nq, const int32_t* cand_doc, const double* cand_bm25, const int32_t* cand_n,
                               int max_cand, const RerankParams& p, const float* cos_in, const int32_t* meta,
                               int32_t* out_doc, double* out_score, double* out_orig, int32_t* out_chunk,
                               int32_t* out_n, int32_t* out_rows, hipStream_t stream);

hipError_t msr_diversify_run(int nq, const int32_t* f_doc, const double* f_score, const double* f_orig, const int32_t* f_chunk,
                             const int32_t* f_n, int max_cand, const int32_t* doc_domain, int64_t n_domain_docs, int top_k,
                             double threshold, int diversify, int32_t* out_doc, double* out_score, double* out_orig,
                             int32_t* out_chunk, int32_t* out_n, hipStream_t stream);

hipError_t msr_or_parts(const void* in, int n_parts, int64_t part_stride_bytes, int64_t n_words, void* out, hipStream_t stream);

struct GemmIndex {
    const void* emb_n;
    const int32_t* tile_row;
    int32_t n_tiles;
    int32_t n_cus;
    int32_t max_queries;
    void* qmat;
    float* tmax;
    int32_t tmax_stride;
    float* tmax_t;
    float* thr; float* thr2;
    int32_t* flag;
    void* wgbuf;
    int32_t wv_cap;
    int32_t* wv_count;
    void* pairs;
    int32_t* pair_n;
};
int msr_gemm_pair_cap();
hipError_t msr_gemm_tmax(const float* tmax_t, int n_j, int parts, int nq_pad, float* out, int out_stride, hipStream_t stream);
hipError_t msr_gemm_kth(const float* tmax, int n, int stride, int nq, int nq_pad, int k, const float* margin, float* thr,
                        int32_t* flag, hipStream_t stream, float short_val = __builtin_inff(), float margin_scale = 1.0f,
                        bool raise = false);
hipError_t msr_gemm_bucket(const void* wvbuf, int wv_cap, const int32_t* wv_count, int n_waves, const float* thr2,
                           void* pairs, int32_t* pair_n, hipStream_t stream);
hipError_t msr_gemm_tmax_clear(float* tmax, int stride, int nq_pad, hipStream_t stream);
hipError_t msr_gemm_entry_tmax(const void* wvbuf, int wv_cap, const int32_t* wv_count, int n_waves, float* tmax, int stride,
                               int tile_lo, int n_tiles, int nq_pad, hipStream_t stream);
void msr_bm25_set_dbg(int v);
void msr_gemm_set_dbg(int v);
hipError_t msr_unit_bf16_rows(const float* src, const float* inv_norm, int64_t n_rows, int64_t n_pad, void* dst,
                              uint32_t* err_max, hipStream_t stream);
hipError_t msr_batch_margin(const float* qn, int nq, const uint32_t* err_max, float* margin, hipStream_t stream);
hipError_t msr_gemm_candidates(const GemmIndex& g, const DenseIndex& ix, const float* qn, int nq, int k, const float* margin,
                               int32_t* cand_doc, int32_t* cand_first_len, int32_t* cand_n, hipEvent_t* ev,
                               hipStream_t stream);

constexpr int MSR_STREAM256_TILE_ROWS = 256;

struct StreamArgs {
    const char* E;
    const float* inv_pad;
    const char* qimg;
    const int32_t* tile_row;
    const int32_t* tile_trow;
    int64_t n_rows;
    int t_first, t_stride, t_count;
    float* tmax_t;
    const float* thr;
    void* wvbuf; int wv_cap; int32_t* wv_count;
    int q_base;
    int append;
    int nt;
    int dbg;
};
hipError_t msr_stream256_bf16_launch(bool emit, const StreamArgs& a, int grid, hipStream_t stream);
hipError_t msr_stream256_bf16_qimage(const float* qn, int nq, int n_groups, void* qimg, hipStream_t stream);

struct GemmF32Index {
    const int32_t* tile_row;
    int32_t n_tiles;
    int32_t n_cus;
    int32_t max_groups;
    const float* inv_pad;
    void* qimg;
    float* tmax_t;
    float* tmax;
    int32_t tmax_stride;
    float* thr; float* thr2; int32_t* flag;
    void* wvbuf; int32_t wv_cap; int32_t* wv_count;
    void* pairs; int32_t* pair_n;
    uint32_t* err_max; float* margin;
    int32_t* cand_doc; float* cand_score; int32_t* cand_chunk; int32_t* cand_n;
    int32_t max_nt;
    const void* emb_tiled;
    const int32_t* tile_trow;
    const void* emb_f16;
    int32_t single_emit;
};
hipError_t msr_f16_rows(const float* emb, int64_t n_rows, int64_t n_pad, void* out, hipStream_t stream);
hipError_t msr_tile_rows(const float* emb, const int32_t* tile_row, const int32_t* tile_trow, int n_tiles, void* emb_tiled,
                         hipStream_t stream);
hipError_t msr_f16_row_error(const float* emb, const float* inv_norm, int64_t n_rows, uint32_t* err_max, hipStream_t stream);
void msr_gemm_f32_set_dbg(int v);
hipError_t msr_pad_inv_norm(const float* inv, int64_t n, int64_t n_pad, float* out, hipStream_t stream);
hipError_t msr_gemm_f32_topk(const GemmF32Index& g, const DenseIndex& ix, const float* qn, int nq, int k,
                             int32_t* out_doc, float* out_score, int32_t* out_chunk,
                             int32_t* out_n, int32_t* gate, hipEvent_t* ev, int* width_out, int* seg_out, hipStream_t stream);
hipError_t msr_gemm_f32_pass(const GemmF32Index& g, const DenseIndex& ix, const float* qn, int nq, int k, int k_part,
                             float* out_part, hipEvent_t* ev, int* width_out, int* seg_out, hipStream_t stream);
hipError_t msr_gemm_f32_finish(const GemmF32Index& g, const DenseIndex& ix, const float* qn, int nq, int k, const float* bound,
                               int32_t* out_doc, float* out_score, int32_t* out_chunk, int32_t* out_n, int32_t* gate,
                               hipStream_t stream);

hipError_t msr_batch_rescore_rows(const DenseIndex& ix, const float* qn, int nq, int k, const int32_t* rows, int row_stride,
                                  int row_cap, int32_t* cand_doc, float* cand_score, int32_t* cand_chunk, int32_t* cand_n,
                                  int32_t* out_doc, float* out_score, int32_t* out_chunk, int32_t* out_n, hipStream_t stream);
hipError_t msr_batch_finish(const DenseIndex& ix, const float* qn, int nq, int k, int max_chunks, const float* margin,
                            const float* scores, const float* top_score, const int32_t* top_n, int32_t* cand_doc,
                            float* cand_score, int32_t* cand_chunk, int32_t* cand_n, int32_t* out_doc,
                            float* out_score, int32_t* out_chunk, int32_t* out_n, hipStream_t stream);
```

Before: 64000.

## Fuse query prep, gate clear and tmax clear into passes; list-based kth; LDS bucketing

Query normalisation, f16 margin computation, gate memset and tmax clearing are folded into a single prepare kernel inside the f32 pass, and tmax is cleared by the kth kernel instead of a separate launch. The kth select keeps valid keys in an LDS list after the first radix pass, so later passes skip re-reading the row. Pair bucketing switches to a per-block LDS count-then-scatter that reserves slots with one global atomic per query. These changes cut kernel launches and global atomics, in exchange for more LDS use and more complex kernels.

```diff
diff --git a/modern-search-engines-project_amd/csrc/msr_common.h b/modern-search-engines-project_amd/csrc/msr_common.h
--- a/modern-search-engines-project_amd/csrc/msr_common.h
+++ b/modern-search-engines-project_amd/csrc/msr_common.h
@@ -31,3 +31,14 @@
 
 __device__ __forceinline__ bool msr_valid(float s) { return s > -__builtin_inff(); }
 __device__ __forceinline__ bool msr_valid(double s) { return s > -__builtin_inf(); }
+
+__device__ __forceinline__ void msr_wave_normalise(float (&v)[12]) {
+#pragma clang fp contract(off)
+    float ss = v[1] * v[1];
+    ss = __builtin_fmaf(v[0], v[0], ss);
+    for (int j = 2; j < 12; ++j) ss = __builtin_fmaf(v[j], v[j], ss);
+    for (int off = 32; off > 0; off >>= 1) ss += __shfl_xor(ss, off);
+    float nrm = sqrtf(ss);
+    if (nrm == 0.f) nrm = 1.f;
+    for (int j = 0; j < 12; ++j) v[j] = v[j] / nrm;
+}
diff --git a/modern-search-engines-project_amd/csrc/msr_dense.hip b/modern-search-engines-project_amd/csrc/msr_dense.hip
--- a/modern-search-engines-project_amd/csrc/msr_dense.hip
+++ b/modern-search-engines-project_amd/csrc/msr_dense.hip
@@ -308,15 +308,9 @@
     const int lane = threadIdx.x & 63;
     if (row >= nq_pad) return;
     float v[12];
-    float ss = 0.f;
-    for (int j = 0; j < 12; ++j) {
-        v[j] = row < nq ? q[(size_t)row * MSR_DIM + lane + 64 * j] : 0.f;
-        ss += v[j] * v[j];
-    }
-    for (int off = 32; off > 0; off >>= 1) ss += __shfl_xor(ss, off);
-    float nrm = sqrtf(ss);
-    if (nrm == 0.f) nrm = 1.f;
-    for (int j = 0; j < 12; ++j) qn[(size_t)row * MSR_DIM + lane + 64 * j] = v[j] / nrm;
+    for (int j = 0; j < 12; ++j) v[j] = row < nq ? q[(size_t)row * MSR_DIM + lane + 64 * j] : 0.f;
+    msr_wave_normalise(v);
+    for (int j = 0; j < 12; ++j) qn[(size_t)row * MSR_DIM + lane + 64 * j] = v[j];
 }
 
 __global__ void fill_chunk_doc_kernel(const int32_t* __restrict__ doc_off, int64_t n_docs,
diff --git a/modern-search-engines-project_amd/csrc/msr_engine.hip b/modern-search-engines-project_amd/csrc/msr_engine.hip
--- a/modern-search-engines-project_amd/csrc/msr_engine.hip
+++ b/modern-search-engines-project_amd/csrc/msr_engine.hip
@@ -1314,13 +1314,12 @@
                     cap, n_queries, k_part, k);
     hipStream_t st = (hipStream_t)stream;
     HIP_TRY(e, hipSetDevice(e->cfg.device));
-    HIP_TRY(e, msr_prep_queries(q, n_queries, e->gf_qn, (n_queries + 63) / 64 * 64, st));
-    HIP_TRY(e, hipMemsetAsync(e->gf_gate, 0, GF_GATE_BYTES, st));
     hipEvent_t ev_buf[4];
     hipEvent_t* ev = pass_events(e, 0, ev_buf);
     int width = 0;
     int segs = 0;
-    HIP_TRY(e, msr_gemm_f32_pass(e->gf, e->dense, e->gf_qn, n_queries, k, k_part, out_part, ev, &width, &segs, st));
+    HIP_TRY(e, msr_gemm_f32_pass(e->gf, e->dense, q, e->gf_qn, n_queries, k, k_part, out_part, e->gf_gate, (int)(GF_GATE_BYTES / 4), ev,
+                                 &width, &segs, st));
     e->last_dense_width = width;
     e->last_dense_segments = segs;
     pass_events_used(e, 0, ev);
@@ -1397,14 +1396,12 @@
         const int left = n_queries - q0;
         if (gemm && left > 64) {
             const int nq = std::min(dense_stream_cap(e), left);
-            HIP_TRY(e, msr_prep_queries(q + (int64_t)q0 * MSR_DIM, nq, e->gf_qn, (nq + 63) / 64 * 64, st));
-            HIP_TRY(e, hipMemsetAsync(e->gf_gate, 0, GF_GATE_BYTES, st));
             hipEvent_t ev_buf[4];
             hipEvent_t* ev = pass_events(e, 0, ev_buf);
             int width = 0, segs = 0;
-            HIP_TRY(e, msr_gemm_f32_topk(e->gf, e->dense, e->gf_qn, nq, k, out_doc + (int64_t)q0 * k,
+            HIP_TRY(e, msr_gemm_f32_topk(e->gf, e->dense, q + (int64_t)q0 * MSR_DIM, e->gf_qn, nq, k, out_doc + (int64_t)q0 * k,
                                          out_score + (int64_t)q0 * k, out_chunk ? out_chunk + (int64_t)q0 * k : nullptr,
-                                         out_n + q0, e->gf_gate, ev, &width, &segs, st));
+                                         out_n + q0, e->gf_gate, (int)(GF_GATE_BYTES / 4), ev, &width, &segs, st));
             e->last_dense_width = std::max(e->last_dense_width, width);
             e->last_dense_segments = segs;
             pass_events_used(e, 0, ev);
diff --git a/modern-search-engines-project_amd/csrc/msr_frag.h b/modern-search-engines-project_amd/csrc/msr_frag.h
--- a/modern-search-engines-project_amd/csrc/msr_frag.h
+++ b/modern-search-engines-project_amd/csrc/msr_frag.h
@@ -25,8 +25,11 @@
     h[4] = (_Float16)b.x; h[5] = (_Float16)b.y; h[6] = (_Float16)b.z; h[7] = (_Float16)b.w;
     return h;
 }
+__device__ __forceinline__ float f16_err(float x) {
+    const float h = (float)(_Float16)x;
+    return __builtin_fabsf(h) < 6.103515625e-05f ? x : h - x;
+}
 __device__ __forceinline__ float f16_err2(float x) {
-    const float h = (float)(_Float16)x;
-    const float d = __builtin_fabsf(h) < 6.103515625e-05f ? x : h - x;
+    const float d = f16_err(x);
     return d * d;
 }
diff --git a/modern-search-engines-project_amd/csrc/msr_gemm.hip b/modern-search-engines-project_amd/csrc/msr_gemm.hip
--- a/modern-search-engines-project_amd/csrc/msr_gemm.hip
+++ b/modern-search-engines-project_amd/csrc/msr_gemm.hip
@@ -116,21 +116,26 @@
     }
 }
 
-__global__ __launch_bounds__(1024) void gemm_kth_kernel(const float* __restrict__ tmax, int n, int stride, int nq, int k,
+constexpr int GM_KTH_LIST = 4096;
+template <bool LIST>
+__global__ __launch_bounds__(1024) void gemm_kth_kernel(float* __restrict__ tmax, int n, int stride, int nq, int k,
                                                          const float* __restrict__ margin, float* __restrict__ thr,
                                                          int32_t* __restrict__ flag, float short_val, float margin_scale,
-                                                         int raise) {
+                                                         int raise, int clear_n) {
     __shared__ uint32_t hist[2048];
     __shared__ uint32_t wsum[16];
-    __shared__ uint32_t s_bin, s_kk, s_hit;
+    __shared__ uint32_t s_bin, s_kk, s_hit, s_cnt;
+    __shared__ uint32_t list[LIST ? GM_KTH_LIST : 1];
     const int q = blockIdx.x, t = threadIdx.x, lane = t & 63, wave = t >> 6;
+    float* row = tmax + (size_t)q * stride;
     if (q >= nq) {
         if (t == 0 && !raise) { thr[q] = short_val; if (flag) flag[q] = 0; }
+        for (int i = t; i < clear_n; i += 1024) row[i] = -__builtin_inff();
         return;
     }
-    const float* row = tmax + (size_t)q * stride;
     uint32_t prefix = 0, mask = 0, kk = (uint32_t)k;
-    bool short_row = false;
+    bool short_row = false, listed = false;
+    if (LIST && t == 0) s_cnt = 0;
 #pragma unroll 1
     for (int pass = 0; pass < 3; ++pass) {
         const int shift = pass == 0 ? 21 : pass == 1 ? 10 : 0;
@@ -138,12 +143,47 @@
         hist[t] = 0; hist[t + 1024] = 0;
         if (t == 0) s_hit = 0;
         __syncthreads();
-        for (int i = t; i < n; i += 1024) {
-            const float x = row[i];
-            if (!msr_valid(x)) continue;
-            const uint32_t key = msr_ord32(x);
-            if ((key & mask) == prefix) atomicAdd(&hist[(key >> shift) & (nb - 1)], 1u);
-        }
+        if (LIST && pass == 0) {
+            for (int base = 0; base < n; base += 8 * 1024) {
+                float x[8];
+#pragma unroll
+                for (int u = 0; u < 8; ++u) {
+                    const int i = base + u * 1024 + t;
+                    x[u] = i < n ? row[i] : -__builtin_inff();
+                }
+#pragma unroll
+                for (int u = 0; u < 8; ++u) {
+                    const bool v = msr_valid(x[u]);
+                    const uint32_t key = msr_ord32(x[u]);
+                    const uint64_t m = __ballot(v);
+                    if (m != 0) {
+                        uint32_t slot0 = 0;
+                        if (lane == 0) slot0 = atomicAdd(&s_cnt, (uint32_t)__popcll(m));
+                        slot0 = __shfl(slot0, 0);
+                        if (v) {
+                            atomicAdd(&hist[key >> 21], 1u);
+                            const uint32_t slot = slot0 + (uint32_t)__popcll(m & ((1ull << lane) - 1ull));
+                            if (slot < (uint32_t)GM_KTH_LIST) list[slot] = key;
+                        }
+                    }
+                }
+            }
+        } else if (LIST && listed) {
+            const int cnt = (int)s_cnt;
+            for (int i = t; i < cnt; i += 1024) {
+                const uint32_t key = list[i];
+                if ((key & mask) == prefix) atomicAdd(&hist[(key >> shift) & (nb - 1)], 1u);
+            }
+        } else {
+            for (int i = t; i < n; i += 1024) {
+                const float x = row[i];
+                if (!msr_valid(x)) continue;
+                const uint32_t key = msr_ord32(x);
+                if ((key & mask) == prefix) atomicAdd(&hist[(key >> shift) & (nb - 1)], 1u);
+            }
+        }
+        __syncthreads();
+        if (LIST && pass == 0) listed = s_cnt <= (uint32_t)GM_KTH_LIST;
         __syncthreads();
         const uint32_t h0 = 2 * t < (int)nb ? hist[2 * t] : 0u, h1 = 2 * t + 1 < (int)nb ? hist[2 * t + 1] : 0u;
         const uint32_t c2 = h0 + h1;
@@ -178,6 +218,7 @@
             if (flag) flag[q] = short_row ? 1 : 0;
         }
     }
+    for (int i = t; i < clear_n; i += 1024) row[i] = -__builtin_inff();
 }
 
 
@@ -192,6 +233,39 @@
         const int4 e = wgbuf[(size_t)wg * wg_cap + i];
         if (__int_as_float(e.z) >= thr2[e.y]) {
             const int pos = atomicAdd(&pair_n[e.y], 1);
+            if (pos < pair_cap) pairs[(size_t)e.y * pair_cap + pos] = make_int2(e.x, e.z);
+        }
+    }
+}
+
+__global__ __launch_bounds__(1024) void gemm_bucket8_kernel(const int4* __restrict__ wgbuf, int wg_cap,
+                                                             const int32_t* __restrict__ wg_count, int n_wg,
+                                                             const float* __restrict__ thr2, int nq, int2* __restrict__ pairs,
+                                                             int pair_cap, int32_t* __restrict__ pair_n) {
+    extern __shared__ int32_t bucket_lds[];
+    int32_t* cnt = bucket_lds;
+    int32_t* first = bucket_lds + nq;
+    const int t = threadIdx.x, tl = t & 127, wg = blockIdx.x * 8 + (t >> 7);
+    for (int q = t; q < nq; q += 1024) cnt[q] = 0;
+    __syncthreads();
+    int n = wg < n_wg ? wg_count[wg] : 0;
+    if (n > wg_cap) n = wg_cap;
+    const int4* buf = wgbuf + (size_t)wg * wg_cap;
+    for (int i = tl; i < n; i += 128) {
+        const int4 e = buf[i];
+        if ((unsigned)e.y < (unsigned)nq && __int_as_float(e.z) >= thr2[e.y]) atomicAdd(&cnt[e.y], 1);
+    }
+    __syncthreads();
+    for (int q = t; q < nq; q += 1024) {
+        const int c = cnt[q];
+        first[q] = c ? atomicAdd(&pair_n[q], c) : 0;
+        cnt[q] = 0;
+    }
+    __syncthreads();
+    for (int i = tl; i < n; i += 128) {
+        const int4 e = buf[i];
+        if ((unsigned)e.y < (unsigned)nq && __int_as_float(e.z) >= thr2[e.y]) {
+            const int pos = first[e.y] + atomicAdd(&cnt[e.y], 1);
             if (pos < pair_cap) pairs[(size_t)e.y * pair_cap + pos] = make_int2(e.x, e.z);
         }
     }
@@ -352,17 +426,32 @@
     else gemm_tmax_kernel<0><<<grid, 256, 0, stream>>>(tmax_t, n_j, parts, nq_pad, out, out_stride);
     return hipGetLastError();
 }
-hipError_t msr_gemm_kth(const float* tmax, int n, int stride, int nq, int nq_pad, int k, const float* margin, float* thr,
-                        int32_t* flag, hipStream_t stream, float short_val, float margin_scale, bool raise) {
+hipError_t msr_gemm_kth(float* tmax, int n, int stride, int nq, int nq_pad, int k, const float* margin, float* thr,
+                        int32_t* flag, hipStream_t stream, float short_val, float margin_scale, bool raise, int clear_n,
+                        bool reread) {
     if (nq_pad <= 0) return hipSuccess;
-    gemm_kth_kernel<<<nq_pad, 1024, 0, stream>>>(tmax, n, stride, nq, k, margin, thr, raise ? nullptr : flag, short_val, margin_scale,
-                                                 raise ? 1 : 0);
-    return hipGetLastError();
-}
-hipError_t msr_gemm_bucket(const void* wvbuf, int wv_cap, const int32_t* wv_count, int n_waves, const float* thr2,
-                           void* pairs, int32_t* pair_n, hipStream_t stream) {
-    gemm_bucket_kernel<<<dim3(2, (unsigned)n_waves), 256, 0, stream>>>((const int4*)wvbuf, wv_cap, wv_count, thr2, (int2*)pairs,
-                                                                      GM_PAIR_CAP, pair_n);
+    if (clear_n < 0 || clear_n > stride) return hipErrorInvalidValue;
+#ifdef MSR_DIAG
+    if (reread) {
+        gemm_kth_kernel<false><<<nq_pad, 1024, 0, stream>>>(tmax, n, stride, nq, k, margin, thr, raise ? nullptr : flag, short_val,
+                                                            margin_scale, raise ? 1 : 0, clear_n);
+        return hipGetLastError();
+    }
+#endif
+    (void)reread;
+    gemm_kth_kernel<true><<<nq_pad, 1024, 0, stream>>>(tmax, n, stride, nq, k, margin, thr, raise ? nullptr : flag, short_val,
+                                                       margin_scale, raise ? 1 : 0, clear_n);
+    return hipGetLastError();
+}
+hipError_t msr_gemm_bucket(const void* wvbuf, int wv_cap, const int32_t* wv_count, int n_waves, const float* thr2, int nq,
+                           void* pairs, int32_t* pair_n, hipStream_t stream, bool per_entry) {
+    if (n_waves <= 0 || nq <= 0) return hipSuccess;
+    if (per_entry || nq > 4096)
+        gemm_bucket_kernel<<<dim3(2, (unsigned)n_waves), 256, 0, stream>>>((const int4*)wvbuf, wv_cap, wv_count, thr2, (int2*)pairs,
+                                                                          GM_PAIR_CAP, pair_n);
+    else
+        gemm_bucket8_kernel<<<(unsigned)((n_waves + 7) / 8), 1024, (size_t)nq * 8, stream>>>((const int4*)wvbuf, wv_cap, wv_count, n_waves,
+                                                                                           thr2, nq, (int2*)pairs, GM_PAIR_CAP, pair_n);
     return hipGetLastError();
 }
 hipError_t msr_gemm_tmax_clear(float* tmax, int stride, int nq_pad, hipStream_t stream) {
@@ -405,17 +494,16 @@
         if ((err = msr_stream256_bf16_launch(false, a, grid, stream)) != hipSuccess) return err;
         if (ev && (err = hipEventRecord(ev[1], stream)) != hipSuccess) return err;
         if ((err = msr_gemm_tmax(g.tmax_t, n_s, 1, nq_pad, (float*)g.tmax, g.tmax_stride, stream)) != hipSuccess) return err;
-        gemm_kth_kernel<<<nq_pad, 1024, 0, stream>>>((const float*)g.tmax, n_s, g.tmax_stride, nq, k, margin, g.thr, g.flag, __builtin_inff(), 1.0f, 0);
+        if ((err = msr_gemm_kth((float*)g.tmax, n_s, g.tmax_stride, nq, nq_pad, k, margin, g.thr, g.flag, stream)) != hipSuccess) return err;
         a.t_first = 0; a.t_stride = 1; a.t_count = g.n_tiles;
         a.thr = g.thr; a.wvbuf = g.wgbuf; a.wv_cap = g.wv_cap; a.wv_count = g.wv_count;
         if (ev && (err = hipEventRecord(ev[2], stream)) != hipSuccess) return err;
         if ((err = msr_stream256_bf16_launch(true, a, grid, stream)) != hipSuccess) return err;
         if (ev && (err = hipEventRecord(ev[3], stream)) != hipSuccess) return err;
         if ((err = msr_gemm_tmax(g.tmax_t, g.n_tiles, 1, nq_pad, (float*)g.tmax, g.tmax_stride, stream)) != hipSuccess) return err;
-        gemm_kth_kernel<<<nq_pad, 1024, 0, stream>>>((const float*)g.tmax, g.n_tiles, g.tmax_stride, nq, k, margin, g.thr2, nullptr, __builtin_inff(), 1.0f, 0);
-    }
-    gemm_bucket_kernel<<<dim3(2, (unsigned)grid * 8), 256, 0, stream>>>((const int4*)g.wgbuf, g.wv_cap, g.wv_count, g.thr2,
-                                                                       (int2*)g.pairs, GM_PAIR_CAP, g.pair_n);
+        if ((err = msr_gemm_kth((float*)g.tmax, g.n_tiles, g.tmax_stride, nq, nq_pad, k, margin, g.thr2, nullptr, stream)) != hipSuccess) return err;
+    }
+    if ((err = msr_gemm_bucket(g.wgbuf, g.wv_cap, g.wv_count, grid * 8, g.thr2, nq, g.pairs, g.pair_n, stream)) != hipSuccess) return err;
     gemm_cand_kernel<<<nq, 1024, 0, stream>>>((int2*)g.pairs, g.pair_n, ix.chunk_doc, ix.n_chunks, g.wv_count, grid * 8, g.wv_cap,
                                               g.flag, k, margin, cand_doc, cand_first_len, cand_n);
     return hipGetLastError();
diff --git a/modern-search-engines-project_amd/csrc/msr_gemm_f32.hip b/modern-search-engines-project_amd/csrc/msr_gemm_f32.hip
--- a/modern-search-engines-project_amd/csrc/msr_gemm_f32.hip
+++ b/modern-search-engines-project_amd/csrc/msr_gemm_f32.hip
@@ -725,16 +725,64 @@
     if (lane == 0) atomicMax(err_max, __float_as_uint(worst));
 }
 
+__device__ __forceinline__ float f16_margin_of(float ss, const uint32_t* __restrict__ err_max) {
+#pragma clang fp contract(off)
+    for (int o = 32; o > 0; o >>= 1) ss += __shfl_xor(ss, o);
+    const float r = sqrtf(ss);
+    const float dq = r * 1.0001f, one_dq = __builtin_fmaf(r, 1.0001f, 1.0f), dE = __uint_as_float(*err_max) * 1.0001f;
+    const float a = dq * 1.000001f, b = dE * one_dq;
+    return __builtin_fmaf(2.0f, a + b, 1.0e-4f);
+}
 __global__ __launch_bounds__(256) void f16_margin_kernel(const float* __restrict__ qn, int nq, const uint32_t* __restrict__ err_max,
                                                           float* __restrict__ margin) {
     const int q = blockIdx.x * 4 + (threadIdx.x >> 6), lane = threadIdx.x & 63;
     if (q >= nq) return;
     float ss = 0.f;
-    for (int j = lane; j < MSR_DIM; j += 64) ss += f16_err2(qn[(size_t)q * MSR_DIM + j]);
-    for (int o = 32; o > 0; o >>= 1) ss += __shfl_xor(ss, o);
-    if (lane == 0) {
-        const float dq = sqrtf(ss) * 1.0001f, dE = __uint_as_float(*err_max) * 1.0001f;
-        margin[q] = 2.0f * (dE * (1.0f + dq) + dq * 1.000001f) + 1.0e-4f;
+    for (int j = lane; j < MSR_DIM; j += 64) {
+        const float d = f16_err(qn[(size_t)q * MSR_DIM + j]);
+        ss = __builtin_fmaf(d, d, ss);
+    }
+    const float m = f16_margin_of(ss, err_max);
+    if (lane == 0) margin[q] = m;
+}
+
+template <int MODE>
+__global__ __launch_bounds__(256) void prepare_kernel(const float* __restrict__ q, int nq, int nq_pad64, float* __restrict__ qn,
+                                                       f16x8* __restrict__ qimg, const uint32_t* __restrict__ err_max,
+                                                       float* __restrict__ margin, int32_t* __restrict__ gate, int gate_words,
+                                                       f32x4* __restrict__ tmax4, size_t n4, int n_qwg) {
+    constexpr int W = MODE == 0 ? 128 : 256;
+    __shared__ __attribute__((aligned(16))) float rows[4][MSR_DIM];
+    const int t = threadIdx.x, lane = t & 63, w = t >> 6;
+    if ((int)blockIdx.x >= n_qwg) {
+        const size_t i = (size_t)(blockIdx.x - n_qwg) * 256 + t;
+        const float ninf = -__builtin_inff();
+        if (i < n4) tmax4[i] = (f32x4){ninf, ninf, ninf, ninf};
+        return;
+    }
+    if (blockIdx.x == 0 && t < gate_words) gate[t] = 0;
+    const int row = blockIdx.x * 4 + w;
+    float v[12];
+    for (int j = 0; j < 12; ++j) v[j] = row < nq ? q[(size_t)row * MSR_DIM + lane + 64 * j] : 0.f;
+    msr_wave_normalise(v);
+    float ss = 0.f;
+    for (int j = 0; j < 12; ++j) {
+        if (row < nq_pad64) qn[(size_t)row * MSR_DIM + lane + 64 * j] = v[j];
+        rows[w][lane + 64 * j] = v[j];
+        const float d = f16_err(v[j]);
+        ss = __builtin_fmaf(d, d, ss);
+    }
+    if (row < nq) {
+        const float m = f16_margin_of(ss, err_max);
+        if (lane == 0) margin[row] = m;
+    }
+    __syncthreads();
+    const int g = row / W, ql = row % W;
+    for (int i = lane; i < GF_KT * 4; i += 64) {
+        const int cp = i & 3, kt = i >> 2;
+        const int c = cp ^ (((ql >> 3) & 1) << 1);
+        const float* src = &rows[w][MODE == 2 ? 64 * (kt >> 1) + 16 * c + 8 * (kt & 1) : 32 * kt + 8 * c];
+        qimg[(size_t)g * (GF_KT * W * 4) + ((size_t)kt * W + ql) * 4 + cp] = cvt_f16_rtn(*(const f32x4*)src, *(const f32x4*)(src + 4));
     }
 }
 
@@ -966,12 +1014,13 @@
 
 }
 
-hipError_t msr_gemm_f32_pass(const GemmF32Index& g, const DenseIndex& ix, const float* qn, int nq, int k, int k_part,
-                             float* out_part, hipEvent_t* ev, int* width_out, int* seg_out, hipStream_t stream) {
+hipError_t msr_gemm_f32_pass(const GemmF32Index& g, const DenseIndex& ix, const float* q, float* qn, int nq, int k, int k_part,
+                             float* out_part, int32_t* gate, int gate_words, hipEvent_t* ev, int* width_out, int* seg_out,
+                             hipStream_t stream) {
     const int W = nq > 128 ? 256 : 128;
     const int waves = 8;
     const int G = (nq + W - 1) / W;
-    if (nq <= 0 || G * W > 128 * g.max_groups || k < 1 || g.n_tiles < 2 * k) return hipErrorInvalidValue;
+    if (nq <= 0 || G * W > 128 * g.max_groups || k < 1 || g.n_tiles < 2 * k || gate_words < 0 || gate_words > 256) return hipErrorInvalidValue;
     if (width_out) *width_out = W;
     hipError_t err;
     int NT0 = 1;
@@ -980,10 +1029,35 @@
 #ifdef MSR_DIAG
     if (g_f32_dbg & (2048 | 1048576)) image16 = false;
 #endif
-    if (image16) build_qimg2_kernel<true, false><<<dim3((GF_KT * 256 * 4 + 255) / 256, G), 256, 0, stream>>>(qn, nq, (f16x8*)g.qimg);
-    else if (W == 256) build_qimg2_kernel<false><<<dim3((GF_KT * 256 * 4 + 255) / 256, G), 256, 0, stream>>>(qn, nq, (f16x8*)g.qimg);
-    else build_qimg1_kernel<<<dim3((GF_KT * 128 * 4 + 255) / 256, G), 256, 0, stream>>>(qn, nq, (f16x8*)g.qimg);
-    f16_margin_kernel<<<(nq + 3) / 4, 256, 0, stream>>>(qn, nq, g.err_max, g.margin);
+    bool parent_chain = false;
+#ifdef MSR_DIAG
+    parent_chain = (g_f32_dbg & 67108864) != 0;
+#endif
+    bool entry_tmax = W == 256 && !image16;
+#ifdef MSR_DIAG
+    if (g_f32_dbg & 33554432) entry_tmax = false;
+#endif
+    const int nq_pad64 = (nq + 63) / 64 * 64;
+#ifdef MSR_DIAG
+    if (parent_chain) {
+        if ((err = msr_prep_queries(q, nq, qn, nq_pad64, stream)) != hipSuccess) return err;
+        if (gate_words && (err = hipMemsetAsync(gate, 0, (size_t)gate_words * 4, stream)) != hipSuccess) return err;
+        if (image16) build_qimg2_kernel<true, false><<<dim3((GF_KT * 256 * 4 + 255) / 256, G), 256, 0, stream>>>(qn, nq, (f16x8*)g.qimg);
+        else if (W == 256) build_qimg2_kernel<false><<<dim3((GF_KT * 256 * 4 + 255) / 256, G), 256, 0, stream>>>(qn, nq, (f16x8*)g.qimg);
+        else build_qimg1_kernel<<<dim3((GF_KT * 128 * 4 + 255) / 256, G), 256, 0, stream>>>(qn, nq, (f16x8*)g.qimg);
+        f16_margin_kernel<<<(nq + 3) / 4, 256, 0, stream>>>(qn, nq, g.err_max, g.margin);
+    } else
+#endif
+    {
+        const size_t n4 = entry_tmax ? (size_t)W * G * g.tmax_stride / 4 : 0;
+        if (entry_tmax && g.tmax_stride % 4 != 0) return hipErrorInvalidValue;
+        const int n_qwg = W * G / 4;
+        const unsigned blocks = (unsigned)(n_qwg + (n4 + 255) / 256);
+        if (image16) prepare_kernel<2><<<blocks, 256, 0, stream>>>(q, nq, nq_pad64, qn, (f16x8*)g.qimg, g.err_max, g.margin, gate, gate_words, (f32x4*)g.tmax, n4, n_qwg);
+        else if (W == 256) prepare_kernel<1><<<blocks, 256, 0, stream>>>(q, nq, nq_pad64, qn, (f16x8*)g.qimg, g.err_max, g.margin, gate, gate_words, (f32x4*)g.tmax, n4, n_qwg);
+        else prepare_kernel<0><<<blocks, 256, 0, stream>>>(q, nq, nq_pad64, qn, (f16x8*)g.qimg, g.err_max, g.margin, gate, gate_words, (f32x4*)g.tmax, n4, n_qwg);
+    }
+    if ((err = hipGetLastError()) != hipSuccess) return err;
     const float* margin = g.margin;
     const int grid = g.n_cus;
     const PassShape shape = pass_shape(g.n_tiles, k, grid, g.single_emit != 0, g_f32_dbg);
@@ -1016,12 +1090,9 @@
         if (ev && gi == 0 && (err = hipEventRecord(ev[1], stream)) != hipSuccess) return err;
         if ((err = msr_gemm_tmax(g.tmax_t, n_s, tmax_parts, W * a.nt, g.tmax + (size_t)gi * W * g.tmax_stride, g.tmax_stride, stream)) != hipSuccess) return err;
     }
-    if ((err = msr_gemm_kth(g.tmax, n_s, g.tmax_stride, nq, W * G, k, margin, g.thr, g.flag, stream)) != hipSuccess) return err;
-    bool entry_tmax = W == 256 && !image16;
-#ifdef MSR_DIAG
-    if (g_f32_dbg & 33554432) entry_tmax = false;
-#endif
-    if (entry_tmax && (err = msr_gemm_tmax_clear(g.tmax, g.tmax_stride, W * G, stream)) != hipSuccess) return err;
+    if ((err = msr_gemm_kth(g.tmax, n_s, g.tmax_stride, nq, W * G, k, margin, g.thr, g.flag, stream, __builtin_inff(), 1.0f, false,
+                            entry_tmax && !parent_chain ? n_s : 0, parent_chain)) != hipSuccess) return err;
+    if (entry_tmax && parent_chain && (err = msr_gemm_tmax_clear(g.tmax, g.tmax_stride, W * G, stream)) != hipSuccess) return err;
     a.t_stride = 1;
     a.wvbuf = g.wvbuf; a.wv_cap = g.wv_cap * (8 / waves); a.wv_count = g.wv_count;
     for (int s = 0; s < shape.n_seg; ++s) {
@@ -1040,12 +1111,14 @@
         if (entry_tmax && (err = msr_gemm_entry_tmax(g.wvbuf, a.wv_cap, g.wv_count, grid * waves, g.tmax, g.tmax_stride, t0,
                                                      g.n_tiles, W * G, stream)) != hipSuccess) return err;
         if (s + 1 < shape.n_seg &&
-            (err = msr_gemm_kth(g.tmax, t1, g.tmax_stride, nq, W * G, k, margin, g.thr, nullptr, stream, __builtin_inff(), 1.0f, true)) != hipSuccess)
+            (err = msr_gemm_kth(g.tmax, t1, g.tmax_stride, nq, W * G, k, margin, g.thr, nullptr, stream, __builtin_inff(), 1.0f, true, 0,
+                                parent_chain)) != hipSuccess)
             return err;
     }
-    if ((err = msr_gemm_kth(g.tmax, g.n_tiles, g.tmax_stride, nq, W * G, k, margin, g.thr2, nullptr, stream)) != hipSuccess) return err;
+    if ((err = msr_gemm_kth(g.tmax, g.n_tiles, g.tmax_stride, nq, W * G, k, margin, g.thr2, nullptr, stream, __builtin_inff(), 1.0f, false,
+                            0, parent_chain)) != hipSuccess) return err;
     if (out_part && (err = msr_gemm_kth(g.tmax, g.n_tiles, g.tmax_stride, nq, nq, k_part, margin, out_part, nullptr, stream,
-                                        -__builtin_inff(), 0.5f)) != hipSuccess) return err;
+                                        -__builtin_inff(), 0.5f, false, 0, parent_chain)) != hipSuccess) return err;
     return hipSuccess;
 }
 
@@ -1070,7 +1143,11 @@
         raise_thr_kernel<<<(nq + 255) / 256, 256, 0, stream>>>(g.thr2, bound, g.margin, nq);
         if ((err = hipGetLastError()) != hipSuccess) return err;
     }
-    if ((err = msr_gemm_bucket(g.wvbuf, wv_cap, g.wv_count, grid * waves, g.thr2, g.pairs, g.pair_n, stream)) != hipSuccess) return err;
+    bool parent_chain = false;
+#ifdef MSR_DIAG
+    parent_chain = (g_f32_dbg & 67108864) != 0;
+#endif
+    if ((err = msr_gemm_bucket(g.wvbuf, wv_cap, g.wv_count, grid * waves, g.thr2, nq, g.pairs, g.pair_n, stream, parent_chain)) != hipSuccess) return err;
     gemm_f32_cand_kernel<<<nq, 1024, 0, stream>>>((int2*)g.pairs, g.pair_n, ix.chunk_doc, ix.n_chunks, g.wv_count, grid * waves,
                                                   wv_cap, g.flag, g.cand_doc, g.cand_chunk, g.cand_n, gate);
     if ((err = hipGetLastError()) != hipSuccess) return err;
@@ -1078,10 +1155,11 @@
                                   g.cand_n, out_doc, out_score, out_chunk, out_n, stream);
 }
 
-hipError_t msr_gemm_f32_topk(const GemmF32Index& g, const DenseIndex& ix, const float* qn, int nq, int k,
+hipError_t msr_gemm_f32_topk(const GemmF32Index& g, const DenseIndex& ix, const float* q, float* qn, int nq, int k,
                              int32_t* out_doc, float* out_score, int32_t* out_chunk,
-                             int32_t* out_n, int32_t* gate, hipEvent_t* ev, int* width_out, int* seg_out, hipStream_t stream) {
-    hipError_t err = msr_gemm_f32_pass(g, ix, qn, nq, k, k, nullptr, ev, width_out, seg_out, stream);
+                             int32_t* out_n, int32_t* gate, int gate_words, hipEvent_t* ev, int* width_out, int* seg_out,
+                             hipStream_t stream) {
+    hipError_t err = msr_gemm_f32_pass(g, ix, q, qn, nq, k, k, nullptr, gate, gate_words, ev, width_out, seg_out, stream);
     if (err != hipSuccess) return err;
     return msr_gemm_f32_finish(g, ix, qn, nq, k, nullptr, out_doc, out_score, out_chunk, out_n, gate, stream);
 }
diff --git a/modern-search-engines-project_amd/csrc/msr_internal.h b/modern-search-engines-project_amd/csrc/msr_internal.h
--- a/modern-search-engines-project_amd/csrc/msr_internal.h
+++ b/modern-search-engines-project_amd/csrc/msr_internal.h
@@ -290,11 +290,11 @@
 };
 int msr_gemm_pair_cap();
 hipError_t msr_gemm_tmax(const float* tmax_t, int n_j, int parts, int nq_pad, float* out, int out_stride, hipStream_t stream);
-hipError_t msr_gemm_kth(const float* tmax, int n, int stride, int nq, int nq_pad, int k, const float* margin, float* thr,
+hipError_t msr_gemm_kth(float* tmax, int n, int stride, int nq, int nq_pad, int k, const float* margin, float* thr,
                         int32_t* flag, hipStream_t stream, float short_val = __builtin_inff(), float margin_scale = 1.0f,
-                        bool raise = false);
-hipError_t msr_gemm_bucket(const void* wvbuf, int wv_cap, const int32_t* wv_count, int n_waves, const float* thr2,
-                           void* pairs, int32_t* pair_n, hipStream_t stream);
+                        bool raise = false, int clear_n = 0, bool reread = false);
+hipError_t msr_gemm_bucket(const void* wvbuf, int wv_cap, const int32_t* wv_count, int n_waves, const float* thr2, int nq,
+                           void* pairs, int32_t* pair_n, hipStream_t stream, bool per_entry = false);
 hipError_t msr_gemm_tmax_clear(float* tmax, int stride, int nq_pad, hipStream_t stream);
 hipError_t msr_gemm_entry_tmax(const void* wvbuf, int wv_cap, const int32_t* wv_count, int n_waves, float* tmax, int stride,
                                int tile_lo, int n_tiles, int nq_pad, hipStream_t stream);
@@ -355,11 +355,13 @@
 hipError_t msr_f16_row_error(const float* emb, const float* inv_norm, int64_t n_rows, uint32_t* err_max, hipStream_t stream);
 void msr_gemm_f32_set_dbg(int v);
 hipError_t msr_pad_inv_norm(const float* inv, int64_t n, int64_t n_pad, float* out, hipStream_t stream);
-hipError_t msr_gemm_f32_topk(const GemmF32Index& g, const DenseIndex& ix, const float* qn, int nq, int k,
+hipError_t msr_gemm_f32_topk(const GemmF32Index& g, const DenseIndex& ix, const float* q, float* qn, int nq, int k,
                              int32_t* out_doc, float* out_score, int32_t* out_chunk,
-                             int32_t* out_n, int32_t* gate, hipEvent_t* ev, int* width_out, int* seg_out, hipStream_t stream);
-hipError_t msr_gemm_f32_pass(const GemmF32Index& g, const DenseIndex& ix, const float* qn, int nq, int k, int k_part,
-                             float* out_part, hipEvent_t* ev, int* width_out, int* seg_out, hipStream_t stream);
+                             int32_t* out_n, int32_t* gate, int gate_words, hipEvent_t* ev, int* width_out, int* seg_out,
+                             hipStream_t stream);
+hipError_t msr_gemm_f32_pass(const GemmF32Index& g, const DenseIndex& ix, const float* q, float* qn, int nq, int k, int k_part,
+                             float* out_part, int32_t* gate, int gate_words, hipEvent_t* ev, int* width_out, int* seg_out,
+                             hipStream_t stream);
 hipError_t msr_gemm_f32_finish(const GemmF32Index& g, const DenseIndex& ix, const float* qn, int nq, int k, const float* bound,
                                int32_t* out_doc, float* out_score, int32_t* out_chunk, int32_t* out_n, int32_t* gate,
                                hipStream_t stream);
```

After: 63960. Within noise of the previous version (-0.1%).
